# jjhbw/GoMILP

Measured on AMD Instinct MI355X. Metric: simplex pivots/sec on 2048x4096 fp64 dense LP, higher is better.
Workload: dtype f64

## Files before the change

gomilp_amd/csrc/c_api.cpp:

```cpp
#include <math.h>
#include <stdint.h>
#include <stdio.h>
#include <stdlib.h>
#include <string.h>

#include <atomic>
#include <chrono>
#include <condition_variable>
#include <deque>
#include <functional>
#include <map>
#include <memory>
#include <mutex>
#include <string>
#include <thread>
#include <vector>

#include "engine.hpp"
#include "engine_batch.hpp"
#include "engine_batch_revised.hpp"
#include "lu_host.h"

using gomilp::BatchEngine;
using gomilp::Engine;
// ... 625 lines not shown

extern "C" {

int gomilp_frontier_solve_roots(gomilp_pool *pool, int64_t count, const int32_t *root_of, const int64_t *koff, const int32_t *var,
                                const double *sign, const double *rhs, double tol, double *z_out, double *x_out, int64_t ldx,
                                int32_t *status_out, int32_t *has_x_out, gomilp_frontier_stats *stats) {
    return frontier_solve_impl(pool, count, root_of, koff, var, sign, rhs, tol, z_out, x_out, ldx, status_out, has_x_out, stats, nullptr);
}

int gomilp_frontier_solve_warm(gomilp_pool *pool, int64_t count, const int64_t *koff, const int32_t *var, const double *sign,
                               const double *rhs, const int64_t *parent, const int64_t *tag, const int32_t *keep, int32_t dual_budget,
                               double tol, double *z_out, double *x_out, int32_t *status_out, int32_t *has_x_out,
                               gomilp_frontier_stats *stats) {
    if (!pool) return GOMILP_ERR_BAD_SHAPE;
    WarmArgs wa{parent, tag, keep, dual_budget};
    return frontier_solve_impl(pool, count, nullptr, koff, var, sign, rhs, tol, z_out, x_out, pool->n0, status_out, has_x_out, stats, &wa);
}

int gomilp_pool_release_warm(gomilp_pool *pool, int64_t tag) {
    if (!pool) return GOMILP_ERR_BAD_SHAPE;
    std::lock_guard<std::mutex> g(pool->call_mu);
    if (tag < 0) pool->warm.clear(); else pool->warm.release(tag);
    return GOMILP_OK;
}

int gomilp_frontier_solve(gomilp_pool *pool, int64_t count, const int64_t *koff, const int32_t *var, const double *sign,
                          const double *rhs, double tol, double *z_out, double *x_out, int32_t *status_out,
                          int32_t *has_x_out, gomilp_frontier_stats *stats) {
    if (!pool) return GOMILP_ERR_BAD_SHAPE;
    return gomilp_frontier_solve_roots(pool, count, nullptr, koff, var, sign, rhs, tol, z_out, x_out, pool->n0, status_out, has_x_out, stats);
}

int gomilp_pool_solve_root(gomilp_pool *pool, double tol, double *opt_f, double *opt_x, int32_t *has_x, gomilp_lp_stats *stats) {
    if (!pool || pool->root[0] < 0) return GOMILP_ERR_BAD_SHAPE;
    std::lock_guard<std::mutex> g(pool->call_mu);
    return pool->eng[0]->solve(pool->root[0], tol, nullptr, opt_f, opt_x, has_x, nullptr, stats);
}

int gomilp_pool_add_root(gomilp_pool *pool, const double *c, const double *A, int64_t lda, const double *b, int64_t m, int64_t n) {
    if (!pool) return -GOMILP_ERR_BAD_SHAPE;
    std::lock_guard<std::mutex> g(pool->call_mu);
    if (pool->root[0] < 0) return -GOMILP_ERR_BAD_SHAPE;
    const int64_t id = pool->eng[0]->upload(c, A, lda, b, m, n);
    if (id < 0) return (int)id;
    std::unique_ptr<Engine::RootView> v(new Engine::RootView);
    if (!pool->eng[0]->root_view(id, v.get())) return -GOMILP_ERR_DEVICE;
    if (!v->unit_basis && v->verify_status == GOMILP_OK) pool->eng[0]->root_general(id, v.get());
    pool->extra_root.push_back(id);
    pool->extra_view.push_back(std::move(v));
    return (int)pool->extra_root.size();
}

int64_t gomilp_debug_find_independent(const double *A, int64_t lda, int64_t m, int64_t n, int64_t *idx_out, int fast) {
    if (!A || !idx_out || m <= 0 || n <= 0 || lda < n || m > 4096 || n > (1 << 20)) return -GOMILP_ERR_BAD_SHAPE;
    std::vector<double> a((size_t)m * n);
    for (int64_t i = 0; i < m; i++) for (int64_t j = 0; j < n; j++) a[(size_t)i * n + j] = A[i * lda + j];
    std::vector<int32_t> idx;
    if (fast) gomilp::general_find_linearly_independent(a, (int)m, (int)n, idx);
    else gomilp::general_find_linearly_independent_slow(a, (int)m, (int)n, idx);
    for (size_t k = 0; k < idx.size(); k++) idx_out[k] = idx[k];
    return (int64_t)idx.size();
}

double gomilp_debug_cond_estimate(const double *B, int64_t n, int inf) {
    if (!B || n <= 0 || n > 4096) return -1.0;
    std::vector<double> b((size_t)n * n), inv;
    for (int64_t i = 0; i < n * n; i++) b[(size_t)i] = B[i];
    if (!gomilp::general_invert(b, (int)n, inv)) return -1.0;
    double norm = 0;
    if (!inf) { for (int64_t j = 0; j < n; j++) { double s2 = 0; for (int64_t i = 0; i < n; i++) s2 += fabs(b[(size_t)(i * n + j)]); norm = std::max(norm, s2); } }
    else { for (int64_t i = 0; i < n; i++) { double s2 = 0; for (int64_t j = 0; j < n; j++) s2 += fabs(b[(size_t)(i * n + j)]); norm = std::max(norm, s2); } }
    return norm * gomilp::inverse_norm1_estimate(inv, (int)n, inf != 0);
}

int gomilp_debug_gonum_lu_cond(const double *M, int64_t n, int transposed, double *cond) {
    if (!M || !cond || n < 1 || n > gomilp::kGonumCondMax) return -1;
    bool dz = false;
    if (!gomilp::gonum_lu_cond(M, (int)n, (int)n, transposed != 0, cond, &dz)) return -1;
    return dz ? 1 : 0;
}

int gomilp_debug_lu_host_solve(int64_t m, int64_t nd, const int32_t *dl, const int32_t *phys, const double *diag, const double *W, int coupled,
                               const double *rhs, double *x) {
    if (m < 1 || m > 16384 || nd < 0 || nd > m || !phys || !diag || !rhs || !x || (nd > 0 && (!dl || !W))) return -1;
    const int64_t nx = coupled ? nd : m;
    for (int64_t i = 0; i < nx; i++) x[i] = 0.0;
    if (gomilp::lu_det_is_zero(diag, phys, (int)m)) return 1;
    if (coupled) {
        std::vector<double> xdl((size_t)nd);
        gomilp::lu_host_solve_coupled((int)nd, dl, phys, diag, W, rhs, xdl.data(), x);
    } else gomilp::lu_host_solve((int)m, (int)nd, dl, phys, diag, W, rhs, x);
    return 0;
}

int64_t gomilp_debug_find_independent_device(gomilp_ctx *ctx, int64_t problem, int64_t *idx_out, int64_t cap) {
    if (!ctx || !idx_out) return -GOMILP_ERR_BAD_SHAPE;
    std::vector<int32_t> idx;
    const int rc = ctx->eng->debug_find_independent(problem, idx);
    if (rc != GOMILP_OK && rc != GOMILP_ERR_SINGULAR) return -rc;
    for (size_t k = 0; k < idx.size() && (int64_t)k < cap; k++) idx_out[k] = idx[k];
    return (int64_t)idx.size();
}

long long gomilp_debug_loop_rep_launches(void) { return gomilp::bt_loop_rep_launches(); }
#ifdef GOMILP_DEBUG
void gomilp_debug_luc_stamps(unsigned long long *out) { gomilp::luc_stamps_read(out); }
void gomilp_debug_lux_stamps(unsigned long long *out) { gomilp::lux_stamps_read(out); }
void gomilp_debug_res_stamps(unsigned long long *out) { gomilp::res_stamps_read(out); }
#endif

int64_t gomilp_lp_last_trace(gomilp_ctx *ctx, gomilp_pivot *out, int64_t cap) {
    if (!ctx) return -1;
    return ctx->eng->last_trace(out, cap);
}

namespace {
constexpr int kFlatMaxCtx = 32;
struct FlatPool {
    std::mutex mu;
    std::condition_variable cv;
    std::vector<gomilp_ctx *> free_list;
    int created = 0;
};
FlatPool &flat_pool(int dev) {
    static std::mutex mu;
    static std::map<int, FlatPool *> pools;
    std::lock_guard<std::mutex> g(mu);
    auto it = pools.find(dev);
    if (it == pools.end()) it = pools.emplace(dev, new FlatPool).first;
    return *it->second;
}
}

int gomilp_lp_simplex(const double *c, const double *A, int64_t lda, const double *b, int64_t m, int64_t n, double tol,
                      const int64_t *initial_basic, double *opt_f, double *opt_x, int32_t *has_x, int64_t *basis_out,
                      gomilp_lp_stats *stats) {
    if (has_x) *has_x = 0;
    if (opt_f) *opt_f = NAN;
    if (!c || !A || !b || !opt_f || !opt_x || !has_x || m <= 0 || n <= 0 || lda < n) return GOMILP_ERR_BAD_SHAPE;
    int dev = 0;
    if (gomilp::device_count() <= 0 || hipGetDevice(&dev) != hipSuccess) return GOMILP_ERR_DEVICE;
    FlatPool &fp = flat_pool(dev);
    gomilp_ctx *ctx = nullptr;
    {
        std::unique_lock<std::mutex> lk(fp.mu);
        for (;;) {
            if (!fp.free_list.empty()) { ctx = fp.free_list.back(); fp.free_list.pop_back(); break; }
            if (fp.created < kFlatMaxCtx) { fp.created++; break; }
            fp.cv.wait(lk);
        }
    }
    if (!ctx) {
        int st = 0;
        ctx = gomilp_ctx_create(dev, &st);
        if (!ctx) {
            { std::lock_guard<std::mutex> lk(fp.mu); fp.created--; }
            fp.cv.notify_one();
            return st;
        }
    }
    int rc;
    int64_t id = ctx->eng->upload(c, A, lda, b, m, n, true);
    if (id < 0) rc = (int)-id;
    else {
        rc = gomilp_lp_solve_resident(ctx, id, tol, initial_basic, opt_f, opt_x, has_x, basis_out, stats);
        gomilp_lp_free(ctx, id);
    }
    { std::lock_guard<std::mutex> lk(fp.mu); fp.free_list.push_back(ctx); }
    fp.cv.notify_one();
    return rc;
}

}
```

gomilp_amd/csrc/device_types.h:

```cpp
#pragma once
#include <stdint.h>
#include <stdlib.h>

#ifdef GOMILP_DEBUG
#define GOMILP_DBG_ENV(name) getenv(name)
#else
#define GOMILP_DBG_ENV(name) (static_cast<const char *>(nullptr))
#endif

namespace gomilp {

enum : int32_t {
    ST_RUNNING = 0,
    ST_OPTIMAL = 1,
    ST_UNBOUNDED = 2,
    ST_NEED_BLAND = 3,
    ST_MAX_PIVOTS = 4,
    ST_LU_SINGULAR = 5,
    ST_BLAND_FAILED = 6,
    ST_FORCED_DONE = 7,
    ST_XCHG_TIMEOUT = 9,
    ST_DUAL_INFEASIBLE = 11,
    ST_NEED_EXACT = 10
};
// ... 128 lines not shown
    BS_HOST = 5,
    BS_DUAL_START = 7,
    BS_DUAL = 8,
    BS_COLD = 9
};

struct BatchLP {
    BTArgs bt;
    const double *At0;
    const double *c0, *b0;
    const int32_t *rho0;
    const int32_t *var;
    const double *sign, *rhs;
    int32_t ld0, m0, n0, K;
    int32_t m, n;
    int32_t ldu, cap_ldt;
    double *T[2];
    double *R, *xb, *U, *V, *scratch, *art;
    int32_t *basic, *nonbasic, *srcpos;
    DevState *st;
    const double *gT0;
    const double *gxb0;
    const int32_t *gbasic0, *gnonbasic0;
    const int32_t *gposvar0;
    int32_t gldt, gen;
    const double *wT, *wxb;
    const int32_t *wbasic, *wnonbasic, *wposvar;
    int32_t warm, wm;
    int32_t dual_budget, art_pos;
    int64_t pivd;
    const double *A0r;
    int32_t lda0r, virt, virt_t0, pad2;
    double tol_user;
    int32_t stage;
    int32_t tcur;
    int32_t do_permute, do_r, r_phase;
    int32_t perm_ld_in, perm_nn_out;
    int32_t kblock;
    int32_t status;
    int32_t wrapped;
    int32_t phase1_used, pad0;
    int64_t piv1, piv2, bland;
};

struct BatchOut {
    int32_t stage, status, wrapped, phase1_used;
    int64_t piv1, piv2, bland, pivd;
    int32_t tcur, pad;
};

struct GsState {
    int32_t k;
    int32_t accept;
    int32_t kacc;
    int32_t done;
    int32_t stop_col;
    int32_t scanned;
    double nR, nRinv;
    double vv;
    double beta_last;
};

struct GsBlock {
    int32_t nacc;
    int32_t k0;
    int32_t pad0, pad1;
    double vv[16];
};

struct LUCtl {
    int32_t k_next;
    int32_t k0, k1;
    int32_t nsteps;
    int32_t ndrop;
    int32_t rounds;
    int32_t nnext;
    int32_t ksync;
    int32_t steps[32];
    int32_t prow[32];
    int32_t dropcol[32], dropin[32], dropout[32];
    int32_t next[32];
    uint32_t cnt_x, cnt_u, cnt_s;
    int32_t fault;
};

struct LUArgs {
    double *W;
    int32_t ldw, m;
    int32_t *lpos;
    int32_t *rowstep;
    unsigned long long *pk[2];
    unsigned int *pl[2];
    unsigned int *pr[2];
    DevState *st;
    const int32_t *unit_row;
    int32_t *dense_flag;
    LUCtl *ctl;
    double *Lp, *Up;
    int32_t slots, look;
    const LUCtl *ctl_prev;
    const double *Lp_prev, *Up_prev;
    int32_t *rowsnap;
    const int32_t *rowsnap_prev;
    LUCtl *ctl_base;
    int32_t round, pad3;
};

}
```

gomilp_amd/csrc/engine.cpp:

```cpp
#include "engine_work.hpp"

#include <condition_variable>
#include <atomic>

namespace gomilp {

int device_count() {
    int n = 0;
    if (hipGetDeviceCount(&n) != hipSuccess) return 0;
    return n;
}

const char *compiled_arch() { return "gfx950"; }

Engine::Engine(int device) : device_(device), w_(new Work) {}

Engine::~Engine() {
    hipSetDevice(device_);
    if (up_dA_) hipFree(up_dA_);
    if (up_stats_) hipFree(up_stats_);
    for (auto *vec : {&problems_, &child_pool_, &root_pool_})
        for (auto &p : *vec) {
            if (!p) continue;
            hipFree(p->dAt); hipFree(p->db);
            if (!p->is_child) {
                hipFree(p->dc); hipFree(p->dc1);
                if (p->dvar) hipFree(p->dvar);
                if (p->dsign) hipFree(p->dsign);
            }
        }
    for (auto &kv : kept_) if (kv.second.d) hipFree(kv.second.d);
    for (auto &b : keep_pool_) hipFree(b.first);
    w_->release_all();
    if (stream_) hipStreamDestroy(stream_);
}

namespace {
struct LoopSlots { std::mutex mu; std::condition_variable cv; int used = 0, big_waiting = 0; bool busy[4] = {false, false, false, false}; };
LoopSlots &loop_slots(int dev) { static LoopSlots s[64]; return s[dev & 63]; }
}
int Engine::loop_acquire(int dev, int weight) {
    LoopSlots &L = loop_slots(dev);
    std::unique_lock<std::mutex> lk(L.mu);
    if (weight >= 4) {
        L.big_waiting++;
        L.cv.wait(lk, [&] { return L.used == 0; });
        L.big_waiting--;
        L.used = 4;
        for (bool &b2 : L.busy) b2 = true;
        return 0;
    }
    L.cv.wait(lk, [&] { return L.used < 4 && L.big_waiting == 0; });
    L.used++;
    for (int i = 0; i < 4; i++) if (!L.busy[i]) { L.busy[i] = true; return i; }
    return 0;
}
bool Engine::loop_try_acquire_all(int dev) {
    LoopSlots &L = loop_slots(dev);
    std::lock_guard<std::mutex> lk(L.mu);
    if (L.used != 0 || L.big_waiting != 0) return false;
    L.used = 4;
    for (bool &b2 : L.busy) b2 = true;
    return true;
}
void Engine::loop_release(int dev, int weight, int slot) {
    LoopSlots &L = loop_slots(dev);
    {
        std::lock_guard<std::mutex> lk(L.mu);
        if (weight >= 4) { L.used = 0; for (bool &b2 : L.busy) b2 = false; }
        else { L.used--; L.busy[slot & 3] = false; }
    }
    L.cv.notify_all();
}

int Engine::set(const std::string &key, int64_t v) {
    std::lock_guard<std::mutex> g(mu_);
    if (key == "chunk") { if (v < 1) return GOMILP_ERR_BAD_SHAPE; chunk_ = v; }
    else if (key == "refresh") { if (v < 0) return GOMILP_ERR_BAD_SHAPE; refresh_ = v; }
    else if (key == "trace") trace_on_ = v ? 1 : 0;
    else if (key == "max_pivots") max_pivots_ = v < 0 ? 0 : v;
    else if (key == "sample_events") sample_events_ = v < 0 ? 0 : v;
    else if (key == "fused") fused_ = v ? 1 : 0;
    else if (key == "lu_look") lu_look_ = v ? 1 : 0;
    else if (key == "lu_large") lu_large_ = v ? 1 : 0;
    else if (key == "lu_blocked") lu_blocked_ = v < 0 ? 0 : (v > 2 ? 3 : v);
    else if (key == "tableau") tableau_ = v ? 1 : 0;
    else if (key == "blocked") blocked_ = v ? 1 : 0;
    else if (key == "bt_nt") { if (v != 0 && v != 256 && v != 512 && v != 1024) return GOMILP_ERR_BAD_SHAPE; bt_nt_ = v; }
    else if (key == "bt_old") bt_old_ = v ? 1 : 0;
    else if (key == "bt_upd_valu") bt_upd_valu_ = v ? 1 : 0;
#ifdef GOMILP_DEBUG
    else if (key == "bt_fault") bt_fault_ = v;
#endif
    else if (key == "general_device") general_device_ = v ? 1 : 0;
    else if (key == "lu_cross") lu_cross_ = v < 0 ? -1 : (v > 2 ? 2 : v);
    else if (key == "general_block") general_block_ = v ? 1 : 0;
    else if (key == "general_min_rows") general_min_rows_ = v < 2 ? 2 : v;
    else if (key == "bt_groups") { if (v != -1 && v != 0 && v != 2 && v != 4 && v != 8 && v != 16) return GOMILP_ERR_BAD_SHAPE; bt_groups_ = v; }
    else if (key == "bt_stamps") bt_stamps_ = v ? 1 : 0;
    else if (key == "bt_lag") bt_lag_ = v ? 1 : 0;
    else if (key == "exact_degenerate") { if (v < 0 || v > 3) return GOMILP_ERR_BAD_SHAPE; exact_degenerate_ = v; }
    else if (key == "loop_grid") { if (v < 0 || v > 4096) return GOMILP_ERR_BAD_SHAPE; loop_grid_ = v; }
    else if (key == "loop_chunk") { if (v < 32) return GOMILP_ERR_BAD_SHAPE; loop_chunk_ = v; }
    else if (key == "cond_guard") cond_guard_ = v ? 1 : 0;
    else if (key == "poll_delay") { if (v < 0 || v > 64) return GOMILP_ERR_BAD_SHAPE; poll_delay_ = v; }
    else if (key == "loop_upd") { if (v < 0) return GOMILP_ERR_BAD_SHAPE; loop_upd_ = v; }
    else if (key == "loop_rep") loop_rep_ = v ? 1 : 0;
    else if (key == "loop_g") { if (v != 0 && v != 8 && v != 16) return GOMILP_ERR_BAD_SHAPE; loop_g_ = v; }
    else if (key == "loop_k") { if (v != 0 && v != 8 && v != 12 && v != 16) return GOMILP_ERR_BAD_SHAPE; loop_k_ = v; }
    else if (key == "row_chunk") { if (v < 0 || v % 512 != 0 || v > kLdsWindowLd) return GOMILP_ERR_BAD_SHAPE; row_chunk_ = v; }
    else if (key == "block_k") { if (v < 0 || v > bt_max_k()) return GOMILP_ERR_BAD_SHAPE; block_k_ = v; }
    else return GOMILP_ERR_BAD_SHAPE;
    return GOMILP_OK;
}

int Engine::ensure_work(int m, int ncols) {
    HIP_TRY(hipSetDevice(device_));
    if (!stream_) HIP_TRY(hipStreamCreateWithFlags(&stream_, hipStreamNonBlocking));
    Work &w = *w_;
    if (!w.st) {
        int ncu = 0;
        if (hipDeviceGetAttribute(&ncu, hipDeviceAttributeMultiprocessorCount, device_) == hipSuccess && ncu > 0) ncu_ = ncu;
        HIP_TRY(dmalloc(&w.pk_price, 2 * kMaxPartials)); HIP_TRY(dmalloc(&w.pk_ratio, 2 * kMaxPartials));
        HIP_TRY(dmalloc(&w.pi_price, kMaxPartials)); HIP_TRY(dmalloc(&w.pi_ratio, kMaxPartials));
        HIP_TRY(dmalloc(&w.pv_price, kMaxPartials)); HIP_TRY(dmalloc(&w.pb_ratio, kMaxPartials)); HIP_TRY(dmalloc(&w.pd_ratio, kMaxPartials)); HIP_TRY(dmalloc(&w.px_ratio, kMaxPartials));
        for (int t = 0; t < 2; t++) {
            HIP_TRY(dmalloc(&w.lpk[t], kMaxPartials)); HIP_TRY(dmalloc(&w.lpl[t], kMaxPartials)); HIP_TRY(dmalloc(&w.lpr[t], kMaxPartials));
        }
        HIP_TRY(dmalloc(&w.st, 1));
        HIP_TRY(hipHostMalloc(reinterpret_cast<void **>(&w.st_host), sizeof(DevState), hipHostMallocDefault));
        HIP_TRY(dmalloc(&w.luctl, 2));
        HIP_TRY(hipHostMalloc(reinterpret_cast<void **>(&w.luctl_host), 2 * sizeof(LUCtl), hipHostMallocDefault));
        w.trace_cap = 1 << 18;
        HIP_TRY(dmalloc(&w.trace, (size_t)w.trace_cap));
        HIP_TRY(hipEventCreate(&w.ev[0])); HIP_TRY(hipEventCreate(&w.ev[1]));
    }
    const int ld = (m + 1) & ~1;
    if (m <= w.cap_m && ncols <= w.cap_cols) return GOMILP_OK;
    const int nm = std::max(m + 32 + m / 16, w.cap_m), nc = std::max(ncols + 64 + ncols / 16, w.cap_cols);
    const int nld = std::max((nm + 1) & ~1, w.cap_ld);
    w.release();
    for (auto &p : w.binv) HIP_TRY(dmalloc(&p, (size_t)nm * nld));
    HIP_TRY(dmalloc(&w.W, (size_t)nm * nld));
    HIP_TRY(dmalloc(&w.xb, (size_t)nld)); HIP_TRY(dmalloc(&w.yb[0], (size_t)nld)); HIP_TRY(dmalloc(&w.yb[1], (size_t)nld));
    HIP_TRY(dmalloc(&w.dvec, (size_t)nld));
    HIP_TRY(dmalloc(&w.move, (size_t)nld)); HIP_TRY(dmalloc(&w.rvec, (size_t)nc));
    HIP_TRY(dmalloc(&w.yscratch, (size_t)64 * nld));
    HIP_TRY(dmalloc(&w.basic, (size_t)nm + (size_t)nc)); w.nonbasic = w.basic + nm;
    HIP_TRY(dmalloc(&w.lpos, (size_t)nm)); HIP_TRY(dmalloc(&w.rowstep, (size_t)3 * nm)); HIP_TRY(dmalloc(&w.rho, (size_t)nm));
    HIP_TRY(dmalloc(&w.unitrow, (size_t)nm)); HIP_TRY(dmalloc(&w.denseflag, (size_t)nm)); HIP_TRY(dmalloc(&w.dlist, (size_t)nm));
    HIP_TRY(dmalloc(&w.ludiag, (size_t)nm)); HIP_TRY(dmalloc(&w.Wd, (size_t)nm * nld + 512));
    HIP_TRY(dmalloc(&w.luLp, (size_t)64 * nld)); HIP_TRY(dmalloc(&w.luUp, (size_t)64 * nld));
    HIP_TRY(hipHostMalloc(reinterpret_cast<void **>(&w.h_W), ((size_t)nm * nld + 512) * sizeof(double), hipHostMallocDefault));
    HIP_TRY(hipHostMalloc(reinterpret_cast<void **>(&w.h_vec), (size_t)std::max(nld, nc) * sizeof(double), hipHostMallocDefault));
    HIP_TRY(hipHostMalloc(reinterpret_cast<void **>(&w.h_chk), (size_t)nld * sizeof(double), hipHostMallocDefault));
    HIP_TRY(hipHostMalloc(reinterpret_cast<void **>(&w.h_idx), ((size_t)nm + (size_t)nc) * sizeof(int32_t), hipHostMallocDefault));
    {
        const size_t cap = std::max<size_t>(4096, sizeof(double) * ((size_t)std::max(nld, nc) + 64));
        for (int t = 0; t < Work::kStageSlots; t++) {
            if (w.stage_cap[t] >= cap) continue;
            if (w.stage_inflight) { hipStreamSynchronize(stream_); w.stage_inflight = 0; }
            if (w.stage_buf[t]) hipHostFree(w.stage_buf[t]);
            w.stage_buf[t] = nullptr; w.stage_cap[t] = 0;
            HIP_TRY(hipHostMalloc(reinterpret_cast<void **>(&w.stage_buf[t]), cap, hipHostMallocDefault));
            w.stage_cap[t] = cap;
        }
    }
    w.cap_m = nm; w.cap_ld = nld; w.cap_cols = nc;
    return GOMILP_OK;
}

int64_t Engine::upload(const double *c, const double *A, int64_t lda, const double *b, int64_t m64, int64_t n64, bool lazy_host) {
    std::lock_guard<std::mutex> g(mu_);
    if (!c || !A || !b || m64 <= 0 || n64 <= 0 || lda < n64 || m64 > (1 << 20) || n64 > (1 << 22)) return -GOMILP_ERR_BAD_SHAPE;
    const int m = (int)m64, n = (int)n64;
    const int ld = (m + 1) & ~1;
    if (ld > kLdsWindowLd && lds_window_only_) return -GOMILP_ERR_UNSUPPORTED;
    if (hipSetDevice(device_) != hipSuccess) return -GOMILP_ERR_DEVICE;
    if (!stream_ && hipStreamCreateWithFlags(&stream_, hipStreamNonBlocking) != hipSuccess) return -GOMILP_ERR_DEVICE;
    const double t0 = now_s();
    const size_t need_at = (size_t)(n + 1) * ld, need_c = (size_t)n + 1, need_b = (size_t)ld;
    std::unique_ptr<Problem> P;
    for (size_t i = 0; i < root_pool_.size(); i++) {
        Problem &q = *root_pool_[i];
        if (q.cap_at >= need_at && q.cap_c >= need_c && q.cap_b >= need_b) {
            P = std::move(root_pool_[i]);
            root_pool_.erase(root_pool_.begin() + i);
            break;
        }
    }
    const bool recycled = (bool)P;
    if (ld > kLdsWindowLd) {
        const size_t dbl = (up_dA_cap_ < (size_t)m * n ? (size_t)m * n : 0) + (recycled ? 0 : need_at + 2 * need_c + need_b);
        if (!device_fits(dbl * sizeof(double))) {
            if (recycled) root_pool_.push_back(std::move(P));
            return -GOMILP_ERR_UNSUPPORTED;
        }
    }
    if (!P) P.reset(new Problem);
    P->m = m; P->n = n; P->ld = ld;
    double *dA = nullptr;
    int32_t *dstats = nullptr;
    auto fail = [&](int code) -> int64_t {
        if (P->dAt) hipFree(P->dAt);
        if (P->dc) hipFree(P->dc);
        if (P->dc1) hipFree(P->dc1);
        if (P->db) hipFree(P->db);
        return -code;
    };
#define UP_TRY(expr) do { if ((expr) != hipSuccess) return fail(GOMILP_ERR_DEVICE); } while (0)
    if (up_dA_cap_ < (size_t)m * n) {
        if (up_dA_) hipFree(up_dA_);
        up_dA_ = nullptr; up_dA_cap_ = 0;
        UP_TRY(dmalloc(&up_dA_, (size_t)m * n));
        up_dA_cap_ = (size_t)m * n;
// ... 804 lines not shown
        {
            LPArgs a = make_args(P, 1, 1e-10, 0, P.dc1);
            launch_ftran(a, 0, -1, n, stream_);
            launch_update(a, 0, (int)minidx, 1, 0, stream_);
            launches_ += 2;
            cur_ ^= 1;
        }
        basic[minidx] = n;
        build_nonbasic(n + 1);
        if ((rc = upload_index_lists(basic, nonbasic)) != GOMILP_OK) return finish(rc);
        refresh_xb_y(P, P.dc1);
        HIP_TRY(hipMemcpyAsync(w.h_vec, w.xb, (size_t)m * sizeof(double), hipMemcpyDeviceToHost, stream_));
        HIP_TRY(sync_stream());
        for (int i = 0; i < m; i++) if (w.h_vec[i] < -1e-13) return finish(GOMILP_ERR_PANIC);
        rc = run_loop(P, 1, 1e-10, (int)nonbasic.size(), P.dc1, st);
        if (rc == GOMILP_ERR_DEVICE) return finish(rc);
        if (rc != GOMILP_OK) { st->wrapped_status = rc; return finish(GOMILP_ERR_PHASE1_WRAPPED); }
        HIP_TRY(hipMemcpyAsync(w.h_idx, w.basic, (size_t)m * sizeof(int32_t), hipMemcpyDeviceToHost, stream_));
        HIP_TRY(hipMemcpyAsync(w.h_vec, w.xb, (size_t)m * sizeof(double), hipMemcpyDeviceToHost, stream_));
        HIP_TRY(sync_stream());
        int added = -1;
        for (int i = 0; i < m; i++) { basic[i] = w.h_idx[i]; xb[i] = w.h_vec[i]; if (basic[i] == n) added = i; }
        double xart = added >= 0 ? xb[added] : 0.0;
        if (added >= 0 && fabs(xart) > 1e-13 && fabs(xart) < 1e-11) {
            if ((rc = final_solve(P, xb_exact, &singular)) != GOMILP_OK) return finish(rc);
            if (!singular) xart = xb_exact[added];
        }
        if (fabs(xart) > 1e-12) return finish(GOMILP_ERR_INFEASIBLE);
        if (added >= 0) {
            bool exchanged = false;
            std::vector<char> inb(n + 1, 0);
            for (int i = 0; i < m; i++) inb[basic[i]] = 1;
            for (int j = 0; j < n && !exchanged; j++) {
                if (inb[j]) continue;
                w.st_host->done = 0; w.st_host->status = ST_RUNNING; w.st_host->rq = 0;
                sync_state_to_device();
                LPArgs a = make_args(P, 1, 1e-10, 0, P.dc1);
                launch_ftran(a, 0, -1, j, stream_);
                launches_++;
                HIP_TRY(hipMemcpyAsync(w.h_vec, w.dvec, (size_t)m * sizeof(double), hipMemcpyDeviceToHost, stream_));
                HIP_TRY(sync_stream());
                double dmax = 0;
                for (int i = 0; i < m; i++) dmax = std::max(dmax, fabs(w.h_vec[i]));
                const double dpv = w.h_vec[added];
                if (!(fabs(dpv) > 1e-9 * std::max(1.0, dmax))) continue;
                const double theta = xb[added] / dpv;
                bool feas = true;
                for (int i = 0; i < m && feas; i++) {
                    const double v = (i == added) ? theta : xb[i] - theta * w.h_vec[i];
                    if (v < -1e-13) feas = false;
                }
                if (!feas) continue;
                launch_update(a, 0, added, 1, 0, stream_);
                launches_++;
                cur_ ^= 1;
                basic[added] = j;
                exchanged = true;
                st->art_exchanges++;
            }
            if (!exchanged) return finish(GOMILP_ERR_INFEASIBLE);
        }
    }

    build_nonbasic(n);
    if ((rc = upload_index_lists(basic, nonbasic)) != GOMILP_OK) return finish(rc);
    if (st->phase1_used) {
        refresh_xb_y(P, P.dc);
    } else {
        launch_y_from_binv(w.binv[cur_], P.ld, m, P.dc, w.basic, w.yscratch, w.yb[ycur_], stream_);
        launches_ += 2;
    }
    loop_rc = run_loop(P, 2, tol, (int)nonbasic.size(), P.dc, st);
    }
    rc = solve_tail(P, id, loop_rc, basic, xb, basic_start, unit_basis ? &rho : nullptr, opt_f, opt_x, has_x, basis_out, st);
    return finish(rc);
}

int Engine::solve_tail(const Problem &P, int64_t id, int loop_rc, std::vector<int32_t> &basic, std::vector<double> &xb,
                       const std::vector<int32_t> &basic_start, const std::vector<int32_t> *rho_slack, double *opt_f, double *opt_x,
                       int32_t *has_x, int64_t *basis_out, gomilp_lp_stats *st) {
    const double inf = std::numeric_limits<double>::infinity();
    const int m = P.m, n = P.n;
    Work &w = *w_;
    if (loop_rc == GOMILP_ERR_DEVICE) return loop_rc;
    const bool loop_unbounded = loop_rc == GOMILP_ERR_UNBOUNDED;
    if (loop_unbounded && !shadow_trace_) { *opt_f = -inf; return loop_rc; }

    HIP_TRY(hipMemcpyAsync(w.h_idx, w.basic, (size_t)m * sizeof(int32_t), hipMemcpyDeviceToHost, stream_));
    HIP_TRY(hipMemcpyAsync(w.h_vec, w.xb, (size_t)m * sizeof(double), hipMemcpyDeviceToHost, stream_));
    HIP_TRY(sync_stream());
    for (int i = 0; i < m; i++) { basic[i] = w.h_idx[i]; xb[i] = w.h_vec[i]; }
    if (shadow_trace_ && (loop_rc == GOMILP_OK || loop_rc == GOMILP_ERR_BLAND || loop_unbounded)) {
        HIP_TRY(hipMemcpyAsync(w.st_host, w.st, sizeof(DevState), hipMemcpyDeviceToHost, stream_));
        HIP_TRY(sync_stream());
        const int64_t cnt = std::min<int64_t>(w.st_host->trace_len, w.trace_cap);
        std::vector<DevPivot> tr((size_t)cnt);
        if (cnt) HIP_TRY(hipMemcpy(tr.data(), w.trace, (size_t)cnt * sizeof(DevPivot), hipMemcpyDeviceToHost));
        std::vector<std::pair<int, int>> piv;
        for (auto &e : tr) piv.emplace_back((int)e.replace, (int)e.entering);
        std::vector<int32_t> bas = basic_start;
        int cst = GOMILP_OK;
        int64_t evals = 0;
        const int stop = general_condition_replay(P.hA, m, n, bas, piv, loop_unbounded, &cst, &evals);
        st->cond_fallbacks += evals;
        if (cst != GOMILP_OK) {
            std::vector<double> xs;
            if (general_solve_basis(P.hA, m, n, bas, P.hb, xs)) {
                std::vector<double> cb(m);
                for (int i = 0; i < m; i++) cb[i] = P.hc[bas[i]];
                *opt_f = dot_unitary(cb.data(), xs.data(), m);
                for (int j = 0; j < n; j++) opt_x[j] = 0;
                for (int i = 0; i < m; i++) opt_x[bas[i]] = xs[i];
                *has_x = 1;
                if (basis_out) for (int i = 0; i < m; i++) basis_out[i] = bas[i];
                st->pivots_phase2 = stop;
                shadow_trace_ = false;
                return cst;
            }
        }
    }
    shadow_trace_ = false;
    if (loop_unbounded) { *opt_f = -inf; return loop_rc; }
    if (keep_id_ == id && loop_rc == GOMILP_OK) keep_capture(P, id, st->pipeline, basic, basic_start, rho_slack);
    const int rc = epilogue(P, basic, xb, loop_rc, opt_f, opt_x, has_x, basis_out, st);
    if (rc == GOMILP_ERR_DEVICE) return rc;
    if (trace_on_) {
        HIP_TRY(hipMemcpyAsync(w.st_host, w.st, sizeof(DevState), hipMemcpyDeviceToHost, stream_));
        HIP_TRY(sync_stream());
        last_trace_total_ = w.st_host->trace_len;
        const int64_t cnt = std::min<int64_t>(last_trace_total_, w.trace_cap);
        std::vector<DevPivot> tmp((size_t)cnt);
        if (cnt) HIP_TRY(hipMemcpy(tmp.data(), w.trace, (size_t)cnt * sizeof(DevPivot), hipMemcpyDeviceToHost));
        last_trace_.resize((size_t)cnt);
        for (int64_t i = 0; i < cnt; i++) {
            last_trace_[i].phase = tmp[i].phase; last_trace_[i].bland = tmp[i].bland;
            last_trace_[i].min_idx = tmp[i].min_idx; last_trace_[i].replace = tmp[i].replace;
            last_trace_[i].entering = tmp[i].entering; last_trace_[i].leaving = tmp[i].leaving;
        }
    }
    return rc;
}

int Engine::epilogue(const Problem &P, std::vector<int32_t> &basic, std::vector<double> &xb, int loop_rc, double *opt_f,
                     double *opt_x, int32_t *has_x, int64_t *basis_out, gomilp_lp_stats *st) {
    const int m = P.m, n = P.n;
    std::vector<double> xb_exact;
    bool singular = false;
    const double t1 = now_s();
    int rc = final_solve(P, xb_exact, &singular, basic.data());
    if (rc != GOMILP_OK) return rc;
    st->seconds_final_solve = now_s() - t1;
    if (singular) {
        xb_exact = xb;
        if (loop_rc == GOMILP_OK) loop_rc = GOMILP_ERR_CONDITION;
    }
    double drift = 0;
    for (int i = 0; i < m; i++) drift = std::max(drift, fabs(xb[i] - xb_exact[i]));
    st->drift_xb = drift;
    std::vector<double> cb(m);
    for (int i = 0; i < m; i++) cb[i] = P.hc[basic[i]];
    *opt_f = dot_unitary(cb.data(), xb_exact.data(), m);
    for (int j = 0; j < n; j++) opt_x[j] = 0;
    for (int i = 0; i < m; i++) opt_x[basic[i]] = xb_exact[i];
    *has_x = 1;
    if (basis_out) for (int i = 0; i < m; i++) basis_out[i] = basic[i];
    return loop_rc;
}

bool Engine::root_view(int64_t id, RootView *out) {
    std::lock_guard<std::mutex> g(mu_);
    if (id < 0 || (size_t)id >= problems_.size() || !problems_[id]) return false;
    const Problem &P = *problems_[id];
    out->gen.reset();
    out->m = P.m; out->n = P.n; out->ld = P.ld; out->dAt = P.dAt; out->dc = P.dc; out->db = P.db;
// ... 250 lines not shown
```

gomilp_amd/csrc/engine.hpp:

```cpp
#pragma once
#include <hip/hip_runtime_api.h>
#include <stdint.h>

#include <functional>
#include <map>
#include <memory>
#include <mutex>
#include <string>
#include <vector>

#include "../../include/gomilp_lp.h"
#include "device_types.h"

namespace gomilp {

constexpr int kLdsWindowLd = 8192;
constexpr int kAutoRowChunk = 4096;

struct Problem {
    int m = 0, n = 0, ld = 0;
    double *dAt = nullptr;
    double *dc = nullptr;
    double *dc1 = nullptr;
    double *db = nullptr;
    std::vector<double> hb, hc;
    mutable std::vector<double> hA;
    std::vector<int32_t> nnz, lastrow, allone;
    int verify_status = GOMILP_OK;
    double seconds_upload = 0;
    uint64_t serial = 0;
    bool lazy_host = false;
    double scale_span = 1.0;
    bool is_child = false;
    size_t cap_at = 0, cap_c = 0, cap_b = 0;
    int32_t *dvar = nullptr;
    double *dsign = nullptr;
    int cap_k = 0;
    int64_t root = -1;
    const Problem *root_ptr = nullptr;
    std::vector<int32_t> kvar;
    std::vector<double> ksign;
};

struct LuPlan {
    int m = 0;
    bool compressed = false;
    bool blocked = false;
    bool large = false;
    bool small = false;
    bool look_wanted = false;
    int cross_G = 0;
    int cross_slots = 16;
    bool oneshot = false;
    bool inject_fault = false;
    int steps_down = 0;
    bool split(int nd) const { return compressed && m >= 1024 && nd > 0; }
    static LuPlan make(int m, int64_t lu_blocked, int64_t lu_look, int64_t lu_cross, int64_t lu_large, int64_t bt_fault, size_t small_pack_cap_bytes);
    bool step_down();
};
struct LuRoundsEnd { bool gave_up = false, landed = false; int enq = 0; };

class Engine {
   public:
    explicit Engine(int device);
    ~Engine();
    int device() const { return device_; }
    static int loop_acquire(int dev, int weight);
    static void loop_release(int dev, int weight, int slot);
    static bool loop_try_acquire_all(int dev);
    int set(const std::string &key, int64_t v);

    int64_t upload(const double *c, const double *A, int64_t lda, const double *b, int64_t m, int64_t n, bool lazy_host = false);
    int free_problem(int64_t id);
    int64_t upload_child(int64_t root, int K, const int32_t *var, const double *sign, const double *rhs);
    int64_t upload_child_of(Engine &owner, int64_t root, int K, const int32_t *var, const double *sign, const double *rhs);
    int solve(int64_t id, double tol, const int64_t *initial_basic, double *opt_f, double *opt_x, int32_t *has_x,
              int64_t *basis_out, gomilp_lp_stats *stats);
    int solve_warm(int64_t id, int64_t parent, int keep, int dual_budget, double tol, double *opt_f, double *opt_x, int32_t *has_x,
                   int64_t *basis_out, gomilp_lp_stats *stats, gomilp_warm_stats *wstats);
   private:
    int solve_locked(int64_t id, double tol, const int64_t *initial_basic, double *opt_f, double *opt_x, int32_t *has_x,
                     int64_t *basis_out, gomilp_lp_stats *stats);
    int solve_cold_locked(int64_t id, double tol, const int64_t *initial_basic, double *opt_f, double *opt_x, int32_t *has_x,
                          int64_t *basis_out, gomilp_lp_stats *stats);
    int solve_tail(const Problem &P, int64_t id, int loop_rc, std::vector<int32_t> &basic, std::vector<double> &xb,
                   const std::vector<int32_t> &basic_start, const std::vector<int32_t> *rho_slack, double *opt_f, double *opt_x,
                   int32_t *has_x, int64_t *basis_out, gomilp_lp_stats *st);
    struct Kept {
        double *d = nullptr;
        size_t cap = 0;
        int m = 0, ld = 0;
        bool no_warm = false;
        std::vector<int32_t> basic;
    };
    std::map<int64_t, Kept> kept_;
    std::vector<std::pair<double *, size_t>> keep_pool_;
    int64_t keep_id_ = -1;
    void keep_capture(const Problem &P, int64_t id, int pipeline, const std::vector<int32_t> &basic, const std::vector<int32_t> &basic_start,
                      const std::vector<int32_t> *rho_slack);
    void drop_kept(int64_t id);
    bool descendant(const Problem &P, int64_t parent, int *J) const;
    int warm_locked(int64_t id, const Kept &K, int J, int dual_budget, double tol, double *opt_f, double *opt_x, int32_t *has_x,
                    int64_t *basis_out, gomilp_lp_stats *st, gomilp_warm_stats *ws);
    int run_dual_loop(const Problem &P, double tol, int nn, int dual_budget, gomilp_warm_stats *ws);
   public:
    int64_t last_trace(gomilp_pivot *out, int64_t cap);

    struct RootView {
        int m = 0, n = 0, ld = 0;
        const double *dAt = nullptr, *dc = nullptr, *db = nullptr;
        double scale_span = 1.0;
        bool unit_basis = false;
        std::vector<int32_t> rho0;
        int verify_status = GOMILP_OK;
        uint64_t serial = 0;
        std::vector<double> hb, hc;
        struct General {
            int m = 0, nn = 0, ldt = 0;
            double *dT0 = nullptr, *dxb0 = nullptr;
            int32_t *dbasic0 = nullptr, *dnonbasic0 = nullptr, *dposvar0 = nullptr;
            ~General();
        };
        std::shared_ptr<General> gen;
        struct RowMajor { double *dA = nullptr; int lda = 0; ~RowMajor(); };
        std::shared_ptr<RowMajor> rm;
    };
    bool root_view(int64_t id, RootView *out);
    bool root_general(int64_t id, RootView *out);
    int finish_from_basis(int64_t id, const int32_t *basic, const double *xb_updated, int loop_rc, double *opt_f, double *opt_x,
                          int32_t *has_x, int64_t *basis_out, gomilp_lp_stats *stats);
    int debug_find_independent(int64_t id, std::vector<int32_t> &idxs);

    void limit_rows_to_lds_window() { lds_window_only_ = true; }

   private:
    struct Work;
    int row_chunk2(const Problem &P) const;
    bool device_fits(size_t bytes);
    bool large_solve_fits(const Problem &P);
    int ensure_work(int m, int ncols);
    const Problem *problem_ptr(int64_t id);
    int64_t upload_child_impl(const Problem &R, int64_t root_id, int K, const int32_t *var, const double *sign, const double *rhs);
    LPArgs make_args(const Problem &P, int phase, double tol, int nn, const double *cost);
    int run_loop(const Problem &P, int phase, double tol, int nn, const double *cost, gomilp_lp_stats *st);
    int run_loop_fused(const Problem &P, int phase, double tol, int nn, const double *cost, gomilp_lp_stats *st);
    int run_loop_tab(const Problem &P, int phase, double tol, int nn, gomilp_lp_stats *st);
    int host_bland_tab(const Problem &P, int phase, double tol, int nn, gomilp_lp_stats *st, int *par_out);
    TabArgs make_tab_args(const Problem &P, int phase, double tol, int nn);
    int tab_forced_pivot(const Problem &P, int phase, double tol, int nn, int q, int ent, double rq, int p, double dp, double xp,
                         int lea, int flags, long long t);
    int solve_tableau(const Problem &P, double tol, std::vector<int32_t> &basic, const std::vector<int32_t> &rho,
                      std::vector<double> &xb, bool feasible, gomilp_lp_stats *st, int *loop_rc,
                      const std::vector<double> *binv_host);
    void bt_layout(const Problem &P, bool tiled);
    BTArgs make_bt_args(const Problem &P, int phase, double tol, int nn, int kmax);
    void bt_plan(const Problem &P, int *K, bool *tiled, bool *lag = nullptr) const;
    int bt_forced_pivot(const Problem &P, int phase, double tol, int nn, int q, int p, int nocommit);
    int run_loop_bt(const Problem &P, int phase, double tol, int nn, gomilp_lp_stats *st);
    void account_samples(gomilp_lp_stats *st, const std::vector<int64_t> &sample_t, int64_t executed, int nk);
    int host_bland(const Problem &P, LPArgs &a, gomilp_lp_stats *st);
    int refresh_xb_y(const Problem &P, const double *cost);
    int epilogue(const Problem &P, std::vector<int32_t> &basic, std::vector<double> &xb, int loop_rc, double *opt_f, double *opt_x,
                 int32_t *has_x, int64_t *basis_out, gomilp_lp_stats *st);
    int final_solve(const Problem &P, std::vector<double> &xb_exact, bool *singular, const int32_t *basic_host = nullptr,
                    bool transpose = false, const double *rhs_host = nullptr);
    int lu_factor(const Problem &P, bool *singular, const int32_t *basic_host = nullptr, bool transpose = false);
    int lu_solve(const Problem &P, std::vector<double> &x, const double *rhs_host = nullptr);
    int gather_basis(const Problem &P, const LuPlan &plan, bool transpose);
    int upload_unit_rows(const Problem &P, const int32_t *basic_host, bool transpose, int *nonunit);
    int run_compressed_rounds(const LUArgs &a, const LuPlan &plan, int nonunit, LuRoundsEnd *end);
    int pack_and_fetch(const LUArgs &a, const LuPlan &plan, std::vector<int32_t> &dl);
    struct LuCache {
        bool valid = false, split = false, singular = false;
        int m = 0, nd = 0;
        std::vector<int32_t> phys, dl;
        std::vector<double> diag;
        LUArgs args;
    } lu_cache_;
    int exact_step(const Problem &P, int phase, double tol, int nn, int *q_out, int *p_out, gomilp_lp_stats *st);
    int exact_iter(const Problem &P, int phase, double tol, int nn, double *y_dev, double *r_dev, int ldr,
                   const std::function<int(int, int, const std::vector<int32_t> &, const std::vector<double> &)> &check_column, int *q_out,
                   int *p_out, gomilp_lp_stats *st);
    int exact_column_check(const Problem &P, const std::vector<int32_t> &basic, const std::vector<double> &dsol, const double *col_dev,
                           double *binv_dst, bool *rebuilt, gomilp_lp_stats *st);
    int cond_check(const Problem &P, int nn, double *k1, double *kinf);
    int cond_fresh(const Problem &P, const int32_t *basic_host, double *k1, double *kinf);
    int groups_knob(const Problem &P) const;
    bool ensure_host_A(const Problem &P);
    int find_independent_device(const Problem &P, std::vector<int32_t> &basic, std::vector<double> *binv_out, bool *binv_on_device = nullptr);
    int stage_upload(void *dst, const void *src, size_t bytes);
    hipError_t sync_stream();
    int upload_index_lists(const std::vector<int32_t> &basic, const std::vector<int32_t> &nonbasic);
    void sync_state_to_device();

    int device_;
    hipStream_t stream_ = nullptr;
    int ncu_ = 256;
    std::mutex mu_;
    std::vector<std::unique_ptr<Problem>> problems_;
    std::vector<std::unique_ptr<Problem>> child_pool_;
    std::vector<std::unique_ptr<Problem>> root_pool_;
    double *up_dA_ = nullptr; size_t up_dA_cap_ = 0;
    int32_t *up_stats_ = nullptr; size_t up_stats_cap_ = 0;
    std::unique_ptr<Work> w_;
    int64_t lu_look_faults_ = 0;
    int lu_look_fault_ = 0;
    int64_t lu_look_ = 1;
    int64_t lu_large_ = 0;
    int64_t chunk_ = 32, refresh_ = 0, trace_on_ = 0, max_pivots_ = 0, sample_events_ = 0, fused_ = 1, lu_blocked_ = 3, tableau_ = 1, blocked_ = 1, block_k_ = 0,
            bt_nt_ = 0, bt_old_ = 0, bt_stamps_ = 0, bt_upd_valu_ = 0, bt_fault_ = 0, general_device_ = 1, general_block_ = 1, general_min_rows_ = 96, lu_cross_ = -1, bt_groups_ = 0,
            bt_lag_ = 1,
            loop_chunk_ = 512,
            loop_grid_ = 0,
            poll_delay_ = 0,
            loop_upd_ = 0,
            loop_rep_ = 0,
            loop_g_ = 0,
            loop_k_ = 0,
            exact_degenerate_ = 1,
            cond_guard_ = 1,
            row_chunk_ = 0;
    bool lds_window_only_ = false;
    bool badly_scaled_ = false;
    bool gen_binv_dev_ = false;
    bool gen_start_ = false;
    bool gen_revised_ = false;
    double lp_guard_ = 0.0;
    std::vector<double> exact_xb_;
    bool xchg_timeout_ = false;
    bool shadow_trace_ = false;
    int cur_ = 0;
    int ycur_ = 0;
    int grid_ratio_ = 1;
    int tcur_ = 0, rcur_ = 0, ldt_ = 0;
    bool t_tiled_ = false;
    bool use_bt_ = false;
    int64_t launches_ = 0;
    double fs_device_ = 0, fs_host_ = 0;
    int64_t lu_dense_ = 0, lu_rounds_ = 0;
    std::vector<gomilp_pivot> last_trace_;
    int64_t last_trace_total_ = 0;
};

int general_find_linearly_independent(const std::vector<double> &A, int m, int n, std::vector<int32_t> &idxs, std::vector<double> *binv_out = nullptr);
int general_finish_last_column(const std::vector<double> &A, int m, int n, std::vector<int32_t> &idxs, int start_col, std::vector<double> *binv_out);
int general_find_linearly_independent_slow(const std::vector<double> &A, int m, int n, std::vector<int32_t> &idxs);
bool general_basis_inverse(const std::vector<double> &A, int m, int n, const std::vector<int32_t> &basic, int ncols_with_art,
                           const std::vector<double> &art, std::vector<double> &binv);

int general_condition_replay(const std::vector<double> &A, int m, int n, std::vector<int32_t> &basic, const std::vector<std::pair<int, int>> &pivots,
                             bool ended_in_compute_move, int *status_out, int64_t *evaluations);
double general_cond_inf(const std::vector<double> &A, int n);
bool general_invert(const std::vector<double> &B, int m, std::vector<double> &inv);
double inverse_norm1_estimate(const std::vector<double> &M, int n, bool transposed);
constexpr int kGonumCondMax = 64;
bool gonum_lu_cond(const double *M, int n, int ldm, bool transposed, double *cond, bool *det_zero);
bool gonum_lu_solve(const double *M, int n, int ldm, const double *b, double *x);
double general_basis_cond1(const std::vector<double> &A, int m, int n, const std::vector<int32_t> &basic, const std::vector<double> &art);
bool general_solve_basis(const std::vector<double> &A, int m, int n, const std::vector<int32_t> &basic, const std::vector<double> &b, std::vector<double> &x);

int device_count();
const char *compiled_arch();

int launch_price(const LPArgs &a, hipStream_t s, hipEvent_t e0 = nullptr, hipEvent_t e1 = nullptr);
int launch_ftran(const LPArgs &a, int nparts_price, int forced_pos, int forced_var, hipStream_t s, hipEvent_t e0 = nullptr,
                 hipEvent_t e1 = nullptr);
void launch_update(const LPArgs &a, int nparts_ratio, int forced_p, int no_swap, int bland, hipStream_t s,
                   hipEvent_t e0 = nullptr, hipEvent_t e1 = nullptr);
void launch_dual_leave(const double *xb, int m, double tol, DevState *st, hipStream_t s);
int launch_dual_price(const LPArgs &a, hipStream_t s);
void launch_warm_binv(const double *Bp, int ldp, int mp, double *B, int ld, int m, const int32_t *kpos, const double *ksign, hipStream_t s);
void launch_tab_to_binv(const double *T, int ldt, bool tiled, int m, const int32_t *src, double *B, int ld, hipStream_t s);
bool fused_supported(int ld);
int launch_price_fused(const LPArgs &a, const double *y_in, double *y_out, int pending, int nparts_ratio, hipStream_t s,
                       hipEvent_t e0, hipEvent_t e1);
int launch_update_ftran_fused(const LPArgs &a, int pending, int nparts_price, hipStream_t s, hipEvent_t e0, hipEvent_t e1);
int tab_ld(int nn);
int launch_tableau_pivot(const TabArgs &a, int flags, int nparts, long long t, hipStream_t s, hipEvent_t e0, hipEvent_t e1);
void launch_tab_gather(const double *At, int ld, int m, int nn, const int32_t *nonbasic, const int32_t *rho, double *T, int ldt,
                       bool tiled, hipStream_t s);
void launch_tab_gemm(const double *Binv, int ldb, const double *At, int ld, int m, int nn, const int32_t *nonbasic, double *T, int ldt, bool tiled, hipStream_t s);
void launch_tab_permute_cols(const double *Tin, int ld_in, double *Tout, int ld_out, int m, int nn_out, const int32_t *srcpos,
                             bool tiled, hipStream_t s);
int tab_r_chunks(int m);
void launch_tab_r(const double *T, int ldt, int m, int nn, const double *cost, const int32_t *basic, const int32_t *nonbasic,
                  double *scratch, double *r, bool tiled, hipStream_t s);
void launch_tab_row_colmax(const double *T, int ldt, int m, int nn, int row, double *out, bool tiled, hipStream_t s);
void launch_tab_column(const double *T, int ldt, int m, int jp, const double *xb, double *dvec, double *move, bool tiled, hipStream_t s);
void launch_cond_check(const double *T, int ldt, int m, int nn, const int32_t *nonbasic, const int32_t *basic, const double *At, int ld, int slack0, int nvar,
                       double *scratch, bool tiled, hipStream_t s);
void launch_exact_r(const double *At, int ld, int m, int nn, const int32_t *nonbasic, const double *y, const double *cost, double *r, int ldt, hipStream_t s);
void launch_gs_init(double *QT, int ldq, int m, GsState *st, hipStream_t s);
void launch_gs_init_perm(double *QT, double *Rinv, int ldq, int m, const int32_t *perm, const double *sgn, const double *beta, int s0, GsState *st, hipStream_t s);
void launch_gs_candidate(const double *acol, double *QT, double *Rinv, int ldq, int m, double *w, double *t, double *ypart, int cand, int32_t *idxs, GsState *st, hipStream_t s,
                         int last = 0);
int launch_luc_rounds_cross(const LUArgs &base, int32_t *pivrow, int nrounds, int round_base, double *xrec, int G, int slots, hipStream_t s);
size_t luc_cross_doubles();
void launch_luc_lpos_final(const LUArgs &a, hipStream_t s);
int luc_cross_groups(int m, int want);
int luc_large_rpt(int m);
int gs_scratch_rows();
int gs_block_width(int m);
int gs_block_scratch_rows();
void launch_gs_block(const double *At, int ld, int col0, int ncand, double *QT, double *Rinv, int ldq, int m, double *scratch, int32_t *idxs, GsState *st, hipStream_t s);
void launch_gs_binv(const double *Rinv, const double *QT, int ldq, int m, double *C, hipStream_t s);
void launch_gs_art(const double *At, int ld, int m, const int32_t *basic, int minidx, const double *b, double *art, hipStream_t s);
void launch_gs_norms(const double *C, int ldq, int m, double *out, const double *At, int ld, const int32_t *idxs, int cand, double *colsum, hipStream_t s);
bool bt_supported(int m, int nn);
int bt_max_k();
int bt_reg_k(int m, int ldt, int nt_force);
bool bt_tiled(int m, int ldt, int kmax, int nt_force, bool old_only);
BtGroupCfg bt_group_cfg(int m, int ldt, int knob);
size_t bt_xbuf_doubles();
void launch_bt_inner_groups(const BTArgs &a, hipStream_t s, hipEvent_t e0, hipEvent_t e1);
const char *bt_group_kernel_name(int G, int ri);
constexpr int kBtStampSegs = 16;
void launch_bt_tile(const double *src, double *dst, int m, int ldt, bool to_tiles, hipStream_t s);
void launch_bt_inner(const BTArgs &a, hipStream_t s, hipEvent_t e0, hipEvent_t e1);
void launch_bt_update(const BTArgs &a, hipStream_t s, hipEvent_t e0, hipEvent_t e1);
bool bt_loop_supported(const BtGroupCfg &c);
void launch_bt_loop(const BTArgs &a, int ncu, hipStream_t s, hipEvent_t e0, hipEvent_t e1);
bool bt_loop_rep_supported(int m, int ldt);
int bt_loop_rep_threads(int m, int ldt);
long long bt_loop_rep_launches();
void launch_bt_loop_rep(const BTArgs &a, int ncu, hipStream_t s, hipEvent_t e0, hipEvent_t e1);
bool bt_batch_supported(int m_max, int ldt_max);
int bt_batch_k(int m_max, int ldt_max);
void launch_bt_inner_batch(const BatchLP *lps, const int *ids, const int *count, int nlp, int m_max, int ldt_max, hipStream_t s, hipEvent_t e0 = nullptr, hipEvent_t e1 = nullptr, int xcd_off = 0);
void launch_bt_update_batch(const BatchLP *lps, const int *ids, const int *count, int nlp, int m_max, int ldt_max, hipStream_t s, hipEvent_t e0 = nullptr, hipEvent_t e1 = nullptr);
const char *bt_batch_kernel_name(int m_max, int ldt_max);
bool bt_virt_batch_supported(int m_max, int ldt_max);
void launch_bt_inner_virt_batch(const BatchLP *lps, const int *ids, const int *count, int nlp, hipStream_t s, hipEvent_t e0 = nullptr, hipEvent_t e1 = nullptr);
int b_loop_slots(int ncu);
bool b_loop_supported(int m_max, int ldt_max);
void launch_b_loop(const BatchLP *lps, const int *ids, const int *count, int nlp, int nblocks, int par, hipStream_t s, hipEvent_t e0 = nullptr, hipEvent_t e1 = nullptr);
size_t b_res_slot_bytes();
int b_res_max_slots();
int b_res_groups(int m_max, int nn_max, int ldt_max);
void launch_b_res(const BatchLP *lps, const int *ids, const int *count, int nlp, int G, int nb, double seq0, void *xbase, hipStream_t s, hipEvent_t e0 = nullptr, hipEvent_t e1 = nullptr);
int batch_ldt(int nn);
void launch_b_setup(BatchLP *lps, int nlp, hipStream_t s);
void launch_b_setup_warm(BatchLP *lps, int nlp, hipStream_t s);
void launch_b_posvar(const int32_t *basic, int m, const int32_t *nonbasic, int nn, int32_t *posvar, hipStream_t s);
bool bt_dual_batch_supported(int m_max, int ldt_max);
void launch_bt_inner_dual_batch(const BatchLP *lps, const int *ids, const int *count, int nlp, int m_max, int ldt_max, hipStream_t s);
void launch_b_gather(const BatchLP *lps, int nlp, int m_max, int ldt_max, int mode, hipStream_t s);
void launch_b_write_virt(const BatchLP *lps, const int *ids, const int *count, int *list, int *nalive, int bound, int m_max, int ldt_max, int ncu, hipStream_t s);
void launch_b_ctrl(BatchLP *lps, const int *ids_in, const int *count_in, int bound, int n_max, BatchOut *outs, int *ids_out, int *count_out, int loop_par, hipStream_t s);
void launch_b_init_ids(int *ids, int *count, int nlp, hipStream_t s);
void launch_b_permute(const BatchLP *lps, const int *ids, const int *count, int bound, int m_max, int ldt_max, hipStream_t s);
void launch_b_tab_r(const BatchLP *lps, const int *ids, const int *count, int bound, int m_max, int ldt_max, hipStream_t s);
void launch_transpose_in(const double *A, int64_t lda, int m, int n, double *At, int ld, hipStream_t s);
void launch_col_stats(const double *At, int ld, int m, int n, int32_t *nnz, int32_t *lastrow, int32_t *allone, int32_t *rowflag, unsigned long long *range,
                      hipStream_t s);
void launch_set_binv_perm(double *binv, int ld, int m, const int32_t *rho, hipStream_t s);
void launch_child_assemble(const double *At0, int ld0, int m0, int n0, double *At1, int ld1, int K, const int32_t *var,
                           const double *sign, hipStream_t s);
void launch_matvec_rows(const double *M, int ld, int m, const double *vec, double *out, hipStream_t s, int row_chunk2 = 0);
int y_chunks(int m);
void launch_y_from_binv(const double *binv, int ld, int m, const double *cost, const int32_t *basic, double *scratch,
                        double *y, hipStream_t s);
void launch_gather_w(const double *At, int ld, int m, const int32_t *basic, double *W, int ldw, hipStream_t s);
int lu_grid(int m);
void launch_lu(const LUArgs &a, hipStream_t s);
bool lu_blocked_supported(int m);
int launch_lu_blocked(const LUArgs &a, int32_t *pivrow, hipStream_t s);
bool lu_compressed_supported(int m, bool large);
int lu_compressed_nb();
void launch_luc_init(const LUArgs &a, hipStream_t s);
int launch_luc_rounds(const LUArgs &a, int32_t *pivrow, int nrounds, int round_base, hipStream_t s);
void launch_luc_gather(const double *At, int ld, int m, const int32_t *basic, double *W, int ldw, hipStream_t s);
void launch_luc_pack_dense(const LUArgs &a, const int32_t *dlist, int nd, const int32_t *pivrow, double *Wdd, double *diag, hipStream_t s);
void launch_luc_solve_rows(const LUArgs &a, const int32_t *dlist, int nd, const double *b, const double *xdL, const double *xdU,
                           double *x, hipStream_t s);
void launch_luc_pack(const LUArgs &a, const int32_t *dlist, int nd, double *Wd, double *diag, hipStream_t s);
void launch_luc_pack_small(const LUArgs &a, double *out, hipStream_t s);
size_t luc_pack_small_bytes(int m);
void launch_lu_pack(const LUArgs &a, const int32_t *dlist, int nd, double *Wd, double *diag, hipStream_t s);

}
```

gomilp_amd/csrc/engine_final.cpp:

```cpp
#include <stdio.h>
#include <stdlib.h>

#include "engine_work.hpp"
#include "lu_host.h"

namespace gomilp {

int Engine::final_solve(const Problem &P, std::vector<double> &x, bool *singular, const int32_t *basic_host, bool transpose, const double *rhs_host) {
    int rc = lu_factor(P, singular, basic_host, transpose);
    if (rc != GOMILP_OK) return rc;
    return lu_solve(P, x, rhs_host);
}

LuPlan LuPlan::make(int m, int64_t lu_blocked, int64_t lu_look, int64_t lu_cross, int64_t lu_large, int64_t bt_fault, size_t small_pack_cap_bytes) {
    LuPlan p;
    p.m = m;
    p.compressed = lu_blocked >= 2 && lu_compressed_supported(m, lu_large != 0);
    p.large = p.compressed && luc_large_rpt(m) > 0;
    p.blocked = p.compressed || (lu_blocked && lu_blocked_supported(m));
    p.small = p.compressed && m <= 128;
    p.inject_fault = bt_fault == 2;
    const int cross_mode = lu_cross >= 0 ? (int)lu_cross : ((m > 1280 && m <= 2048 && lu_look) ? 2 : 0);
    p.cross_G = p.large ? 8 : ((cross_mode && p.compressed) ? luc_cross_groups(m, 1) : 0);
    p.cross_slots = (p.large ? lu_cross == 2 : cross_mode == 2) ? 32 : 16;
    p.look_wanted = lu_blocked >= 3 && lu_look && m > 768 && p.compressed && !p.large && !(p.cross_G && cross_mode != 2);
    p.oneshot = p.small && !p.cross_G && luc_pack_small_bytes(m) <= small_pack_cap_bytes;
    return p;
}

bool LuPlan::step_down() {
    if (steps_down >= 2 || !(look_wanted || cross_G)) return false;
    steps_down++;
    if (look_wanted) look_wanted = false; else cross_G = 0;
    if (large) compressed = blocked = large = false;
    oneshot = false;
    return true;
}

namespace {

struct LookSlot {
    int dev; bool held;
    LookSlot(int d, bool want) : dev(d), held(want && Engine::loop_try_acquire_all(d)) {}
    ~LookSlot() { drop(); }
    void drop() { if (held) Engine::loop_release(dev, 4, 0); held = false; }
};

}

int Engine::gather_basis(const Problem &P, const LuPlan &plan, bool transpose) {
    Work &w = *w_;
    if (plan.compressed != transpose) launch_luc_gather(P.dAt, P.ld, P.m, w.basic, w.W, P.ld, stream_);
    else {
        if (transpose) HIP_TRY(hipMemsetAsync(w.W, 0, (size_t)P.m * P.ld * sizeof(double), stream_));
        launch_gather_w(P.dAt, P.ld, P.m, w.basic, w.W, P.ld, stream_);
    }
    return GOMILP_OK;
}

int Engine::upload_unit_rows(const Problem &P, const int32_t *basic_host, bool transpose, int *nonunit) {
    Work &w = *w_;
    const int m = P.m;
    if (!basic_host) {
        HIP_TRY(hipMemcpyAsync(w.h_idx, w.basic, (size_t)m * sizeof(int32_t), hipMemcpyDeviceToHost, stream_));
        HIP_TRY(sync_stream());
        basic_host = w.h_idx;
    }
    std::vector<int32_t> ur(m);
    *nonunit = 0;
    for (int pos = 0; pos < m; pos++) {
        const int j = basic_host[pos];
        ur[pos] = (!transpose && j < P.n && P.nnz[j] == 1 && P.allone[j]) ? P.lastrow[j] : -1;
        if (ur[pos] < 0) (*nonunit)++;
    }
    return stage_upload(w.unitrow, ur.data(), (size_t)m * sizeof(int32_t));
}

int Engine::run_compressed_rounds(const LUArgs &a, const LuPlan &plan, int nonunit, LuRoundsEnd *end) {
    Work &w = *w_;
    const int m = a.m;
    int32_t *h_dense = w.h_idx + w.cap_m;
    launch_luc_init(a, stream_);
    launches_++;
    const int nb = lu_compressed_nb();
    int batch = std::max(1, (std::min(m, (5 * nonunit) / 2) + nb - 1) / nb);
    bool oneshot = plan.oneshot;
    if (oneshot && GOMILP_DBG_ENV("GOMILP_DEBUG_LU_SHORT")) batch = 1;
    int enq = 0;
    int k_seen = -1;
    const LUCtl *last = w.luctl_host;
    for (;;) {
        launches_ += plan.cross_G ? launch_luc_rounds_cross(a, w.rho, batch, enq, w.luxrec, plan.cross_G, plan.cross_slots, stream_) : launch_luc_rounds(a, w.rho, batch, enq, stream_);
        enq += batch;
        if (oneshot) {
            launch_luc_pack_small(a, w.Wd, stream_);
            launches_++;
            HIP_TRY(hipMemcpyAsync(w.h_W, w.Wd, luc_pack_small_bytes(m), hipMemcpyDeviceToHost, stream_));
            HIP_TRY(sync_stream());
            const double *blk = w.h_W;
            const int32_t *io = reinterpret_cast<const int32_t *>(blk + (size_t)m * m + m);
            memcpy(w.h_vec, blk + (size_t)m * m, (size_t)m * sizeof(double));
            memcpy(w.h_idx, io, (size_t)m * sizeof(int32_t));
            memcpy(h_dense, io + m, (size_t)m * sizeof(int32_t));
            memcpy(w.luctl_host, io + 2 * m, 2 * sizeof(LUCtl));
            w.st_host->lu_singular = io[2 * m + (int)(2 * sizeof(LUCtl) / sizeof(int32_t))];
        } else {
            HIP_TRY(hipMemcpyAsync(w.luctl_host, w.luctl, 2 * sizeof(LUCtl), hipMemcpyDeviceToHost, stream_));
            HIP_TRY(hipMemcpyAsync(h_dense, w.denseflag, (size_t)m * sizeof(int32_t), hipMemcpyDeviceToHost, stream_));
            HIP_TRY(sync_stream());
        }
        last = w.luctl_host + (a.look ? ((enq - 1) & 1) : 0);
        if (w.luctl_host[0].fault || last->k_next >= m) break;
        if (last->k_next <= k_seen) return GOMILP_ERR_DEVICE;
        k_seen = last->k_next;
        oneshot = false;
        batch = std::max(4, (int)(((int64_t)(m - last->k_next) * last->rounds) / std::max(1, last->k_next)) + 2);
        if (batch > 64) batch = 64;
    }
    lu_rounds_ = last->rounds;
    end->gave_up = w.luctl_host[0].fault != 0;
    end->landed = oneshot;
    end->enq = enq;
    if (plan.cross_G && !end->gave_up) { launch_luc_lpos_final(a, stream_); launches_++; }
    return GOMILP_OK;
}

int Engine::pack_and_fetch(const LUArgs &a, const LuPlan &plan, std::vector<int32_t> &dl) {
    Work &w = *w_;
    const int m = a.m;
    int32_t *h_dense = w.h_idx + w.cap_m;
    dl.clear();
    if (plan.blocked) {
        if (!plan.compressed) {
            HIP_TRY(hipMemcpyAsync(h_dense, w.denseflag, (size_t)m * sizeof(int32_t), hipMemcpyDeviceToHost, stream_));
            HIP_TRY(sync_stream());
        }
        for (int k = 0; k < m; k++) if (h_dense[k]) dl.push_back(k);
    } else {
        for (int k = 0; k < m; k++) dl.push_back(k);
    }
    const int nd = (int)dl.size();
    int rc = stage_upload(w.dlist, dl.data(), (size_t)nd * sizeof(int32_t));
    if (rc != GOMILP_OK) return rc;
    const bool split = plan.split(nd);
    if (split) launch_luc_pack_dense(a, w.dlist, nd, w.rho, w.Wd, w.ludiag, stream_);
    else if (plan.compressed) launch_luc_pack(a, w.dlist, nd, w.Wd, w.ludiag, stream_);
    else launch_lu_pack(a, w.dlist, nd, w.Wd, w.ludiag, stream_);
    launches_++;
    if (nd) HIP_TRY(hipMemcpyAsync(w.h_W, w.Wd, (size_t)(split ? nd : m) * nd * sizeof(double), hipMemcpyDeviceToHost, stream_));
    HIP_TRY(hipMemcpyAsync(w.h_vec, w.ludiag, (size_t)m * sizeof(double), hipMemcpyDeviceToHost, stream_));
    HIP_TRY(hipMemcpyAsync(w.h_idx, w.lpos, (size_t)m * sizeof(int32_t), hipMemcpyDeviceToHost, stream_));
    if (plan.small)
        HIP_TRY(hipMemcpyAsync(&w.st_host->lu_singular, &w.st->lu_singular, sizeof(w.st_host->lu_singular), hipMemcpyDeviceToHost, stream_));
    else
        HIP_TRY(hipMemcpyAsync(w.st_host, w.st, sizeof(DevState), hipMemcpyDeviceToHost, stream_));
    HIP_TRY(sync_stream());
    return GOMILP_OK;
}

int Engine::lu_factor(const Problem &P, bool *singular, const int32_t *basic_host, bool transpose) {
    Work &w = *w_;
    const double tf0 = now_s();
    const int m = P.m;
    LuPlan plan = LuPlan::make(m, lu_blocked_, lu_look_, lu_cross_, lu_large_, bt_fault_, ((size_t)w.cap_m * w.cap_ld + 512) * sizeof(double));
    lu_cache_.valid = false;
    int rc = gather_basis(P, plan, transpose);
    if (rc != GOMILP_OK) return rc;
    int nonunit = 0;
    if ((rc = upload_unit_rows(P, basic_host, transpose, &nonunit)) != GOMILP_OK) return rc;
    LookSlot look_slot(device_, plan.look_wanted);
    if (!look_slot.held) plan.look_wanted = false;
    LUArgs a;
    a.W = w.W; a.ldw = P.ld; a.m = m; a.lpos = w.lpos; a.rowstep = w.rowstep;
    for (int t = 0; t < 2; t++) { a.pk[t] = w.lpk[t]; a.pl[t] = w.lpl[t]; a.pr[t] = w.lpr[t]; }
    a.st = w.st;
    a.unit_row = w.unitrow;
    a.dense_flag = plan.blocked ? w.denseflag : nullptr;
    a.ctl = w.luctl; a.Lp = w.luLp; a.Up = w.luUp;
    a.slots = 1; a.look = plan.look_wanted ? 1 : 0;
    a.ctl_prev = a.ctl; a.Lp_prev = a.Lp; a.Up_prev = a.Up;
    a.rowsnap = w.rowstep + w.cap_m; a.rowsnap_prev = a.rowsnap;
    a.ctl_base = a.ctl; a.round = 0; a.pad3 = plan.inject_fault ? 1 : 0;
    if (plan.cross_G && !w.luxrec) {
        HIP_TRY(dmalloc(&w.luxrec, luc_cross_doubles()));
        HIP_TRY(hipMemsetAsync(w.luxrec, 0, luc_cross_doubles() * sizeof(double), stream_));
    }
    w.st_host->lu_singular = 0;
    if (!plan.small) sync_state_to_device();
    lu_rounds_ = 0;
    LuRoundsEnd end;
    if (plan.compressed) {
        for (;;) {
            rc = run_compressed_rounds(a, plan, nonunit, &end);
            look_slot.drop();
            if (rc != GOMILP_OK) return rc;
            if (!end.gave_up) break;
            if (!plan.step_down()) return GOMILP_ERR_DEVICE;
            a.look = 0; a.dense_flag = plan.blocked ? w.denseflag : nullptr;
            lu_look_faults_++; lu_look_fault_++;
            if (w.luxrec) HIP_TRY(hipMemsetAsync(w.luxrec, 0, luc_cross_doubles() * sizeof(double), stream_));
            if (GOMILP_DBG_ENV("GOMILP_DEBUG_LOOP")) fprintf(stderr, "final_solve: a look-ahead launch gave up a wait (m %d, rounds enqueued %d, cnt_x %u cnt_u %u cnt_s %u): plain schedule\n", m, end.enq, w.luctl_host[0].cnt_x, w.luctl_host[0].cnt_u, w.luctl_host[0].cnt_s);
            if ((rc = gather_basis(P, plan, transpose)) != GOMILP_OK) return rc;
            if (!plan.compressed) { lu_rounds_ = 0; sync_state_to_device(); launch_lu(a, stream_); launches_ += m + 2; end = LuRoundsEnd(); break; }
        }
    } else if (plan.blocked) launches_ += launch_lu_blocked(a, w.rho, stream_) + 1;
    else { launch_lu(a, stream_); launches_ += m + 2; }
    std::vector<int32_t> dl;
    if (end.landed) {
        dl.resize(m);
        for (int k = 0; k < m; k++) dl[k] = k;
        const int32_t *h_dense = w.h_idx + w.cap_m;
        lu_dense_ = 0;
        for (int k = 0; k < m; k++) lu_dense_ += h_dense[k] != 0;
    } else {
        if ((rc = pack_and_fetch(a, plan, dl)) != GOMILP_OK) return rc;
        lu_dense_ = (int64_t)dl.size();
    }
    const int nd = (int)dl.size();
    HIP_TRY(hipGetLastError());
    const double tf1 = now_s();
    fs_device_ += tf1 - tf0;
    std::vector<int32_t> phys(m);
    for (int R = 0; R < m; R++) phys[w.h_idx[R]] = R;
    const double *diag = w.h_vec;
    *singular = w.st_host->lu_singular != 0 || lu_det_is_zero(diag, phys.data(), m);
    if (*singular && GOMILP_DBG_ENV("GOMILP_DEBUG_LOOP")) {
        int nz = 0; double dmin = 1e300, logdet = 0;
        for (int i = 0; i < m; i++) { if (diag[phys[i]] == 0) nz++; dmin = std::min(dmin, fabs(diag[phys[i]])); logdet += log(fabs(diag[phys[i]])); }
        fprintf(stderr, "final_solve: singular (transpose %d, m %d, nd %d, rounds %lld, lu_singular flag %d, logdet %g, zero diagonals %d, min |u_ii| %g, compressed %d)\n",
                (int)transpose, m, nd, (long long)lu_rounds_, (int)w.st_host->lu_singular, logdet, nz, dmin, (int)plan.compressed);
    }
    lu_cache_.m = m; lu_cache_.nd = nd; lu_cache_.split = !end.landed && plan.split(nd); lu_cache_.singular = *singular;
    lu_cache_.phys = phys; lu_cache_.dl = dl;
    lu_cache_.diag.assign(diag, diag + m);
    lu_cache_.args = a;
    lu_cache_.valid = true;
    fs_host_ += now_s() - tf1;
    return GOMILP_OK;
}

int Engine::lu_solve(const Problem &P, std::vector<double> &x, const double *rhs_host) {
    Work &w = *w_;
    const LuCache &c = lu_cache_;
    if (!c.valid || c.m != P.m) return GOMILP_ERR_DEVICE;
    const double tf1 = now_s();
    const int m = P.m, nd = c.nd;
    const double *rhs = rhs_host ? rhs_host : P.hb.data();
    x.assign(m, 0.0);
    if (c.singular) return GOMILP_OK;
    if (!c.split) {
        lu_host_solve(m, nd, c.dl.data(), c.phys.data(), c.diag.data(), w.h_W, rhs, x.data());
        fs_host_ += now_s() - tf1;
        return GOMILP_OK;
    }
    const double *rhs_dev = P.db;
    if (rhs_host) {
        int rcr = stage_upload(w.move, rhs_host, (size_t)m * sizeof(double));
        if (rcr != GOMILP_OK) return rcr;
        rhs_dev = w.move;
    }
    std::vector<double> xdl(nd), xdu(nd);
    lu_host_solve_coupled(nd, c.dl.data(), c.phys.data(), c.diag.data(), w.h_W, rhs, xdl.data(), xdu.data());
    fs_host_ += now_s() - tf1;
    const double tf2 = now_s();
    double *dxl = w.yscratch, *dxu = w.yscratch + P.ld, *dx = w.yscratch + 2 * (size_t)P.ld;
    int rcs = stage_upload(dxl, xdl.data(), (size_t)nd * sizeof(double));
    if (rcs == GOMILP_OK) rcs = stage_upload(dxu, xdu.data(), (size_t)nd * sizeof(double));
    if (rcs != GOMILP_OK) return rcs;
    launch_luc_solve_rows(c.args, w.dlist, nd, rhs_dev, dxl, dxu, dx, stream_);
    launches_++;
    HIP_TRY(hipMemcpyAsync(w.h_vec, dx, (size_t)m * sizeof(double), hipMemcpyDeviceToHost, stream_));
    HIP_TRY(sync_stream());
    HIP_TRY(hipGetLastError());
    for (int i = 0; i < m; i++) x[i] = w.h_vec[i];
    for (int s = 0; s < nd; s++) x[c.dl[s]] = xdu[s];
    fs_device_ += now_s() - tf2;
    return GOMILP_OK;
}

}
```

gomilp_amd/csrc/engine_tableau.cpp:

```cpp
#include <stdio.h>
#include <stdlib.h>

#include "engine_work.hpp"

namespace gomilp {

TabArgs Engine::make_tab_args(const Problem &P, int phase, double tol, int nn) {
    Work &w = *w_;
    TabArgs a;
    memset(&a, 0, sizeof(a));
    a.m = P.m; a.nn = nn; a.ldt = ldt_; a.phase = phase; a.tol = tol;
    bt_layout(P, false);
    a.T_cur = w.T[tcur_]; a.T_next = w.T[tcur_ ^ 1];
    a.r_in = w.R[rcur_]; a.r_out = w.R[rcur_ ^ 1];
    a.xb = w.xb; a.dvec = w.dvec; a.move = w.move;
    a.basic = w.basic; a.nonbasic = w.nonbasic;
    a.pk_ratio = w.pk_ratio; a.pi_ratio = w.pi_ratio; a.pb_ratio = w.pb_ratio; a.pd_ratio = w.pd_ratio; a.px_ratio = w.px_ratio;
    a.st = w.st;
    a.trace = (trace_on_ || shadow_trace_) ? w.trace : nullptr;
    a.trace_cap = w.trace_cap;
    return a;
}

int Engine::tab_forced_pivot(const Problem &P, int phase, double tol, int nn, int q, int ent, double rq, int p, double dp,
// ... 517 lines not shown
        }
        seen = hs.pivots;
        last_par = ci.par;
        if (!hs.done) {
            if (max_pivots_ > 0 && hs.pivots >= max_pivots_) { ret = GOMILP_ERR_UNSUPPORTED; break; }
            if (!more) { ret = GOMILP_ERR_UNSUPPORTED; break; }
            if (!speculate) { int rc1 = enqueue_chunk(cur ^ 1, pred, blocks_per_chunk); if (rc1 != GOMILP_OK) return rc1; pred += blocks_per_chunk * K; }
            cur ^= 1;
            continue;
        }
        if (hs.status == ST_OPTIMAL) break;
        if (hs.status == ST_UNBOUNDED) { ret = GOMILP_ERR_UNBOUNDED; break; }
        if (hs.status == ST_BLAND_FAILED) { ret = GOMILP_ERR_BLAND; break; }
        if (hs.status == ST_NEED_EXACT) {
            if (lag) {
                tcur_ = hs.tsel2[(last_par ^ 1) & 1];
                if (launch_no > 0) hipEventSynchronize(w.pipe_ev[(int)(last_slot_enqueued)]);
            } else HIP_TRY(hipEventSynchronize(w.pipe_ev[last_slot_enqueued]));
            hs.done = 0; hs.status = ST_RUNNING;
            const DevState keep = hs;
            int fq = -1, fp = -1;
            const int verdict = exact_step(P, phase, tol, nn, &fq, &fp, st);
            hs = keep;
            hs.done = 0; hs.status = ST_RUNNING; hs.lu_singular = 0;
            hs.tsel2[0] = hs.tsel2[1] = tcur_; hs.kdone2[0] = hs.kdone2[1] = 0; hs.loop_blocks = 0;
            if (verdict < 0) { ret = -verdict; break; }
            if (verdict == 1) { hs.done = 1; hs.status = ST_OPTIMAL; break; }
            if (verdict == 2) { ret = GOMILP_ERR_UNBOUNDED; break; }
            sync_state_to_device();
            forced_q_pending = fq; forced_p_pending = fp;
            exact_pending = true;
            seg0 = hs.pivots;
            goto restart_segment;
        }
        if (hs.status == ST_XCHG_TIMEOUT && w.xbuf) {
            hipStreamSynchronize(stream_);
            hipMemsetAsync(w.xbuf, 0, bt_xbuf_doubles() * sizeof(double), stream_);
            w.loop_launches = 0;
            xchg_timeout_ = true;
        }
        if (GOMILP_DBG_ENV("GOMILP_DEBUG_LOOP")) fprintf(stderr, "run_loop_bt: device status %d after %lld pivots (lag %d, loop_blocks %d)\n", hs.status, (long long)hs.pivots, (int)lag, hs.loop_blocks);
        ret = GOMILP_ERR_DEVICE;
        break;
    }
    if (lag) {
        tcur_ = hs.tsel2[(last_par ^ 1) & 1];
        if (launch_no > 0) hipEventSynchronize(w.pipe_ev[(int)(last_slot_enqueued)]);
    }
    if (bt_stamps_ && w.stamps) {
        const size_t nb = (size_t)(16 * kBtStampSegs + 8) * sizeof(unsigned long long);
        HIP_TRY(hipMemcpyAsync(w.stamps_host, w.stamps, nb, hipMemcpyDeviceToHost, stream_));
        HIP_TRY(sync_stream());
        const unsigned long long np = w.stamps_host[16 * kBtStampSegs];
        fprintf(stderr, "{\"bt_stamps\": {\"m\": %d, \"nn\": %d, \"phase\": %d, \"pivots\": %llu, \"cycles_per_pivot_by_wave\": [", P.m, nn, phase, np);
        for (int wv = 0; wv < 16; wv++) {
            fprintf(stderr, "%s[", wv ? ", " : "");
            for (int sg = 0; sg < 13; sg++) fprintf(stderr, "%s%.1f", sg ? ", " : "", np ? (double)w.stamps_host[wv * kBtStampSegs + sg] / (double)np : 0.0);
            fprintf(stderr, "]");
        }
        fprintf(stderr, "]}}\n");
    }
    if (st) {
        st->seconds_pivot_loop += now_s() - t_loop0;
        st->bland_steps += hs.bland_steps;
        if (phase == 1) st->pivots_phase1 += hs.pivots; else st->pivots_phase2 += hs.pivots;
    }
    return ret;
}

int Engine::solve_tableau(const Problem &P, double tol, std::vector<int32_t> &basic, const std::vector<int32_t> &rho,
                          std::vector<double> &xb, bool feasible, gomilp_lp_stats *st, int *loop_rc,
                          const std::vector<double> *binv_host) {
    Work &w = *w_;
    const int m = P.m, n = P.n;
    int rc;
    std::vector<int32_t> nonbasic;
    auto build_nonbasic = [&](int ncols) {
        std::vector<char> inb(ncols, 0);
        for (int i = 0; i < m; i++) inb[basic[i]] = 1;
        nonbasic.clear();
        for (int j = 0; j < ncols; j++) if (!inb[j]) nonbasic.push_back(j);
    };
    tcur_ = 0; rcur_ = 0; t_tiled_ = false;
    if (!binv_host && (rc = stage_upload(w.rho, rho.data(), (size_t)m * sizeof(int32_t))) != GOMILP_OK) return rc;
    std::vector<double> art(P.ld, 0.0);
    bool binv_on_device = gen_binv_dev_;
    auto set_up_T = [&](int nn) -> int {
        ldt_ = tab_ld(nn);
        if (!binv_host) {
            { int K0; bool tl0; bt_plan(P, &K0, &tl0); t_tiled_ = use_bt_ && tl0; }
            launch_tab_gather(P.dAt, P.ld, m, nn, w.nonbasic, w.rho, w.T[0], ldt_, t_tiled_, stream_);
            launches_++;
            return GOMILP_OK;
        }
        { int K0; bool tl0; bt_plan(P, &K0, &tl0); t_tiled_ = use_bt_ && tl0; }
        if (!binv_on_device) {
            HIP_TRY(hipMemcpy2DAsync(w.binv[0], (size_t)P.ld * sizeof(double), binv_host->data(), (size_t)m * sizeof(double), (size_t)m * sizeof(double), m,
                                     hipMemcpyHostToDevice, stream_));
            HIP_TRY(sync_stream());
            binv_on_device = true;
        }
        launch_tab_gemm(w.binv[0], P.ld, P.dAt, P.ld, m, nn, w.nonbasic, w.T[0], ldt_, t_tiled_, stream_);
        launches_++;
        return GOMILP_OK;
    };
    int nn;
    const double t_st0 = now_s();
    if (!feasible) {
        st->phase1_used = 1;
        const int64_t minidx = min_idx(xb.data(), m);
        const bool art_on_device = binv_host && m >= general_min_rows_;
        for (int k = 0; k < m; k++) art[k] = P.hb[k];
        if (!binv_host) {
            for (int i = 0; i < m; i++) { if (i == minidx) continue; art[rho[i]] = -1 * 1.0 + art[rho[i]]; }
        } else if (!art_on_device) {
            for (int i = 0; i < m; i++) {
                if (i == minidx) continue;
                for (int k = 0; k < m; k++) art[k] = -1 * P.hA[(size_t)k * n + basic[i]] + art[k];
            }
        }
        build_nonbasic(n + 1);
        nn = (int)nonbasic.size();
        if ((rc = upload_index_lists(basic, nonbasic)) != GOMILP_OK) return rc;
        if (art_on_device) {
            launch_gs_art(P.dAt, P.ld, m, w.basic, (int)minidx, P.db, P.dAt + (size_t)n * P.ld, stream_);
            launches_++;
            HIP_TRY(hipMemcpyAsync(art.data(), P.dAt + (size_t)n * P.ld, (size_t)P.ld * sizeof(double), hipMemcpyDeviceToHost, stream_));
            HIP_TRY(sync_stream());
        }
        bool art_zero = true;
        for (int k = 0; k < m; k++) if (art[k] != 0) { art_zero = false; break; }
        if (art_zero) { st->wrapped_status = GOMILP_ERR_ZERO_COLUMN; return GOMILP_ERR_PHASE1_WRAPPED; }
        if (!art_on_device && (rc = stage_upload(P.dAt + (size_t)n * P.ld, art.data(), (size_t)P.ld * sizeof(double))) != GOMILP_OK) return rc;
        const double t_st1 = now_s();
        if ((rc = set_up_T(nn)) != GOMILP_OK) return rc;
        if (binv_host && GOMILP_DBG_ENV("GOMILP_DEBUG_GS")) { (void)sync_stream(); fprintf(stderr, "phase I set-up: artificial column + lists %.2f ms, B^-1 upload + T = B^-1 A_N %.2f ms\n", 1e3 * (t_st1 - t_st0), 1e3 * (now_s() - t_st1)); }
        const int qa = nn - 1;
        if (!use_bt_) {
            launch_tab_column(w.T[0], ldt_, m, qa, w.xb, w.dvec, w.move, t_tiled_, stream_);
            launches_++;
        }
        double dp = 0;
        if (!binv_host) dp = art[rho[minidx]];
        else if (!use_bt_) {
            std::vector<double> brow(m);
            if (gen_binv_dev_) { HIP_TRY(hipMemcpyAsync(brow.data(), w.binv[0] + (size_t)minidx * P.ld, (size_t)m * sizeof(double), hipMemcpyDeviceToHost, stream_)); HIP_TRY(sync_stream()); }
            else for (int i = 0; i < m; i++) brow[i] = (*binv_host)[(size_t)minidx * m + i];
            for (int i = 0; i < m; i++) dp += brow[i] * art[i];
        }
        const int slack = basic[minidx];
        const bool swap_on_device = use_bt_ && t_tiled_;
        if (use_bt_) rc = bt_forced_pivot(P, 1, 1e-10, nn, qa, (int)minidx, swap_on_device ? 2 : 1);
        else rc = tab_forced_pivot(P, 1, 1e-10, nn, qa, n, 0.0, (int)minidx, dp, xb[minidx], slack, 4, 0);
        if (rc != GOMILP_OK) return rc;
        basic[minidx] = n;
        nonbasic[qa] = slack;
        bool lists_current = swap_on_device;
        {
            std::vector<int32_t> asc = nonbasic;
            std::sort(asc.begin(), asc.end());
            if (asc != nonbasic) {
                std::vector<int32_t> pos_of(n + 1, -1), srcpos(nn);
                for (int jp = 0; jp < nn; jp++) pos_of[nonbasic[jp]] = jp;
                for (int jp = 0; jp < nn; jp++) srcpos[jp] = pos_of[asc[jp]];
                if ((rc = stage_upload(w.srcpos, srcpos.data(), (size_t)nn * sizeof(int32_t))) != GOMILP_OK) return rc;
                launch_tab_permute_cols(w.T[tcur_], ldt_, w.T[tcur_ ^ 1], ldt_, m, nn, w.srcpos, t_tiled_, stream_);
// ... 9 lines not shown
        HIP_TRY(hipMemcpyAsync(w.h_chk, w.xb, (size_t)m * sizeof(double), hipMemcpyDeviceToHost, stream_));
        rc = use_bt_ ? run_loop_bt(P, 1, 1e-10, nn, st) : run_loop_tab(P, 1, 1e-10, nn, st);
        if (rc == GOMILP_ERR_DEVICE) return rc;
        for (int i = 0; i < m; i++) if (w.h_chk[i] < -1e-13) return GOMILP_ERR_PANIC;
        if (rc != GOMILP_OK) { st->wrapped_status = rc; return GOMILP_ERR_PHASE1_WRAPPED; }
        const size_t gap = (size_t)(w.nonbasic - w.basic);
        HIP_TRY(hipMemcpyAsync(w.h_idx, w.basic, (gap + (size_t)nn) * sizeof(int32_t), hipMemcpyDeviceToHost, stream_));
        HIP_TRY(hipMemcpyAsync(w.h_vec, w.xb, (size_t)m * sizeof(double), hipMemcpyDeviceToHost, stream_));
        HIP_TRY(sync_stream());
        int added = -1;
        for (int i = 0; i < m; i++) { basic[i] = w.h_idx[i]; xb[i] = w.h_vec[i]; if (basic[i] == n) added = i; }
        for (int jp = 0; jp < nn; jp++) nonbasic[jp] = w.h_idx[gap + jp];
        double xart = added >= 0 ? xb[added] : 0.0;
        if (added >= 0 && fabs(xart) > 1e-13 && fabs(xart) < 1e-11) {
            std::vector<double> xe;
            bool sing = false;
            if ((rc = final_solve(P, xe, &sing)) != GOMILP_OK) return rc;
            if (!sing) xart = xe[added];
        }
        if (fabs(xart) > 1e-12) return GOMILP_ERR_INFEASIBLE;
        if (added >= 0) {
            std::vector<std::pair<int32_t, int>> cand;
            for (int jp = 0; jp < nn; jp++) if (nonbasic[jp] < n) cand.emplace_back(nonbasic[jp], jp);
            std::sort(cand.begin(), cand.end());
            bool exchanged = false;
            launch_tab_row_colmax(w.T[tcur_], ldt_, m, nn, added, w.tscratch, t_tiled_, stream_);
            launches_++;
            std::vector<double> rowmax((size_t)2 * ldt_);
            HIP_TRY(hipMemcpyAsync(rowmax.data(), w.tscratch, rowmax.size() * sizeof(double), hipMemcpyDeviceToHost, stream_));
            HIP_TRY(sync_stream());
            for (auto &cv : cand) {
                const int jp = cv.second;
                if (!(fabs(rowmax[jp]) > 1e-9 * std::max(1.0, rowmax[(size_t)ldt_ + jp]))) continue;
                launch_tab_column(w.T[tcur_], ldt_, m, jp, w.xb, w.dvec, w.move, t_tiled_, stream_);
                launches_++;
                HIP_TRY(hipMemcpyAsync(w.h_vec, w.dvec, (size_t)m * sizeof(double), hipMemcpyDeviceToHost, stream_));
                HIP_TRY(sync_stream());
                double dmax = 0;
                for (int i = 0; i < m; i++) dmax = std::max(dmax, fabs(w.h_vec[i]));
                const double dpv = w.h_vec[added];
                if (!(fabs(dpv) > 1e-9 * std::max(1.0, dmax))) continue;
                const double theta = xb[added] / dpv;
                bool feas = true;
                for (int i = 0; i < m && feas; i++) {
                    const double v = (i == added) ? theta : xb[i] - theta * w.h_vec[i];
                    if (v < -1e-13) feas = false;
                }
                if (!feas) continue;
                if (use_bt_) rc = bt_forced_pivot(P, 1, 1e-10, nn, jp, added, 1);
                else rc = tab_forced_pivot(P, 1, 1e-10, nn, jp, cv.first, 0.0, added, dpv, xb[added], n, 4, 0);
                if (rc != GOMILP_OK) return rc;
                basic[added] = cv.first;
                nonbasic[jp] = n;
                exchanged = true;
                st->art_exchanges++;
                break;
            }
            if (!exchanged) return GOMILP_ERR_INFEASIBLE;
        }
        std::vector<int32_t> old_nb = nonbasic;
        build_nonbasic(n);
        const int nn2 = (int)nonbasic.size();
        std::vector<int32_t> pos_of(n + 1, -1), srcpos(nn2);
        for (int jp = 0; jp < nn; jp++) pos_of[old_nb[jp]] = jp;
        for (int jp = 0; jp < nn2; jp++) srcpos[jp] = pos_of[nonbasic[jp]];
        if ((rc = stage_upload(w.srcpos, srcpos.data(), (size_t)nn2 * sizeof(int32_t))) != GOMILP_OK) return rc;
        const int ldt2 = tab_ld(nn2);
        launch_tab_permute_cols(w.T[tcur_], ldt_, w.T[tcur_ ^ 1], ldt2, m, nn2, w.srcpos, t_tiled_, stream_);
        launches_++;
        tcur_ ^= 1;
        ldt_ = ldt2;
        nn = nn2;
        if ((rc = upload_index_lists(basic, nonbasic)) != GOMILP_OK) return rc;
    } else {
        build_nonbasic(n);
        nn = (int)nonbasic.size();
        if ((rc = upload_index_lists(basic, nonbasic)) != GOMILP_OK) return rc;
        if ((rc = set_up_T(nn)) != GOMILP_OK) return rc;
    }
    launch_tab_r(w.T[tcur_], ldt_, m, nn, P.dc, w.basic, w.nonbasic, w.tscratch, w.R[rcur_], t_tiled_, stream_);
    launches_ += 2;
    *loop_rc = use_bt_ ? run_loop_bt(P, 2, tol, nn, st) : run_loop_tab(P, 2, tol, nn, st);
    if (*loop_rc == GOMILP_OK && cond_guard_ && !binv_host && m > 64) {
        double k1 = 0, kinf = 0;
        if ((rc = cond_check(P, nn, &k1, &kinf)) != GOMILP_OK) return rc;
        st->cond1_final = k1; st->condinf_final = kinf;
        if (k1 > 1e16 || k1 != k1 || kinf > 1e16 || kinf != kinf) *loop_rc = GOMILP_ERR_CONDITION;
    }
    return GOMILP_OK;
}

int Engine::cond_check(const Problem &P, int nn, double *k1, double *kinf) {
    Work &w = *w_;
    *k1 = *kinf = 0.0;
    const size_t need = (size_t)ldt_ + 3 * (size_t)P.ld + 4;
    if (need > (size_t)64 * w.cap_ldt) return GOMILP_OK;
    launch_cond_check(w.T[tcur_], ldt_, P.m, nn, w.nonbasic, w.basic, P.dAt, P.ld, P.n - P.m, P.n, w.tscratch, t_tiled_, stream_);
    launches_ += 3;
    HIP_TRY(hipMemcpyAsync(w.h_vec, w.tscratch + (size_t)ldt_ + 3 * (size_t)P.ld, 4 * sizeof(double), hipMemcpyDeviceToHost, stream_));
    HIP_TRY(sync_stream());
    const double b1 = w.h_vec[0], binf = w.h_vec[2];
    *k1 = b1 * w.h_vec[1];
    *kinf = binf * w.h_vec[3];
    if (!(*k1 > 1e16) && !(*kinf > 1e16)) return GOMILP_OK;
    const int m = P.m;
    const double tk1 = *k1, tkinf = *kinf;
    { int rc = cond_fresh(P, nullptr, k1, kinf); if (rc != GOMILP_OK) return rc; }
    if (GOMILP_DBG_ENV("GOMILP_DEBUG_LOOP")) fprintf(stderr, "cond_check: m %d tableau kappa_1 %.6g kappa_inf %.6g -> fresh %.6g %.6g\n", m, tk1, tkinf, *k1, *kinf);
    return GOMILP_OK;
}


int Engine::cond_fresh(const Problem &P, const int32_t *basic_host, double *k1, double *kinf) {
    Work &w = *w_;
    const int m = P.m;
    std::vector<int32_t> basic(m);
    if (basic_host) for (int i = 0; i < m; i++) basic[i] = basic_host[i];
    else {
        HIP_TRY(hipMemcpyAsync(w.h_idx, w.basic, (size_t)m * sizeof(int32_t), hipMemcpyDeviceToHost, stream_));
        HIP_TRY(sync_stream());
        for (int i = 0; i < m; i++) basic[i] = w.h_idx[i];
    }
    std::vector<double> cols((size_t)m * P.ld), B((size_t)m * m), inv;
    for (int p = 0; p < m; p++)
        HIP_TRY(hipMemcpyAsync(&cols[(size_t)p * P.ld], P.dAt + (size_t)basic[p] * P.ld, (size_t)m * sizeof(double), hipMemcpyDeviceToHost, stream_));
    HIP_TRY(sync_stream());
    for (int i = 0; i < m; i++) for (int p = 0; p < m; p++) B[(size_t)i * m + p] = cols[(size_t)p * P.ld + i];
    if (m <= kGonumCondMax) {
        bool dz = false;
        gonum_lu_cond(B.data(), m, m, true, k1, &dz);
        if (dz) *k1 = std::numeric_limits<double>::infinity();
        gonum_lu_cond(B.data(), m, m, false, kinf, &dz);
        if (dz) *kinf = std::numeric_limits<double>::infinity();
        return GOMILP_OK;
    }
    if (!general_invert(B, m, inv)) { *k1 = *kinf = std::numeric_limits<double>::infinity(); return GOMILP_OK; }
    double n1 = 0, ninf = 0, i1 = 0, iinf = 0;
    {
        std::vector<double> cb(m, 0.0), ci(m, 0.0);
        for (int i = 0; i < m; i++) {
            double rb = 0, ri = 0;
            for (int p = 0; p < m; p++) { const double vb = fabs(B[(size_t)i * m + p]), vi = fabs(inv[(size_t)i * m + p]); rb += vb; ri += vi; cb[p] += vb; ci[p] += vi; }
            ninf = std::max(ninf, rb); iinf = std::max(iinf, ri);
        }
        for (int p = 0; p < m; p++) { n1 = std::max(n1, cb[p]); i1 = std::max(i1, ci[p]); }
    }
    *k1 = n1 * i1; *kinf = ninf * iinf;
    if (*k1 > 1e16 || *kinf > 1e16) {
        *k1 = n1 * inverse_norm1_estimate(inv, m, false);
        *kinf = ninf * inverse_norm1_estimate(inv, m, true);
    }
    return GOMILP_OK;
}

}
```

gomilp_amd/csrc/engine_work.hpp:

```cpp
#pragma once
#include <math.h>
#include <string.h>

#include <algorithm>
#include <chrono>
#include <limits>

#include "engine.hpp"

namespace gomilp {

namespace {

double now_s() {
    using namespace std::chrono;
    return duration<double>(steady_clock::now().time_since_epoch()).count();
}

#ifdef GOMILP_DEBUG
#define HIP_TRY(expr)                                                                                                   \
    do {                                                                                                                \
        hipError_t _e = (expr);                                                                                         \
        if (_e != hipSuccess) {                                                                                         \
            fprintf(stderr, "gomilp: %s:%d: %s -> %s\n", __FILE__, __LINE__, #expr, hipGetErrorString(_e));              \
            return GOMILP_ERR_DEVICE;                                                                                   \
        }                                                                                                               \
    } while (0)
#else
#define HIP_TRY(expr)                                   \
    do {                                                \
        hipError_t _e = (expr);                         \
        if (_e != hipSuccess) return GOMILP_ERR_DEVICE; \
    } while (0)
#endif

int64_t min_idx(const double *s, int64_t n) {
    double mn = std::numeric_limits<double>::quiet_NaN();
    int64_t ind = 0;
    for (int64_t i = 0; i < n; i++) {
        const double v = s[i];
        if (v != v) continue;
        if (v < mn || mn != mn) { mn = v; ind = i; }
    }
    return ind;
}

double dot_unitary(const double *x, const double *y, int64_t n) {
    double s0 = 0, s1 = 0, s2 = 0, s3 = 0;
    int64_t i = 0;
    for (; i + 4 <= n; i += 4) {
        s0 += x[i] * y[i];
        s1 += x[i + 1] * y[i + 1];
        s2 += x[i + 2] * y[i + 2];
        s3 += x[i + 3] * y[i + 3];
    }
    for (; i < n; i++) s0 += x[i] * y[i];
    return (s0 + s2) + (s1 + s3);
}

template <typename T>
hipError_t dmalloc(T **p, size_t count) {
    return hipMalloc(reinterpret_cast<void **>(p), std::max<size_t>(count, 1) * sizeof(T));
}

}

struct Engine::Work {
    int cap_m = 0, cap_ld = 0, cap_cols = 0;
    double *binv[2] = {nullptr, nullptr};
    double *yb[2] = {nullptr, nullptr};
    double *xb = nullptr, *dvec = nullptr, *move = nullptr, *rvec = nullptr, *yscratch = nullptr, *W = nullptr;
    int32_t *basic = nullptr, *nonbasic = nullptr, *lpos = nullptr, *rowstep = nullptr, *rho = nullptr;
    unsigned long long *pk_price = nullptr, *pk_ratio = nullptr, *lpk[2] = {nullptr, nullptr};
    unsigned int *pi_price = nullptr, *pi_ratio = nullptr, *lpl[2] = {nullptr, nullptr}, *lpr[2] = {nullptr, nullptr};
    unsigned int *pv_price = nullptr, *pb_ratio = nullptr;
    double *pd_ratio = nullptr, *px_ratio = nullptr;
    double *T[2] = {nullptr, nullptr}, *R[2] = {nullptr, nullptr}, *tscratch = nullptr;
    double *btU = nullptr, *btV = nullptr;
    double *xbuf = nullptr;
    int64_t loop_launches = 0;
    double *luxrec = nullptr;
    GsState *gs_state = nullptr, *gs_host = nullptr;
    int32_t *gs_idx = nullptr; int cap_gs_idx = 0;
    int32_t *srcpos = nullptr;
    int32_t *unitrow = nullptr;
    int32_t *denseflag = nullptr, *dlist = nullptr;
    double *ludiag = nullptr;
    double *luLp = nullptr, *luUp = nullptr;
    double *Wd = nullptr;
    size_t cap_T = 0;
    size_t cap_btU = 0;
    unsigned long long *stamps = nullptr, *stamps_host = nullptr;
    int cap_ldt = 0;
    DevState *st = nullptr;
    DevState *st_host = nullptr;
    LUCtl *luctl = nullptr, *luctl_host = nullptr;
    DevPivot *trace = nullptr;
    int64_t trace_cap = 0;
    double *h_W = nullptr;
    double *h_vec = nullptr;
    double *h_chk = nullptr;
    int32_t *h_idx = nullptr;
    static constexpr int kStageSlots = 32;
    char *stage_buf[kStageSlots] = {};
    size_t stage_cap[kStageSlots] = {};
    int stage_next = 0;
    int stage_inflight = 0;
    char *child_stage = nullptr;
    size_t child_stage_cap = 0;
    hipEvent_t ev[2] = {nullptr, nullptr};
    DevState *pipe_state[2] = {nullptr, nullptr};
    hipEvent_t pipe_ev[2] = {nullptr, nullptr};
    std::vector<hipEvent_t> sample_ev;

    void release() {
        for (auto &p : binv) { if (p) hipFree(p); p = nullptr; }
        for (double **p : {&xb, &yb[0], &yb[1], &dvec, &move, &rvec, &yscratch, &W, &ludiag, &Wd, &luLp, &luUp}) { if (*p) hipFree(*p); *p = nullptr; }
        nonbasic = nullptr;
        for (int32_t **p : {&basic, &lpos, &rowstep, &rho, &unitrow, &denseflag, &dlist}) { if (*p) hipFree(*p); *p = nullptr; }
        if (h_W) hipHostFree(h_W); h_W = nullptr;
        if (h_vec) hipHostFree(h_vec); h_vec = nullptr;
        if (h_chk) hipHostFree(h_chk); h_chk = nullptr;
        if (h_idx) hipHostFree(h_idx); h_idx = nullptr;
        cap_m = cap_ld = cap_cols = 0;
    }
    void release_all() {
        release();
        for (auto **p : {&pk_price, &pk_ratio, &lpk[0], &lpk[1]}) { if (*p) hipFree(*p); *p = nullptr; }
        for (auto **p : {&pi_price, &pi_ratio, &lpl[0], &lpl[1], &lpr[0], &lpr[1], &pv_price, &pb_ratio}) { if (*p) hipFree(*p); *p = nullptr; }
        if (pd_ratio) hipFree(pd_ratio); pd_ratio = nullptr;
        if (px_ratio) hipFree(px_ratio); px_ratio = nullptr;
        for (double **p : {&T[0], &T[1], &R[0], &R[1], &tscratch, &btU, &btV, &xbuf}) { if (*p) hipFree(*p); *p = nullptr; }
        if (srcpos) hipFree(srcpos); srcpos = nullptr;
        cap_T = 0; cap_ldt = 0; cap_btU = 0;
        if (luxrec) hipFree(luxrec); luxrec = nullptr;
        if (gs_state) hipFree(gs_state); gs_state = nullptr;
        if (gs_host) hipHostFree(gs_host); gs_host = nullptr;
        if (gs_idx) hipFree(gs_idx); gs_idx = nullptr; cap_gs_idx = 0;
        if (stamps) hipFree(stamps); stamps = nullptr;
        if (stamps_host) hipHostFree(stamps_host); stamps_host = nullptr;
        if (st) hipFree(st); st = nullptr;
        if (st_host) hipHostFree(st_host); st_host = nullptr;
        if (child_stage) hipHostFree(child_stage); child_stage = nullptr; child_stage_cap = 0;
        if (trace) hipFree(trace); trace = nullptr;
        for (auto &e : ev) { if (e) hipEventDestroy(e); e = nullptr; }
        for (auto &e : sample_ev) hipEventDestroy(e);
        sample_ev.clear();
        for (int t = 0; t < 2; t++) {
            if (pipe_state[t]) hipHostFree(pipe_state[t]); pipe_state[t] = nullptr;
            if (pipe_ev[t]) hipEventDestroy(pipe_ev[t]); pipe_ev[t] = nullptr;
        }
        for (int t = 0; t < kStageSlots; t++) {
            if (stage_buf[t]) hipHostFree(stage_buf[t]); stage_buf[t] = nullptr; stage_cap[t] = 0;
        }
        if (luctl) hipFree(luctl); luctl = nullptr;
        if (luctl_host) hipHostFree(luctl_host); luctl_host = nullptr;
    }
};


}
```

gomilp_amd/csrc/lu_compressed.hip:

```cpp
#include <hip/hip_runtime.h>
#include <stdint.h>
#include <stdlib.h>

#include <algorithm>

#include "device_types.h"
#include "kernels_common.h"
#include "luc_role.h"

namespace gomilp {

#ifdef GOMILP_DEBUG
__device__ unsigned long long g_luc_stamps[4 * 16];
#define LUC_STAMP(S)                                                                      \
    do {                                                                                  \
        unsigned long long t_;                                                            \
        __builtin_amdgcn_sched_barrier(0);                                                \
        asm volatile("s_memtime %0\n\ts_waitcnt lgkmcnt(0)" : "=s"(t_)::"memory");        \
        __builtin_amdgcn_sched_barrier(0);                                                \
        if ((S) >= 0) tacc[(S) >= 0 ? (S) : 0] += t_ - tprev;                             \
        tprev = t_;                                                                       \
    } while (0)
#else
#define LUC_STAMP(S) do { } while (0)
// ... 401 lines not shown
    for (int idx = tid; idx < NB * 64; idx += 256) {
        const int s = idx / 64, c = idx % 64;
        Ls[s][c] = (s < ns && R0 + c < a.m) ? a.Lp[(size_t)s * ldw + R0 + c] : 0.0;
        Us[s][c] = (s < ns && j0 + c < a.m) ? a.Up[(size_t)s * ldw + j0 + c] : 0.0;
    }
    __syncthreads();
    int cls = 0;
    if (tid < 64) {
        const int R = R0 + tid;
        int rs = -1;
        if (R < a.m) {
            rs = a.rowstep[R];
            cls = rs < 0 ? 1 : (rs >= k0 ? 2 : 0);
        }
        rowcls[tid] = (unsigned char)cls;
        rstep[tid] = rs;
    } else if (tid < 128) {
        const int j = j0 + (tid - 64);
        int din = 0, dout = 0;
        for (int t = 0; t < nd; t++)
            if (Dc[t] == j) { din = Di[t]; dout = Do[t]; }
        cdin[tid - 64] = din; cdout[tid - 64] = dout;
    }
    if (!__syncthreads_or(cls > 0)) return;
    bool live[4][4];
#pragma unroll
    for (int cc = 0; cc < 4; cc++) {
        const int c = ty * 4 + cc;
#pragma unroll
        for (int rr = 0; rr < 4; rr++) {
            const int r = tx * 4 + rr;
            live[cc][rr] = rowcls[r] > 0 && (j0 + c) < a.m && !(rowcls[r] == 2 && rstep[r] >= cdin[c] && rstep[r] < cdout[c]);
        }
    }
#pragma unroll
    for (int s = 0; s < NB; s++) {
        if (s < ns) {
            double l[4], u[4];
#pragma unroll
            for (int rr = 0; rr < 4; rr++) l[rr] = Ls[s][tx * 4 + rr];
#pragma unroll
            for (int cc = 0; cc < 4; cc++) u[cc] = Us[s][ty * 4 + cc];
#pragma unroll
            for (int rr = 0; rr < 4; rr++) {
                const bool nz = l[rr] != 0;
#pragma unroll
                for (int cc = 0; cc < 4; cc++) acc[cc][rr] = nz ? __dadd_rn(__dmul_rn(l[rr], u[cc]), acc[cc][rr]) : acc[cc][rr];
            }
        }
    }
#pragma unroll
    for (int cc = 0; cc < 4; cc++) {
        const int c = ty * 4 + cc;
#pragma unroll
        for (int rr = 0; rr < 4; rr++)
            if (live[cc][rr]) a.W[(size_t)(j0 + c) * ldw + R0 + tx * 4 + rr] = acc[cc][rr];
    }
}

__global__ void k_luc_init(LUArgs a) {
    const int R = blockIdx.x * blockDim.x + threadIdx.x;
    if (R < a.m) {
        a.lpos[R] = R; a.rowstep[R] = -1;
        if (a.dense_flag) a.dense_flag[R] = 0;
    }
    if (R == 0) {
        a.st->lu_singular = 0;
        for (int t = 0; t < 2; t++) {
            LUCtl *c = a.ctl + t;
            c->k_next = 0; c->k0 = 0; c->k1 = 0; c->nsteps = 0; c->ndrop = 0; c->rounds = 0; c->nnext = 0; c->ksync = 0;
            c->cnt_x = 0; c->cnt_u = 0; c->cnt_s = 0; c->fault = 0;
        }
    }
}

__global__ __launch_bounds__(256) void k_luc_gather(const double *__restrict__ At, int ld, int m, const int32_t *__restrict__ basic,
                                                    double *__restrict__ W, int ldw) {
    const int k = blockIdx.x;
    const double *src = At + (size_t)basic[k] * ld;
    double *dst = W + (size_t)k * ldw;
    for (int R = threadIdx.x; R < ldw; R += 256) dst[R] = R < m ? src[R] : 0.0;
}

__global__ __launch_bounds__(256) void k_luc_pack(LUArgs a, const int32_t *__restrict__ dlist, int nd, double *__restrict__ Wd,
                                                  double *__restrict__ diag) {
    __shared__ double tile[32][33];
    const int t0 = blockIdx.x * 32, R0 = blockIdx.y * 32;
    const int tx = threadIdx.x & 31, ty = threadIdx.x >> 5;
    const size_t ldw = (size_t)a.ldw;
    for (int tt = ty; tt < 32; tt += 8) {
        const int t = t0 + tt, R = R0 + tx;
        tile[tt][tx] = (t < nd && R < a.m) ? a.W[(size_t)dlist[t] * ldw + R] : 0.0;
    }
    __syncthreads();
    for (int rr = ty; rr < 32; rr += 8) {
        const int R = R0 + rr, t = t0 + tx;
        if (R < a.m && t < nd) Wd[(size_t)R * nd + t] = tile[tx][rr];
    }
    if (blockIdx.x == 0 && threadIdx.x < 32) {
        const int R = R0 + threadIdx.x;
        if (R < a.m) diag[R] = a.W[(size_t)a.lpos[R] * ldw + R];
    }
}


__global__ __launch_bounds__(256) void k_luc_pack_dense(LUArgs a, const int32_t *__restrict__ dlist, int nd,
                                                        const int32_t *__restrict__ pivrow, double *__restrict__ Wdd,
                                                        double *__restrict__ diag) {
    const size_t ldw = (size_t)a.ldw;
    const int s = blockIdx.x;
    if (s < nd) {
        const int R = pivrow[dlist[s]];
        for (int t = threadIdx.x; t < nd; t += 256) Wdd[(size_t)s * nd + t] = a.W[(size_t)dlist[t] * ldw + R];
    }
    for (int R = blockIdx.x * 256 + threadIdx.x; R < a.m; R += gridDim.x * 256) diag[R] = a.W[(size_t)a.lpos[R] * ldw + R];
}

__global__ __launch_bounds__(256) void k_luc_solve_rows(LUArgs a, const int32_t *__restrict__ dlist, int nd,
                                                        const double *__restrict__ b, const double *__restrict__ xdL,
                                                        const double *__restrict__ xdU, double *__restrict__ x) {
    const int R = blockIdx.x * 256 + threadIdx.x;
    if (R >= a.m) return;
    const int i = a.lpos[R];
    if (a.dense_flag[i]) return;
    const size_t ldw = (size_t)a.ldw;
    int lo = 0, hi = nd;
    while (lo < hi) { const int mid = (lo + hi) >> 1; if (dlist[mid] < i) lo = mid + 1; else hi = mid; }
    const int cnt = lo;
    double acc = b[R];
    for (int t0 = 0; t0 < nd; t0 += 8) {
        double va[8], xk[8];
#pragma unroll
        for (int u = 0; u < 8; u++) {
            const int t = t0 + u;
            va[u] = t < nd ? a.W[(size_t)dlist[t < nd ? t : 0] * ldw + R] : 0.0;
            xk[u] = t < nd ? (t < cnt ? xdL[t] : xdU[t]) : 0.0;
        }
#pragma unroll
        for (int u = 0; u < 8; u++)
            if (va[u] != 0) acc = __dadd_rn(__dmul_rn(-va[u], xk[u]), acc);
    }
    const double tinv = 1.0 / a.W[(size_t)i * ldw + R];
    x[i] = __dmul_rn(acc, tinv);
}

constexpr int kLucSlotSteps = 32;
template <int T, int RPT, int NB>
static void luc_rounds_slots(const LUArgs &base, int32_t *pivrow, int nrounds, int round_base, hipStream_t s) {
    const int m = base.m;
    const int nt = (m + 63) / 64;
    if (!base.look) {
        LUArgs a = base;
        a.ctl_prev = a.ctl; a.Lp_prev = a.Lp; a.Up_prev = a.Up; a.rowsnap_prev = a.rowsnap;
        for (int r = 0; r < nrounds; r++) {
            hipLaunchKernelGGL((k_luc_panel_slots<T, RPT, NB, kLucSlotSteps, false>), dim3(1), dim3(T), 0, s, a, pivrow);
            hipLaunchKernelGGL((k_luc_usolve<kLucSlotSteps>), dim3(nt), dim3(256), 0, s, a);
            hipLaunchKernelGGL((k_luc_trail<kLucSlotSteps>), dim3(nt, nt), dim3(256), 0, s, a);
        }
        return;
    }
    const size_t pstride = (size_t)kLucSlotSteps * (size_t)base.ldw;
    const int rest = std::max(nt, std::min(255, (nt * nt + std::max(1, T / 256) - 1) / std::max(1, T / 256)));
    for (int r = 0; r < nrounds; r++) {
        const int p = (round_base + r) & 1;
        LUArgs a = base;
        a.ctl = base.ctl + p; a.ctl_prev = base.ctl + (p ^ 1);
        a.Lp = base.Lp + p * pstride; a.Lp_prev = base.Lp + (p ^ 1) * pstride;
        a.Up = base.Up + p * pstride; a.Up_prev = base.Up + (p ^ 1) * pstride;
        a.rowsnap = base.rowsnap + (size_t)p * m; a.rowsnap_prev = base.rowsnap + (size_t)(p ^ 1) * m;
        if (!luc_look_ok<T, RPT>()) {
            a.look = 0;
            hipLaunchKernelGGL((k_luc_panel_slots<T, RPT, NB, kLucSlotSteps, false>), dim3(1), dim3(T), 0, s, a, pivrow);
            hipLaunchKernelGGL((k_luc_usolve<kLucSlotSteps>), dim3(nt), dim3(256), 0, s, a);
            hipLaunchKernelGGL((k_luc_trail<kLucSlotSteps>), dim3(nt, nt), dim3(256), 0, s, a);
            continue;
        }
        a.ctl_base = base.ctl; a.round = round_base + r;
        if constexpr (luc_look_ok<T, RPT>()) hipLaunchKernelGGL((k_luc_panel_slots<T, RPT, NB, kLucSlotSteps, true>), dim3(1 + rest), dim3(T), 0, s, a, pivrow);
    }
}

void launch_luc_cross_panel(const LUArgs &a, int32_t *pivrow, double *xrec, int G, int slots, int nrole, hipStream_t s);
void launch_luc_large_panel(const LUArgs &a, int32_t *pivrow, double *xrec, int slots, hipStream_t s);
int luc_large_rpt(int m);
int launch_luc_rounds_cross(const LUArgs &base, int32_t *pivrow, int nrounds, int round_base, double *xrec, int G, int slots, hipStream_t s) {
    const int m = base.m, nt = (m + 63) / 64;
    if (!base.look) {
        LUArgs a = base;
        a.ctl_prev = a.ctl; a.Lp_prev = a.Lp; a.Up_prev = a.Up; a.rowsnap_prev = a.rowsnap;
        for (int r = 0; r < nrounds; r++) {
            if (luc_large_rpt(m)) launch_luc_large_panel(a, pivrow, xrec, slots, s);
            else launch_luc_cross_panel(a, pivrow, xrec, G, slots, 0, s);
            hipLaunchKernelGGL((k_luc_usolve<kLucSlotSteps>), dim3(nt), dim3(256), 0, s, a);
            hipLaunchKernelGGL((k_luc_trail<kLucSlotSteps>), dim3(nt, nt), dim3(256), 0, s, a);
        }
        return 3 * nrounds;
    }
    const size_t pstride = (size_t)kLucSlotSteps * (size_t)base.ldw;
    const int rest = std::max(nt, std::min(256 - G, nt * nt));
    for (int r = 0; r < nrounds; r++) {
        const int p = (round_base + r) & 1;
        LUArgs a = base;
        a.ctl = base.ctl + p; a.ctl_prev = base.ctl + (p ^ 1);
        a.Lp = base.Lp + p * pstride; a.Lp_prev = base.Lp + (p ^ 1) * pstride;
        a.Up = base.Up + p * pstride; a.Up_prev = base.Up + (p ^ 1) * pstride;
        a.rowsnap = base.rowsnap + (size_t)p * m; a.rowsnap_prev = base.rowsnap + (size_t)(p ^ 1) * m;
        a.ctl_base = base.ctl; a.round = round_base + r;
        launch_luc_cross_panel(a, pivrow, xrec, G, 32, rest, s);
    }
    return 3 * nrounds;
}

bool lu_compressed_supported(int m, bool large) { return m <= 4096 || (large && luc_large_rpt(m) > 0); }
int lu_compressed_nb() { return kLucSlotSteps; }

void launch_luc_init(const LUArgs &a, hipStream_t s) {
    hipLaunchKernelGGL(k_luc_init, dim3((a.m + 255) / 256), dim3(256), 0, s, a);
}
void launch_luc_gather(const double *At, int ld, int m, const int32_t *basic, double *W, int ldw, hipStream_t s) {
    hipLaunchKernelGGL(k_luc_gather, dim3(m), dim3(256), 0, s, At, ld, m, basic, W, ldw);
}
void launch_luc_pack_dense(const LUArgs &a, const int32_t *dlist, int nd, const int32_t *pivrow, double *Wdd, double *diag, hipStream_t s) {
    const int grid = std::max(nd, (a.m + 255) / 256);
    hipLaunchKernelGGL(k_luc_pack_dense, dim3(grid > 0 ? grid : 1), dim3(256), 0, s, a, dlist, nd, pivrow, Wdd, diag);
}
void launch_luc_solve_rows(const LUArgs &a, const int32_t *dlist, int nd, const double *b, const double *xdL, const double *xdU,
                           double *x, hipStream_t s) {
    hipLaunchKernelGGL(k_luc_solve_rows, dim3((a.m + 255) / 256), dim3(256), 0, s, a, dlist, nd, b, xdL, xdU, x);
}
__global__ __launch_bounds__(256) void k_luc_pack_small(LUArgs a, double *__restrict__ out) {
    const int m = a.m;
    const size_t ldw = (size_t)a.ldw;
    const int tid = blockIdx.x * 256 + threadIdx.x, nth = gridDim.x * 256;
    for (int idx = tid; idx < m * m; idx += nth) {
        const int R = idx / m, t = idx % m;
        out[idx] = a.W[(size_t)t * ldw + R];
    }
    double *diag = out + (size_t)m * m;
    for (int R = tid; R < m; R += nth) diag[R] = a.W[(size_t)a.lpos[R] * ldw + R];
    int32_t *io = reinterpret_cast<int32_t *>(diag + m);
    for (int R = tid; R < m; R += nth) { io[R] = a.lpos[R]; io[m + R] = a.dense_flag ? a.dense_flag[R] : 1; }
    int32_t *cb = io + 2 * m;
    const int32_t *src = reinterpret_cast<const int32_t *>(a.ctl_base);
    constexpr int NC = (int)(2 * sizeof(LUCtl) / sizeof(int32_t));
    for (int t = tid; t < NC; t += nth) cb[t] = src[t];
    if (tid == 0) cb[NC] = a.st->lu_singular;
}
size_t luc_pack_small_bytes(int m) { return ((size_t)m * m + m) * sizeof(double) + (size_t)(2 * m + 1) * sizeof(int32_t) + 2 * sizeof(LUCtl); }
void launch_luc_pack_small(const LUArgs &a, double *out, hipStream_t s) {
    const int grid = std::max(1, std::min(64, (a.m * a.m + 255) / 256));
    hipLaunchKernelGGL(k_luc_pack_small, dim3(grid), dim3(256), 0, s, a, out);
}
void launch_luc_pack(const LUArgs &a, const int32_t *dlist, int nd, double *Wd, double *diag, hipStream_t s) {
    dim3 grid((nd + 31) / 32 > 0 ? (nd + 31) / 32 : 1, (a.m + 31) / 32);
    hipLaunchKernelGGL(k_luc_pack, grid, dim3(256), 0, s, a, dlist, nd, Wd, diag);
}

int launch_luc_rounds(const LUArgs &a, int32_t *pivrow, int nrounds, int round_base, hipStream_t s) {
    const int m = a.m;
    {
#ifdef GOMILP_DEBUG
        static const int forced = [] { const char *e = getenv("GOMILP_LUC_SLOTS"); return e ? atoi(e) : -1; }();
        if (forced >= 0) {
            bool done = true;
            switch (forced) {
                case 10: if (m <= 2048) luc_rounds_slots<256, 8, 8>(a, pivrow, nrounds, round_base, s); else done = false; break;
                case 11: if (m <= 2048) luc_rounds_slots<512, 4, 16>(a, pivrow, nrounds, round_base, s); else done = false; break;
                case 12: if (m <= 2048) luc_rounds_slots<1024, 2, 16>(a, pivrow, nrounds, round_base, s); else done = false; break;
                case 13: if (m <= 2048) luc_rounds_slots<512, 4, 8>(a, pivrow, nrounds, round_base, s); else done = false; break;
                case 20: if (m <= 1024) luc_rounds_slots<512, 2, 32>(a, pivrow, nrounds, round_base, s); else done = false; break;
                case 21: if (m <= 1024) luc_rounds_slots<256, 4, 16>(a, pivrow, nrounds, round_base, s); else done = false; break;
                case 22: if (m <= 1024) luc_rounds_slots<512, 2, 16>(a, pivrow, nrounds, round_base, s); else done = false; break;
                case 23: if (m <= 1024) luc_rounds_slots<1024, 1, 32>(a, pivrow, nrounds, round_base, s); else done = false; break;
                case 30: if (m <= 512) luc_rounds_slots<256, 2, 32>(a, pivrow, nrounds, round_base, s); else done = false; break;
                case 31: if (m <= 512) luc_rounds_slots<256, 2, 16>(a, pivrow, nrounds, round_base, s); else done = false; break;
                case 32: if (m <= 512) luc_rounds_slots<128, 4, 16>(a, pivrow, nrounds, round_base, s); else done = false; break;
                default: done = false;
            }
            if (done) return 3 * nrounds;
        }
#endif
        if (m <= 512) luc_rounds_slots<512, 1, 32>(a, pivrow, nrounds, round_base, s);
        else if (m <= 1024) luc_rounds_slots<512, 2, 16>(a, pivrow, nrounds, round_base, s);
        else if (m <= 2048) luc_rounds_slots<1024, 2, 16>(a, pivrow, nrounds, round_base, s);
        else luc_rounds_slots<1024, 4, 8>(a, pivrow, nrounds, round_base, s);
        return 3 * nrounds;
    }
    return 0;
}

#ifdef GOMILP_DEBUG
void luc_stamps_read(unsigned long long *out) { (void)hipMemcpyFromSymbol(out, HIP_SYMBOL(g_luc_stamps), sizeof(unsigned long long) * 64); }
#endif

}
```

gomilp_amd/csrc/lu_host.cpp:

```cpp
#include "lu_host.h"

#include <math.h>

#include <algorithm>
#include <cmath>
#include <vector>

namespace gomilp {

bool lu_det_is_zero(const double *diag, const int32_t *phys, int m) {
    long long esum = 0;
    bool plain = true;
    for (int i = 0; i < m; i++) {
        int e = 0;
        const double d = diag[i];
        if (!(fabs(d) > 0) || !std::isfinite(d)) { plain = false; break; }
        (void)frexp(d, &e);
        esum += e;
    }
    if (plain && (double)(esum - m) * 0.6931471805599453 > -700.0) return false;
    double logdet = 0;
    for (int i = 0; i < m; i++) logdet += log(fabs(diag[phys[i]]));
    return exp(logdet) == 0;
}

namespace {

inline double term(double bi, double va, double xk) { return va != 0 ? (-va) * xk + bi : bi; }

inline double chain(double bi, const double *row, const double *x, int lo, int hi) {
    for (int t = lo; t < hi; t++) bi = term(bi, row[t], x[t]);
    return bi;
}

inline void chain4(double acc[4], const double *const row[4], const double *x, int lo, int hi) {
    double b0 = acc[0], b1 = acc[1], b2 = acc[2], b3 = acc[3];
    const double *r0 = row[0], *r1 = row[1], *r2 = row[2], *r3 = row[3];
    for (int t = lo; t < hi; t++) {
        const double xk = x[t];
        b0 = term(b0, r0[t], xk); b1 = term(b1, r1[t], xk); b2 = term(b2, r2[t], xk); b3 = term(b3, r3[t], xk);
    }
    acc[0] = b0; acc[1] = b1; acc[2] = b2; acc[3] = b3;
}

}

void lu_host_solve(int m, int nd, const int32_t *dl, const int32_t *phys, const double *diag, const double *W, const double *rhs, double *x) {
    for (int i = 0; i < m; i++) x[i] = rhs[phys[i]];
    std::vector<double> xdv(nd);
    double *xd = xdv.data();
    struct Row { int i, below; };
    std::vector<Row> nl;
    nl.reserve(m - nd);
    for (int i = 0, cnt = 0; i < m; i++) {
        if (cnt < nd && dl[cnt] == i) cnt++;
        else nl.push_back({i, cnt});
    }
    const double *row[4];
    double acc[4];
    auto load = [&](size_t g) {
        const int k = (int)std::min<size_t>(4, nl.size() - g);
        for (int r = 0; r < k; r++) { row[r] = W + (size_t)phys[nl[g + r].i] * nd; acc[r] = x[nl[g + r].i]; }
        return k;
    };
    for (int s = 0; s < nd; s++) {
        const int i = dl[s];
        x[i] = xd[s] = chain(x[i], W + (size_t)phys[i] * nd, xd, 0, s);
    }
    for (size_t g = 0; g < nl.size(); g += 4) {
        const int k = load(g);
        const int c0 = k == 4 ? nl[g].below : 0;
        if (k == 4) chain4(acc, row, xd, 0, c0);
        for (int r = 0; r < k; r++) x[nl[g + r].i] = chain(acc[r], row[r], xd, c0, nl[g + r].below);
    }
    for (int s = nd - 1; s >= 0; s--) {
        const int i = dl[s];
        const double tinv = 1 / diag[phys[i]];
        x[i] = xd[s] = chain(x[i], W + (size_t)phys[i] * nd, xd, s + 1, nd) * tinv;
    }
    for (size_t g = 0; g < nl.size(); g += 4) {
        const int k = load(g);
        const int f3 = k == 4 ? nl[g + 3].below : nd;
        for (int r = 0; r < k; r++) acc[r] = chain(acc[r], row[r], xd, nl[g + r].below, f3);
        if (k == 4) chain4(acc, row, xd, f3, nd);
        for (int r = 0; r < k; r++) {
            const int i = nl[g + r].i;
            const double tinv = 1 / diag[phys[i]];
            x[i] = acc[r] * tinv;
        }
    }
}

void lu_host_solve_coupled(int nd, const int32_t *dl, const int32_t *phys, const double *diag, const double *W, const double *rhs,
                           double *xdl, double *xdu) {
    int s = 0;
    for (; s + 4 <= nd; s += 4) {
        const double *row[4];
        double acc[4];
        for (int r = 0; r < 4; r++) { row[r] = W + (size_t)(s + r) * nd; acc[r] = rhs[phys[dl[s + r]]]; }
        chain4(acc, row, xdl, 0, s);
        for (int r = 0; r < 4; r++) xdl[s + r] = chain(acc[r], row[r], xdl, s, s + r);
    }
    for (; s < nd; s++) xdl[s] = chain(rhs[phys[dl[s]]], W + (size_t)s * nd, xdl, 0, s);
    for (s = nd - 1; s >= 0; s--) {
        const double tinv = 1 / diag[phys[dl[s]]];
        xdu[s] = chain(xdl[s], W + (size_t)s * nd, xdu, s + 1, nd) * tinv;
    }
}

}
```

gomilp_amd/csrc/lu_host.h:

```cpp
#pragma once
#include <stdint.h>

namespace gomilp {

bool lu_det_is_zero(const double *diag, const int32_t *phys, int m);

void lu_host_solve(int m, int nd, const int32_t *dl, const int32_t *phys, const double *diag, const double *W, const double *rhs, double *x);

void lu_host_solve_coupled(int nd, const int32_t *dl, const int32_t *phys, const double *diag, const double *W, const double *rhs,
                           double *xdl, double *xdu);

}
```

gomilp_amd/lp.py:

```python
from __future__ import annotations

import ctypes as C
import math
import os
from dataclasses import dataclass, field
from typing import List, Optional

import numpy as np

from . import build as _build

OK, ERR_BLAND, ERR_INFEASIBLE, ERR_LINSOLVE, ERR_UNBOUNDED, ERR_SINGULAR = 0, 1, 2, 3, 4, 5
ERR_ZERO_COLUMN, ERR_ZERO_ROW, ERR_CONDITION, ERR_PHASE1_WRAPPED, ERR_BAD_SHAPE, ERR_PANIC = 6, 7, 8, 9, 10, 11
ERR_DEVICE, ERR_UNSUPPORTED = 12, 13

STATUS_NAMES = {
    OK: "ok", ERR_BLAND: "ErrBland", ERR_INFEASIBLE: "ErrInfeasible", ERR_LINSOLVE: "ErrLinSolve",
    ERR_UNBOUNDED: "ErrUnbounded", ERR_SINGULAR: "ErrSingular", ERR_ZERO_COLUMN: "ErrZeroColumn",
    ERR_ZERO_ROW: "ErrZeroRow", ERR_CONDITION: "mat.Condition", ERR_PHASE1_WRAPPED: "phase1-wrapped",
    ERR_BAD_SHAPE: "panic:badShape", ERR_PANIC: "panic", ERR_DEVICE: "device", ERR_UNSUPPORTED: "unsupported",
}


class Stats(C.Structure):
    _fields_ = [
        ("pivots_phase1", C.c_int64), ("pivots_phase2", C.c_int64), ("bland_steps", C.c_int64),
        ("refreshes", C.c_int64), ("kernel_launches", C.c_int64),
        ("phase1_used", C.c_int32), ("device_id", C.c_int32), ("wrapped_status", C.c_int32), ("pipeline", C.c_int32),
        ("seconds_total", C.c_double), ("seconds_upload", C.c_double), ("seconds_pivot_loop", C.c_double),
        ("seconds_final_solve", C.c_double), ("drift_xb", C.c_double), ("pivot_kernel_seconds", C.c_double * 4),
        ("seconds_final_device", C.c_double), ("seconds_final_host", C.c_double), ("lu_dense_steps", C.c_int64),
        ("lu_rounds", C.c_int64), ("art_exchanges", C.c_int64), ("cond_fallbacks", C.c_int64), ("device_retries", C.c_int64),
        ("cond1_final", C.c_double), ("condinf_final", C.c_double),
    ]


class WarmStats(C.Structure):
    _fields_ = [("warm_started", C.c_int32), ("fallback", C.c_int32), ("new_rows", C.c_int32), ("kept", C.c_int32),
                ("pivots_dual", C.c_int64), ("keep_bytes", C.c_int64), ("seconds_setup", C.c_double), ("seconds_dual", C.c_double)]


WARM_FALLBACKS = {0: "none", 1: "no parent", 2: "parent not kept", 3: "not a descendant", 4: "dual budget spent",
                  5: "no warm path for this mode / shape"}


class Pivot(C.Structure):
    _fields_ = [("phase", C.c_int32), ("bland", C.c_int32), ("min_idx", C.c_int64), ("replace", C.c_int64),
                ("entering", C.c_int64), ("leaving", C.c_int64)]


class FrontierStats(C.Structure):
    _fields_ = [("relaxations", C.c_int64), ("pivots_phase1", C.c_int64), ("pivots_phase2", C.c_int64),
                ("bland_steps", C.c_int64), ("phase1_runs", C.c_int64), ("kernel_launches", C.c_int64),
                ("workers", C.c_int32), ("device_id", C.c_int32), ("seconds_total", C.c_double),
                ("seconds_busy_sum", C.c_double), ("batched_relaxations", C.c_int64), ("host_fallbacks", C.c_int64),
                ("supersteps", C.c_int64), ("seconds_batch", C.c_double), ("blocks", C.c_int64), ("blocks_sampled", C.c_int64),
                ("seconds_inner_kernels", C.c_double), ("seconds_update_kernels", C.c_double),
                ("warm_started", C.c_int64), ("warm_fallbacks", C.c_int64), ("warm_kept", C.c_int64), ("pivots_dual", C.c_int64),
                ("art_exchanges", C.c_int64)]


EXPORTS = [
    "gomilp_lp_solve_warm", "gomilp_frontier_solve_warm", "gomilp_pool_release_warm",
    "gomilp_lp_upload_child", "gomilp_pool_create", "gomilp_pool_destroy", "gomilp_pool_set", "gomilp_pool_set_root", "gomilp_frontier_solve", "gomilp_pool_add_root", "gomilp_frontier_solve_roots", "gomilp_pool_solve_root", "gomilp_debug_find_independent", "gomilp_debug_find_independent_device", "gomilp_debug_cond_estimate", "gomilp_debug_gonum_lu_cond", "gomilp_debug_lu_host_solve",
    "gomilp_lp_simplex", "gomilp_ctx_create", "gomilp_ctx_destroy", "gomilp_ctx_device", "gomilp_ctx_set",
    "gomilp_lp_upload", "gomilp_lp_free", "gomilp_lp_solve_resident", "gomilp_lp_last_trace", "gomilp_version",
    "gomilp_device_count", "gomilp_compiled_arch", "gomilp_comm_unique_id", "gomilp_comm_create", "gomilp_comm_destroy",
    "gomilp_comm_rank", "gomilp_comm_world", "gomilp_incumbent_allreduce", "gomilp_incumbent_pick",
]

_lib = None


def lib():
    global _lib
    if _lib is not None:
        return _lib
    path = _build.build()
    L = C.CDLL(path)
    dp, ip = C.POINTER(C.c_double), C.POINTER(C.c_int64)
    L.gomilp_version.restype = C.c_char_p
    L.gomilp_compiled_arch.restype = C.c_char_p
    L.gomilp_device_count.restype = C.c_int
    L.gomilp_ctx_create.restype = C.c_void_p
    L.gomilp_ctx_create.argtypes = [C.c_int, C.POINTER(C.c_int)]
    L.gomilp_ctx_destroy.argtypes = [C.c_void_p]
    L.gomilp_ctx_device.argtypes = [C.c_void_p]
    L.gomilp_ctx_set.argtypes = [C.c_void_p, C.c_char_p, C.c_int64]
    L.gomilp_lp_upload.restype = C.c_int64
    L.gomilp_lp_upload.argtypes = [C.c_void_p, dp, dp, C.c_int64, dp, C.c_int64, C.c_int64]
    L.gomilp_lp_free.argtypes = [C.c_void_p, C.c_int64]
    L.gomilp_lp_solve_resident.argtypes = [C.c_void_p, C.c_int64, C.c_double, ip, dp, dp, C.POINTER(C.c_int32), ip,
                                           C.POINTER(Stats)]
    L.gomilp_lp_solve_warm.argtypes = [C.c_void_p, C.c_int64, C.c_int64, C.c_int32, C.c_int32, C.c_double, dp, dp,
                                       C.POINTER(C.c_int32), ip, C.POINTER(Stats), C.POINTER(WarmStats)]
    L.gomilp_lp_last_trace.restype = C.c_int64
    L.gomilp_lp_last_trace.argtypes = [C.c_void_p, C.POINTER(Pivot), C.c_int64]
    L.gomilp_lp_simplex.argtypes = [dp, dp, C.c_int64, dp, C.c_int64, C.c_int64, C.c_double, ip, dp, dp,
                                    C.POINTER(C.c_int32), ip, C.POINTER(Stats)]
    i32p = C.POINTER(C.c_int32)
    L.gomilp_lp_upload_child.restype = C.c_int64
    L.gomilp_lp_upload_child.argtypes = [C.c_void_p, C.c_int64, C.c_int32, i32p, dp, dp]
    L.gomilp_pool_create.restype = C.c_void_p
    L.gomilp_pool_create.argtypes = [C.c_int, C.c_int, C.POINTER(C.c_int)]
    L.gomilp_pool_destroy.argtypes = [C.c_void_p]
    L.gomilp_pool_set.argtypes = [C.c_void_p, C.c_char_p, C.c_int64]
    L.gomilp_pool_set_root.argtypes = [C.c_void_p, dp, dp, C.c_int64, dp, C.c_int64, C.c_int64]
    L.gomilp_frontier_solve.argtypes = [C.c_void_p, C.c_int64, ip, i32p, dp, dp, C.c_double, dp, dp, i32p, i32p,
                                        C.POINTER(FrontierStats)]
    L.gomilp_frontier_solve_warm.argtypes = [C.c_void_p, C.c_int64, ip, i32p, dp, dp, ip, ip, i32p, C.c_int32, C.c_double, dp, dp, i32p, i32p,
                                             C.POINTER(FrontierStats)]
    L.gomilp_pool_release_warm.argtypes = [C.c_void_p, C.c_int64]
    L.gomilp_pool_solve_root.argtypes = [C.c_void_p, C.c_double, dp, dp, i32p, C.POINTER(Stats)]
    L.gomilp_pool_add_root.argtypes = [C.c_void_p, dp, dp, C.c_int64, dp, C.c_int64, C.c_int64]
    L.gomilp_frontier_solve_roots.argtypes = [C.c_void_p, C.c_int64, i32p, ip, i32p, dp, dp, C.c_double, dp, dp, C.c_int64, i32p, i32p,
                                              C.POINTER(FrontierStats)]
    L.gomilp_debug_cond_estimate.restype = C.c_double
    L.gomilp_debug_cond_estimate.argtypes = [dp, C.c_int64, C.c_int]
    L.gomilp_debug_gonum_lu_cond.restype = C.c_int
    L.gomilp_debug_gonum_lu_cond.argtypes = [dp, C.c_int64, C.c_int, C.POINTER(C.c_double)]
    L.gomilp_debug_lu_host_solve.restype = C.c_int
    L.gomilp_debug_lu_host_solve.argtypes = [C.c_int64, C.c_int64, i32p, i32p, dp, dp, C.c_int, dp, dp]
    L.gomilp_debug_find_independent.restype = C.c_int64
    L.gomilp_debug_find_independent_device.restype = C.c_int64
    L.gomilp_debug_find_independent_device.argtypes = [C.c_void_p, C.c_int64, ip, C.c_int64]
    L.gomilp_debug_find_independent.argtypes = [dp, C.c_int64, C.c_int64, C.c_int64, ip, C.c_int]
    L.gomilp_comm_unique_id.argtypes = [C.c_char_p]
    L.gomilp_comm_create.restype = C.c_void_p
    L.gomilp_comm_create.argtypes = [C.c_int, C.c_int, C.c_char_p, C.c_int, C.POINTER(C.c_int)]
    L.gomilp_comm_destroy.argtypes = [C.c_void_p]
    L.gomilp_comm_rank.argtypes = [C.c_void_p]
    L.gomilp_comm_world.argtypes = [C.c_void_p]
    L.gomilp_incumbent_allreduce.argtypes = [C.c_void_p, C.c_double, C.c_int64, dp, ip]
    L.gomilp_incumbent_pick.restype = None
    L.gomilp_incumbent_pick.argtypes = [dp, C.c_int, dp, ip]
    _lib = L
    return L


def _dp(a):
    return a.ctypes.data_as(C.POINTER(C.c_double))


def _ip(a):
    return a.ctypes.data_as(C.POINTER(C.c_int64))


@dataclass
class LPResult:
    status: int
    z: float
    x: Optional[np.ndarray]
    basis: Optional[np.ndarray]
    stats: dict = field(default_factory=dict)
    pivots: List[tuple] = field(default_factory=list)

    @property
    def ok(self) -> bool:
        return self.status == OK


def _stats_dict(s: Stats) -> dict:
    d = {k: getattr(s, k) for k, _ in Stats._fields_ if k not in ("pivot_kernel_seconds", "pipeline")}
    d["pipeline"] = {0: "three-kernel", 1: "fused", 2: "tableau", 3: "blocked"}.get(s.pipeline, str(s.pipeline))
    d["pivot_kernel_seconds"] = list(s.pivot_kernel_seconds)
    return d


def simplex(c, A, b, tol: float = 0.0, initial_basic=None) -> LPResult:
    A = np.ascontiguousarray(A, dtype=np.float64)
    c = np.ascontiguousarray(c, dtype=np.float64)
    b = np.ascontiguousarray(b, dtype=np.float64)
    m, n = A.shape
    if c.shape != (n,) or b.shape != (m,):
        return LPResult(ERR_BAD_SHAPE, math.nan, None, None)
    x = np.zeros(n)
    basis = np.zeros(m, dtype=np.int64)
    z = C.c_double(math.nan)
    has_x = C.c_int32(0)
    st = Stats()
    ib = None if initial_basic is None else np.ascontiguousarray(initial_basic, dtype=np.int64)
    if ib is not None and ib.shape != (m,):
        return LPResult(ERR_PANIC, math.nan, None, None)
    rc = lib().gomilp_lp_simplex(_dp(c), _dp(A), n, _dp(b), m, n, float(tol), None if ib is None else _ip(ib),
                                 C.byref(z), _dp(x), C.byref(has_x), _ip(basis), C.byref(st))
    return LPResult(rc, z.value, x if has_x.value else None, basis if has_x.value and m != n else None, _stats_dict(st))


class Context:

    def __init__(self, device: int = -1, **knobs):
        st = C.c_int(0)
        self._h = lib().gomilp_ctx_create(int(device), C.byref(st))
        if not self._h:
            raise RuntimeError("gomilp_ctx_create failed: %s (no HIP device or libgomilp_hip.so not usable)"
                               % STATUS_NAMES.get(st.value, st.value))
        for k, v in knobs.items():
            self.set(k, v)

    def set(self, key: str, value: int) -> None:
        rc = lib().gomilp_ctx_set(self._h, key.encode(), int(value))
        if rc != OK:
            raise ValueError("bad knob %s=%s" % (key, value))

    @property
# ... 226 lines not shown


def find_independent(A, fast: bool = True):
    A = np.ascontiguousarray(A, dtype=np.float64)
    m, n = A.shape
    idx = np.zeros(m, dtype=np.int64)
    cnt = lib().gomilp_debug_find_independent(_dp(A), n, m, n, _ip(idx), 1 if fast else 0)
    if cnt < 0:
        raise ValueError("bad shape")
    return [int(v) for v in idx[:cnt]]


def find_independent_device(A, device: int = -1, **knobs):
    A = np.ascontiguousarray(A, dtype=np.float64)
    m, n = A.shape
    cx = Context(device, **knobs)
    try:
        p = cx.upload(np.zeros(n), A, np.zeros(m))
        idx = np.zeros(m, dtype=np.int64)
        cnt = lib().gomilp_debug_find_independent_device(cx._h, p.pid, _ip(idx), m)
        if cnt < 0:
            raise RuntimeError("device search failed: %s" % STATUS_NAMES.get(-cnt, -cnt))
        return [int(v) for v in idx[:cnt]]
    finally:
        cx.close()


def comm_unique_id() -> bytes:
    buf = C.create_string_buffer(COMM_ID_BYTES)
    rc = lib().gomilp_comm_unique_id(buf)
    if rc != OK:
        raise RuntimeError("gomilp_comm_unique_id failed: %s" % STATUS_NAMES.get(rc, rc))
    return buf.raw


def incumbent_pick(table) -> tuple:
    t = np.ascontiguousarray(table, dtype=np.float64).reshape(-1, 2)
    z = C.c_double(math.inf)
    i = C.c_int64(NO_INCUMBENT)
    lib().gomilp_incumbent_pick(_dp(t), t.shape[0], C.byref(z), C.byref(i))
    return z.value, i.value


class Comm:

    def __init__(self, rank: int, world: int, unique_id: bytes, device: int = -1):
        st = C.c_int(0)
        self._h = lib().gomilp_comm_create(int(rank), int(world), unique_id, int(device), C.byref(st))
        if not self._h:
            raise RuntimeError("gomilp_comm_create failed: %s" % STATUS_NAMES.get(st.value, st.value))
        self.rank, self.world = rank, world

    def incumbent_allreduce(self, z_local: float, index_local: int) -> tuple:
        z = C.c_double(math.inf)
        i = C.c_int64(NO_INCUMBENT)
        rc = lib().gomilp_incumbent_allreduce(self._h, float(z_local), int(index_local), C.byref(z), C.byref(i))
        if rc != OK:
            raise RuntimeError("gomilp_incumbent_allreduce failed: %s" % STATUS_NAMES.get(rc, rc))
        return z.value, i.value

    def close(self) -> None:
        if self._h:
            lib().gomilp_comm_destroy(self._h)
            self._h = None

    def __del__(self):
        try:
            self.close()
        except Exception:
            pass


def debug_gonum_lu_cond(M, transposed: bool = False):
    M = np.ascontiguousarray(M, dtype=np.float64)
    n = M.shape[0]
    assert M.shape == (n, n)
    c = C.c_double(0.0)
    rc = lib().gomilp_debug_gonum_lu_cond(_dp(M), n, 1 if transposed else 0, C.byref(c))
    if rc < 0:
        raise ValueError("n out of range")
    return float(c.value), bool(rc)


def debug_lu_host_solve(dl, phys, diag, W, rhs, coupled: bool = False):
    dl = np.ascontiguousarray(dl, dtype=np.int32)
    phys = np.ascontiguousarray(phys, dtype=np.int32)
    diag = np.ascontiguousarray(diag, dtype=np.float64)
    W = np.ascontiguousarray(W, dtype=np.float64)
    rhs = np.ascontiguousarray(rhs, dtype=np.float64)
    m, nd = phys.size, dl.size
    assert diag.shape == (m,) and rhs.shape == (m,) and W.shape == ((nd if coupled else m), nd)
    x = np.zeros(nd if coupled else m)
    i32p = C.POINTER(C.c_int32)
    rc = lib().gomilp_debug_lu_host_solve(m, nd, dl.ctypes.data_as(i32p), phys.ctypes.data_as(i32p), _dp(diag), _dp(W), 1 if coupled else 0, _dp(rhs), _dp(x))
    if rc < 0:
        raise ValueError("bad shape")
    return x, bool(rc)


def debug_cond_estimate(B, inf: bool = False) -> float:
    B = np.ascontiguousarray(B, dtype=np.float64)
    n = B.shape[0]
    assert B.shape == (n, n)
    return float(lib().gomilp_debug_cond_estimate(_dp(B), n, 1 if inf else 0))
```

include/gomilp_lp.h:

```cpp
#ifndef GOMILP_LP_H
#define GOMILP_LP_H

#include <stdint.h>

#ifdef __cplusplus
extern "C" {
#endif

typedef enum {
    GOMILP_OK = 0,
    GOMILP_ERR_BLAND = 1,
    GOMILP_ERR_INFEASIBLE = 2,
    GOMILP_ERR_LINSOLVE = 3,
    GOMILP_ERR_UNBOUNDED = 4,
    GOMILP_ERR_SINGULAR = 5,
    GOMILP_ERR_ZERO_COLUMN = 6,
    GOMILP_ERR_ZERO_ROW = 7,
    GOMILP_ERR_CONDITION = 8,
    GOMILP_ERR_PHASE1_WRAPPED = 9,
    GOMILP_ERR_BAD_SHAPE = 10,
    GOMILP_ERR_PANIC = 11,
    GOMILP_ERR_DEVICE = 12,
    GOMILP_ERR_UNSUPPORTED = 13
} gomilp_status;
// ... 58 lines not shown

int64_t gomilp_lp_upload_child(gomilp_ctx *ctx, int64_t root_problem, int32_t K, const int32_t *var, const double *sign,
                               const double *rhs);

typedef struct gomilp_warm_stats {
    int32_t warm_started;
    int32_t fallback;
    int32_t new_rows;
    int32_t kept;
    int64_t pivots_dual;
    int64_t keep_bytes;
    double seconds_setup;
    double seconds_dual;
} gomilp_warm_stats;

int gomilp_lp_solve_warm(gomilp_ctx *ctx, int64_t problem, int64_t parent, int32_t keep, int32_t dual_budget, double tol,
                         double *opt_f, double *opt_x, int32_t *has_x, int64_t *basis_out,
                         gomilp_lp_stats *stats, gomilp_warm_stats *wstats);

typedef struct gomilp_pool gomilp_pool;

typedef struct gomilp_frontier_stats {
    int64_t relaxations;
    int64_t pivots_phase1, pivots_phase2, bland_steps, phase1_runs;
    int64_t kernel_launches;
    int32_t workers, device_id;
    double seconds_total;
    double seconds_busy_sum;
    int64_t batched_relaxations;
    int64_t host_fallbacks;
    int64_t supersteps;
    double seconds_batch;
    int64_t blocks;
    int64_t blocks_sampled;
    double seconds_inner_kernels;
    double seconds_update_kernels;
    int64_t warm_started;
    int64_t warm_fallbacks;
    int64_t warm_kept;
    int64_t pivots_dual;
    int64_t art_exchanges;
} gomilp_frontier_stats;

gomilp_pool *gomilp_pool_create(int device, int workers, int *status);
void gomilp_pool_destroy(gomilp_pool *pool);
int gomilp_pool_set(gomilp_pool *pool, const char *key, int64_t value);
int gomilp_pool_set_root(gomilp_pool *pool, const double *c0, const double *A0, int64_t lda, const double *b0, int64_t m0,
                         int64_t n0);
int gomilp_frontier_solve(gomilp_pool *pool, int64_t count, const int64_t *koff, const int32_t *var, const double *sign,
                          const double *rhs, double tol, double *z_out, double *x_out, int32_t *status_out,
                          int32_t *has_x_out, gomilp_frontier_stats *stats);

typedef struct gomilp_comm gomilp_comm;
#define GOMILP_COMM_ID_BYTES 128
#define GOMILP_NO_INCUMBENT ((int64_t)1 << 52)
int gomilp_comm_unique_id(char *id_out);
gomilp_comm *gomilp_comm_create(int rank, int world, const char *id, int device, int *status);
void gomilp_comm_destroy(gomilp_comm *comm);
int gomilp_comm_rank(const gomilp_comm *comm);
int gomilp_comm_world(const gomilp_comm *comm);
int gomilp_incumbent_allreduce(gomilp_comm *comm, double local_z, int64_t local_index, double *global_z,
                               int64_t *global_index);
void gomilp_incumbent_pick(const double *table, int world, double *global_z, int64_t *global_index);

int gomilp_pool_solve_root(gomilp_pool *pool, double tol, double *opt_f, double *opt_x, int32_t *has_x, gomilp_lp_stats *stats);

int gomilp_frontier_solve_warm(gomilp_pool *pool, int64_t count, const int64_t *koff, const int32_t *var, const double *sign,
                               const double *rhs, const int64_t *parent, const int64_t *tag, const int32_t *keep, int32_t dual_budget,
                               double tol, double *z_out, double *x_out, int32_t *status_out, int32_t *has_x_out,
                               gomilp_frontier_stats *stats);
int gomilp_pool_release_warm(gomilp_pool *pool, int64_t tag);

int gomilp_pool_add_root(gomilp_pool *pool, const double *c, const double *A, int64_t lda, const double *b, int64_t m, int64_t n);
int gomilp_frontier_solve_roots(gomilp_pool *pool, int64_t count, const int32_t *root_of, const int64_t *koff, const int32_t *var,
                                const double *sign, const double *rhs, double tol, double *z_out, double *x_out, int64_t ldx,
                                int32_t *status_out, int32_t *has_x_out, gomilp_frontier_stats *stats);

int64_t gomilp_debug_find_independent(const double *A, int64_t lda, int64_t m, int64_t n, int64_t *idx_out, int fast);
int64_t gomilp_debug_find_independent_device(gomilp_ctx *ctx, int64_t problem, int64_t *idx_out, int64_t cap);
double gomilp_debug_cond_estimate(const double *B, int64_t n, int inf);
int gomilp_debug_gonum_lu_cond(const double *M, int64_t n, int transposed, double *cond);
int gomilp_debug_lu_host_solve(int64_t m, int64_t nd, const int32_t *dl, const int32_t *phys, const double *diag, const double *W, int coupled,
                               const double *rhs, double *x);

const char *gomilp_version(void);
int gomilp_device_count(void);
const char *gomilp_compiled_arch(void);

#ifdef __cplusplus
}
#endif
#endif
```

Before: 212,000.

## Pack LU factors on device in-loop and defer condition-check readback

For non-large LU plans, each round batch now ends with a device-side finish and pack kernel. The packed dense factor block, using a bounded leading dimension, is copied back in the same synchronisation, so the separate pack-and-fetch round trip goes away. The round batch size is estimated from the projected dense count, and a new lu_batch knob can override it. The condition-number check is now enqueued asynchronously and its verdict read at final extraction, which removes one stream sync per solve. The cost is a strided W layout that the host solvers must honour, and wasted work if the dense-count bound is underestimated.

```diff
diff --git a/gomilp_amd/csrc/c_api.cpp b/gomilp_amd/csrc/c_api.cpp
--- a/gomilp_amd/csrc/c_api.cpp
+++ b/gomilp_amd/csrc/c_api.cpp
@@ -731,14 +731,19 @@
 
 int gomilp_debug_lu_host_solve(int64_t m, int64_t nd, const int32_t *dl, const int32_t *phys, const double *diag, const double *W, int coupled,
                                const double *rhs, double *x) {
-    if (m < 1 || m > 16384 || nd < 0 || nd > m || !phys || !diag || !rhs || !x || (nd > 0 && (!dl || !W))) return -1;
+    return gomilp_debug_lu_host_solve_ld(m, nd, dl, phys, diag, W, nd, coupled, rhs, x);
+}
+
+int gomilp_debug_lu_host_solve_ld(int64_t m, int64_t nd, const int32_t *dl, const int32_t *phys, const double *diag, const double *W, int64_t ld,
+                                  int coupled, const double *rhs, double *x) {
+    if (m < 1 || m > 16384 || nd < 0 || nd > m || ld < nd || ld > 16384 || !phys || !diag || !rhs || !x || (nd > 0 && (!dl || !W))) return -1;
     const int64_t nx = coupled ? nd : m;
     for (int64_t i = 0; i < nx; i++) x[i] = 0.0;
     if (gomilp::lu_det_is_zero(diag, phys, (int)m)) return 1;
     if (coupled) {
         std::vector<double> xdl((size_t)nd);
-        gomilp::lu_host_solve_coupled((int)nd, dl, phys, diag, W, rhs, xdl.data(), x);
-    } else gomilp::lu_host_solve((int)m, (int)nd, dl, phys, diag, W, rhs, x);
+        gomilp::lu_host_solve_coupled((int)nd, dl, phys, diag, W, (int)ld, rhs, xdl.data(), x);
+    } else gomilp::lu_host_solve((int)m, (int)nd, dl, phys, diag, W, (int)ld, rhs, x);
     return 0;
 }
 
diff --git a/gomilp_amd/csrc/device_types.h b/gomilp_amd/csrc/device_types.h
--- a/gomilp_amd/csrc/device_types.h
+++ b/gomilp_amd/csrc/device_types.h
@@ -234,6 +234,7 @@
     int32_t next[32];
     uint32_t cnt_x, cnt_u, cnt_s;
     int32_t fault;
+    int32_t nd;
 };
 
 struct LUArgs {
diff --git a/gomilp_amd/csrc/engine.cpp b/gomilp_amd/csrc/engine.cpp
--- a/gomilp_amd/csrc/engine.cpp
+++ b/gomilp_amd/csrc/engine.cpp
@@ -83,6 +83,7 @@
     else if (key == "fused") fused_ = v ? 1 : 0;
     else if (key == "lu_look") lu_look_ = v ? 1 : 0;
     else if (key == "lu_large") lu_large_ = v ? 1 : 0;
+    else if (key == "lu_batch") { if (v < 0 || v > 4096) return GOMILP_ERR_BAD_SHAPE; lu_batch_ = v; }
     else if (key == "lu_blocked") lu_blocked_ = v < 0 ? 0 : (v > 2 ? 3 : v);
     else if (key == "tableau") tableau_ = v ? 1 : 0;
     else if (key == "blocked") blocked_ = v ? 1 : 0;
@@ -131,6 +132,7 @@
         HIP_TRY(hipHostMalloc(reinterpret_cast<void **>(&w.st_host), sizeof(DevState), hipHostMallocDefault));
         HIP_TRY(dmalloc(&w.luctl, 2));
         HIP_TRY(hipHostMalloc(reinterpret_cast<void **>(&w.luctl_host), 2 * sizeof(LUCtl), hipHostMallocDefault));
+        HIP_TRY(hipHostMalloc(reinterpret_cast<void **>(&w.h_cond), 4 * sizeof(double), hipHostMallocDefault));
         w.trace_cap = 1 << 18;
         HIP_TRY(dmalloc(&w.trace, (size_t)w.trace_cap));
         HIP_TRY(hipEventCreate(&w.ev[0])); HIP_TRY(hipEventCreate(&w.ev[1]));
@@ -1101,6 +1103,8 @@
     const double inf = std::numeric_limits<double>::infinity();
     const int m = P.m, n = P.n;
     Work &w = *w_;
+    const int cond_pending = cond_pending_;
+    cond_pending_ = 0;
     if (loop_rc == GOMILP_ERR_DEVICE) return loop_rc;
     const bool loop_unbounded = loop_rc == GOMILP_ERR_UNBOUNDED;
     if (loop_unbounded && !shadow_trace_) { *opt_f = -inf; return loop_rc; }
@@ -1109,6 +1113,13 @@
     HIP_TRY(hipMemcpyAsync(w.h_vec, w.xb, (size_t)m * sizeof(double), hipMemcpyDeviceToHost, stream_));
     HIP_TRY(sync_stream());
     for (int i = 0; i < m; i++) { basic[i] = w.h_idx[i]; xb[i] = w.h_vec[i]; }
+    if (cond_pending && loop_rc == GOMILP_OK) {
+        double k1 = 0, kinf = 0;
+        const int rcc = cond_verdict(P, cond_pending == 1, &k1, &kinf);
+        if (rcc != GOMILP_OK) return rcc;
+        st->cond1_final = k1; st->condinf_final = kinf;
+        if (k1 > 1e16 || k1 != k1 || kinf > 1e16 || kinf != kinf) loop_rc = GOMILP_ERR_CONDITION;
+    }
     if (shadow_trace_ && (loop_rc == GOMILP_OK || loop_rc == GOMILP_ERR_BLAND || loop_unbounded)) {
         HIP_TRY(hipMemcpyAsync(w.st_host, w.st, sizeof(DevState), hipMemcpyDeviceToHost, stream_));
         HIP_TRY(sync_stream());
diff --git a/gomilp_amd/csrc/engine.hpp b/gomilp_amd/csrc/engine.hpp
--- a/gomilp_amd/csrc/engine.hpp
+++ b/gomilp_amd/csrc/engine.hpp
@@ -54,11 +54,12 @@
     bool oneshot = false;
     bool inject_fault = false;
     int steps_down = 0;
-    bool split(int nd) const { return compressed && m >= 1024 && nd > 0; }
+    bool split_rows() const { return compressed && m >= 1024; }
+    bool split(int nd) const { return split_rows() && nd > 0; }
     static LuPlan make(int m, int64_t lu_blocked, int64_t lu_look, int64_t lu_cross, int64_t lu_large, int64_t bt_fault, size_t small_pack_cap_bytes);
     bool step_down();
 };
-struct LuRoundsEnd { bool gave_up = false, landed = false; int enq = 0; };
+struct LuRoundsEnd { bool gave_up = false, landed = false, packed = false; int enq = 0, ld = 0; };
 
 class Engine {
    public:
@@ -172,7 +173,7 @@
     int pack_and_fetch(const LUArgs &a, const LuPlan &plan, std::vector<int32_t> &dl);
     struct LuCache {
         bool valid = false, split = false, singular = false;
-        int m = 0, nd = 0;
+        int m = 0, nd = 0, ld = 0;
         std::vector<int32_t> phys, dl;
         std::vector<double> diag;
         LUArgs args;
@@ -184,6 +185,9 @@
     int exact_column_check(const Problem &P, const std::vector<int32_t> &basic, const std::vector<double> &dsol, const double *col_dev,
                            double *binv_dst, bool *rebuilt, gomilp_lp_stats *st);
     int cond_check(const Problem &P, int nn, double *k1, double *kinf);
+    int cond_enqueue(const Problem &P, int nn, bool *enqueued);
+    int cond_verdict(const Problem &P, bool enqueued, double *k1, double *kinf);
+    int cond_pending_ = 0;
     int cond_fresh(const Problem &P, const int32_t *basic_host, double *k1, double *kinf);
     int groups_knob(const Problem &P) const;
     bool ensure_host_A(const Problem &P);
@@ -207,6 +211,7 @@
     int lu_look_fault_ = 0;
     int64_t lu_look_ = 1;
     int64_t lu_large_ = 0;
+    int64_t lu_batch_ = 0;
     int64_t chunk_ = 32, refresh_ = 0, trace_on_ = 0, max_pivots_ = 0, sample_events_ = 0, fused_ = 1, lu_blocked_ = 3, tableau_ = 1, blocked_ = 1, block_k_ = 0,
             bt_nt_ = 0, bt_old_ = 0, bt_stamps_ = 0, bt_upd_valu_ = 0, bt_fault_ = 0, general_device_ = 1, general_block_ = 1, general_min_rows_ = 96, lu_cross_ = -1, bt_groups_ = 0,
             bt_lag_ = 1,
@@ -367,6 +372,7 @@
 int launch_lu_blocked(const LUArgs &a, int32_t *pivrow, hipStream_t s);
 bool lu_compressed_supported(int m, bool large);
 int lu_compressed_nb();
+int luc_round_slots(int m);
 void launch_luc_init(const LUArgs &a, hipStream_t s);
 int launch_luc_rounds(const LUArgs &a, int32_t *pivrow, int nrounds, int round_base, hipStream_t s);
 void launch_luc_gather(const double *At, int ld, int m, const int32_t *basic, double *W, int ldw, hipStream_t s);
@@ -374,6 +380,9 @@
 void launch_luc_solve_rows(const LUArgs &a, const int32_t *dlist, int nd, const double *b, const double *xdL, const double *xdU,
                            double *x, hipStream_t s);
 void launch_luc_pack(const LUArgs &a, const int32_t *dlist, int nd, double *Wd, double *diag, hipStream_t s);
+void launch_luc_finish(const LUArgs &a, LUCtl *base, int last_parity, bool cross, int bound, int32_t *dlist, hipStream_t s);
+void launch_luc_pack_dense_dev(const LUArgs &a, const int32_t *dlist, const int32_t *ndp, int bound, const int32_t *pivrow, double *Wdd, double *diag, hipStream_t s);
+void launch_luc_pack_dev(const LUArgs &a, const int32_t *dlist, const int32_t *ndp, int bound, double *Wd, double *diag, hipStream_t s);
 void launch_luc_pack_small(const LUArgs &a, double *out, hipStream_t s);
 size_t luc_pack_small_bytes(int m);
 void launch_lu_pack(const LUArgs &a, const int32_t *dlist, int nd, double *Wd, double *diag, hipStream_t s);
diff --git a/gomilp_amd/csrc/engine_final.cpp b/gomilp_amd/csrc/engine_final.cpp
--- a/gomilp_amd/csrc/engine_final.cpp
+++ b/gomilp_amd/csrc/engine_final.cpp
@@ -83,15 +83,24 @@
     launch_luc_init(a, stream_);
     launches_++;
     const int nb = lu_compressed_nb();
-    int batch = std::max(1, (std::min(m, (5 * nonunit) / 2) + nb - 1) / nb);
+    const bool tail = !plan.large;
+    const int slots = plan.cross_G ? plan.cross_slots : luc_round_slots(m);
+    const int est = std::min(m, 3 * nonunit);
+    int batch = tail && !plan.oneshot ? (est + slots - 1) / slots + 1 : std::max(1, (std::min(m, (5 * nonunit) / 2) + nb - 1) / nb);
+    if (lu_batch_ > 0) batch = (int)std::min<int64_t>(lu_batch_, (m + nb - 1) / nb + 64);
+    int expect = est + std::max(32, est / 8);
     bool oneshot = plan.oneshot;
     if (oneshot && GOMILP_DBG_ENV("GOMILP_DEBUG_LU_SHORT")) batch = 1;
     int enq = 0;
     int k_seen = -1;
+    bool packed = false;
+    int bound = 0;
     const LUCtl *last = w.luctl_host;
     for (;;) {
         launches_ += plan.cross_G ? launch_luc_rounds_cross(a, w.rho, batch, enq, w.luxrec, plan.cross_G, plan.cross_slots, stream_) : launch_luc_rounds(a, w.rho, batch, enq, stream_);
         enq += batch;
+        const int lastp = a.look ? ((enq - 1) & 1) : 0;
+        packed = false;
         if (oneshot) {
             launch_luc_pack_small(a, w.Wd, stream_);
             launches_++;
@@ -104,24 +113,49 @@
             memcpy(h_dense, io + m, (size_t)m * sizeof(int32_t));
             memcpy(w.luctl_host, io + 2 * m, 2 * sizeof(LUCtl));
             w.st_host->lu_singular = io[2 * m + (int)(2 * sizeof(LUCtl) / sizeof(int32_t))];
+        } else if (tail) {
+            bound = (int)std::min<int64_t>(std::min(m, expect), (int64_t)nb * enq);
+            launch_luc_finish(a, w.luctl, lastp, plan.cross_G != 0, bound, w.dlist, stream_);
+            if (plan.split_rows()) launch_luc_pack_dense_dev(a, w.dlist, &w.luctl->nd, bound, w.rho, w.Wd, w.ludiag, stream_);
+            else launch_luc_pack_dev(a, w.dlist, &w.luctl->nd, bound, w.Wd, w.ludiag, stream_);
+            launches_ += 2;
+            HIP_TRY(hipMemcpyAsync(w.luctl_host, w.luctl, 2 * sizeof(LUCtl), hipMemcpyDeviceToHost, stream_));
+            HIP_TRY(hipMemcpyAsync(h_dense, w.denseflag, (size_t)m * sizeof(int32_t), hipMemcpyDeviceToHost, stream_));
+            HIP_TRY(hipMemcpyAsync(w.h_W, w.Wd, (size_t)(plan.split_rows() ? bound : m) * bound * sizeof(double), hipMemcpyDeviceToHost, stream_));
+            HIP_TRY(hipMemcpyAsync(w.h_vec, w.ludiag, (size_t)m * sizeof(double), hipMemcpyDeviceToHost, stream_));
+            HIP_TRY(hipMemcpyAsync(w.h_idx, w.lpos, (size_t)m * sizeof(int32_t), hipMemcpyDeviceToHost, stream_));
+            if (plan.small)
+                HIP_TRY(hipMemcpyAsync(&w.st_host->lu_singular, &w.st->lu_singular, sizeof(w.st_host->lu_singular), hipMemcpyDeviceToHost, stream_));
+            else
+                HIP_TRY(hipMemcpyAsync(w.st_host, w.st, sizeof(DevState), hipMemcpyDeviceToHost, stream_));
+            HIP_TRY(sync_stream());
+            packed = true;
         } else {
             HIP_TRY(hipMemcpyAsync(w.luctl_host, w.luctl, 2 * sizeof(LUCtl), hipMemcpyDeviceToHost, stream_));
             HIP_TRY(hipMemcpyAsync(h_dense, w.denseflag, (size_t)m * sizeof(int32_t), hipMemcpyDeviceToHost, stream_));
             HIP_TRY(sync_stream());
         }
-        last = w.luctl_host + (a.look ? ((enq - 1) & 1) : 0);
+        last = w.luctl_host + lastp;
         if (w.luctl_host[0].fault || last->k_next >= m) break;
         if (last->k_next <= k_seen) return GOMILP_ERR_DEVICE;
         k_seen = last->k_next;
         oneshot = false;
-        batch = std::max(4, (int)(((int64_t)(m - last->k_next) * last->rounds) / std::max(1, last->k_next)) + 2);
+        if (tail) {
+            int d = 0;
+            for (int k = 0; k < last->k_next; k++) d += h_dense[k] != 0;
+            const int64_t proj = d + ((int64_t)(m - last->k_next) * d) / std::max(1, (int)last->k_next);
+            expect = (int)std::min<int64_t>(m, proj + std::max<int64_t>(32, proj / 4));
+        }
+        batch = std::max(tail ? 1 : 4, (int)(((int64_t)(m - last->k_next) * last->rounds) / std::max(1, last->k_next)) + 2);
         if (batch > 64) batch = 64;
     }
     lu_rounds_ = last->rounds;
     end->gave_up = w.luctl_host[0].fault != 0;
     end->landed = oneshot;
+    end->packed = packed && !end->gave_up && w.luctl_host[0].nd >= 0;
+    end->ld = bound;
     end->enq = enq;
-    if (plan.cross_G && !end->gave_up) { launch_luc_lpos_final(a, stream_); launches_++; }
+    if (plan.cross_G && !end->gave_up && !packed) { launch_luc_lpos_final(a, stream_); launches_++; }
     return GOMILP_OK;
 }
 
@@ -212,6 +246,11 @@
         const int32_t *h_dense = w.h_idx + w.cap_m;
         lu_dense_ = 0;
         for (int k = 0; k < m; k++) lu_dense_ += h_dense[k] != 0;
+    } else if (end.packed) {
+        const int32_t *h_dense = w.h_idx + w.cap_m;
+        for (int k = 0; k < m; k++) if (h_dense[k]) dl.push_back(k);
+        if ((int)dl.size() != w.luctl_host[0].nd) return GOMILP_ERR_DEVICE;
+        lu_dense_ = (int64_t)dl.size();
     } else {
         if ((rc = pack_and_fetch(a, plan, dl)) != GOMILP_OK) return rc;
         lu_dense_ = (int64_t)dl.size();
@@ -231,6 +270,7 @@
                 (int)transpose, m, nd, (long long)lu_rounds_, (int)w.st_host->lu_singular, logdet, nz, dmin, (int)plan.compressed);
     }
     lu_cache_.m = m; lu_cache_.nd = nd; lu_cache_.split = !end.landed && plan.split(nd); lu_cache_.singular = *singular;
+    lu_cache_.ld = end.packed ? end.ld : nd;
     lu_cache_.phys = phys; lu_cache_.dl = dl;
     lu_cache_.diag.assign(diag, diag + m);
     lu_cache_.args = a;
@@ -244,12 +284,12 @@
     const LuCache &c = lu_cache_;
     if (!c.valid || c.m != P.m) return GOMILP_ERR_DEVICE;
     const double tf1 = now_s();
-    const int m = P.m, nd = c.nd;
+    const int m = P.m, nd = c.nd, ld = c.ld;
     const double *rhs = rhs_host ? rhs_host : P.hb.data();
     x.assign(m, 0.0);
     if (c.singular) return GOMILP_OK;
     if (!c.split) {
-        lu_host_solve(m, nd, c.dl.data(), c.phys.data(), c.diag.data(), w.h_W, rhs, x.data());
+        lu_host_solve(m, nd, c.dl.data(), c.phys.data(), c.diag.data(), w.h_W, ld, rhs, x.data());
         fs_host_ += now_s() - tf1;
         return GOMILP_OK;
     }
@@ -260,7 +300,7 @@
         rhs_dev = w.move;
     }
     std::vector<double> xdl(nd), xdu(nd);
-    lu_host_solve_coupled(nd, c.dl.data(), c.phys.data(), c.diag.data(), w.h_W, rhs, xdl.data(), xdu.data());
+    lu_host_solve_coupled(nd, c.dl.data(), c.phys.data(), c.diag.data(), w.h_W, ld, rhs, xdl.data(), xdu.data());
     fs_host_ += now_s() - tf1;
     const double tf2 = now_s();
     double *dxl = w.yscratch, *dxu = w.yscratch + P.ld, *dx = w.yscratch + 2 * (size_t)P.ld;
diff --git a/gomilp_amd/csrc/engine_tableau.cpp b/gomilp_amd/csrc/engine_tableau.cpp
--- a/gomilp_amd/csrc/engine_tableau.cpp
+++ b/gomilp_amd/csrc/engine_tableau.cpp
@@ -623,6 +623,7 @@
         for (int j = 0; j < ncols; j++) if (!inb[j]) nonbasic.push_back(j);
     };
     tcur_ = 0; rcur_ = 0; t_tiled_ = false;
+    cond_pending_ = 0;
     if (!binv_host && (rc = stage_upload(w.rho, rho.data(), (size_t)m * sizeof(int32_t))) != GOMILP_OK) return rc;
     std::vector<double> art(P.ld, 0.0);
     bool binv_on_device = gen_binv_dev_;
@@ -798,26 +799,41 @@
     launches_ += 2;
     *loop_rc = use_bt_ ? run_loop_bt(P, 2, tol, nn, st) : run_loop_tab(P, 2, tol, nn, st);
     if (*loop_rc == GOMILP_OK && cond_guard_ && !binv_host && m > 64) {
-        double k1 = 0, kinf = 0;
-        if ((rc = cond_check(P, nn, &k1, &kinf)) != GOMILP_OK) return rc;
-        st->cond1_final = k1; st->condinf_final = kinf;
-        if (k1 > 1e16 || k1 != k1 || kinf > 1e16 || kinf != kinf) *loop_rc = GOMILP_ERR_CONDITION;
+        bool enq = false;
+        if ((rc = cond_enqueue(P, nn, &enq)) != GOMILP_OK) return rc;
+        cond_pending_ = enq ? 1 : 2;
     }
     return GOMILP_OK;
 }
 
 int Engine::cond_check(const Problem &P, int nn, double *k1, double *kinf) {
-    Work &w = *w_;
+    bool enq = false;
     *k1 = *kinf = 0.0;
+    int rc = cond_enqueue(P, nn, &enq);
+    if (rc != GOMILP_OK) return rc;
+    if (enq) HIP_TRY(sync_stream());
+    return cond_verdict(P, enq, k1, kinf);
+}
+
+int Engine::cond_enqueue(const Problem &P, int nn, bool *enqueued) {
+    Work &w = *w_;
+    *enqueued = false;
     const size_t need = (size_t)ldt_ + 3 * (size_t)P.ld + 4;
     if (need > (size_t)64 * w.cap_ldt) return GOMILP_OK;
     launch_cond_check(w.T[tcur_], ldt_, P.m, nn, w.nonbasic, w.basic, P.dAt, P.ld, P.n - P.m, P.n, w.tscratch, t_tiled_, stream_);
     launches_ += 3;
-    HIP_TRY(hipMemcpyAsync(w.h_vec, w.tscratch + (size_t)ldt_ + 3 * (size_t)P.ld, 4 * sizeof(double), hipMemcpyDeviceToHost, stream_));
-    HIP_TRY(sync_stream());
-    const double b1 = w.h_vec[0], binf = w.h_vec[2];
-    *k1 = b1 * w.h_vec[1];
-    *kinf = binf * w.h_vec[3];
+    HIP_TRY(hipMemcpyAsync(w.h_cond, w.tscratch + (size_t)ldt_ + 3 * (size_t)P.ld, 4 * sizeof(double), hipMemcpyDeviceToHost, stream_));
+    *enqueued = true;
+    return GOMILP_OK;
+}
+
+int Engine::cond_verdict(const Problem &P, bool enqueued, double *k1, double *kinf) {
+    Work &w = *w_;
+    *k1 = *kinf = 0.0;
+    if (!enqueued) return GOMILP_OK;
+    const double b1 = w.h_cond[0], binf = w.h_cond[2];
+    *k1 = b1 * w.h_cond[1];
+    *kinf = binf * w.h_cond[3];
     if (!(*k1 > 1e16) && !(*kinf > 1e16)) return GOMILP_OK;
     const int m = P.m;
     const double tk1 = *k1, tkinf = *kinf;
diff --git a/gomilp_amd/csrc/engine_work.hpp b/gomilp_amd/csrc/engine_work.hpp
--- a/gomilp_amd/csrc/engine_work.hpp
+++ b/gomilp_amd/csrc/engine_work.hpp
@@ -95,6 +95,7 @@
     DevState *st = nullptr;
     DevState *st_host = nullptr;
     LUCtl *luctl = nullptr, *luctl_host = nullptr;
+    double *h_cond = nullptr;
     DevPivot *trace = nullptr;
     int64_t trace_cap = 0;
     double *h_W = nullptr;
@@ -155,6 +156,7 @@
         }
         if (luctl) hipFree(luctl); luctl = nullptr;
         if (luctl_host) hipHostFree(luctl_host); luctl_host = nullptr;
+        if (h_cond) hipHostFree(h_cond); h_cond = nullptr;
     }
 };
 
diff --git a/gomilp_amd/csrc/lu_compressed.hip b/gomilp_amd/csrc/lu_compressed.hip
--- a/gomilp_amd/csrc/lu_compressed.hip
+++ b/gomilp_amd/csrc/lu_compressed.hip
@@ -507,10 +507,46 @@
     for (int R = threadIdx.x; R < ldw; R += 256) dst[R] = R < m ? src[R] : 0.0;
 }
 
-__global__ __launch_bounds__(256) void k_luc_pack(LUArgs a, const int32_t *__restrict__ dlist, int nd, double *__restrict__ Wd,
-                                                  double *__restrict__ diag) {
+__global__ __launch_bounds__(1024) void k_luc_finish(LUArgs a, LUCtl *base, int last_parity, int cross, int bound, int32_t *__restrict__ dlist) {
+    __shared__ int s_cnt[16];
+    __shared__ int s_base;
+    const int tid = threadIdx.x, lane = tid & 63, w = tid >> 6;
+    const int m = a.m;
+    if (base->fault || base[last_parity].k_next < m) {
+        if (tid == 0) base->nd = -1;
+        return;
+    }
+    if (cross)
+        for (int R = tid; R < m; R += 1024) a.lpos[R] = a.rowstep[R];
+    if (tid == 0) s_base = 0;
+    __syncthreads();
+    for (int k0 = 0; k0 < m; k0 += 1024) {
+        const int k = k0 + tid;
+        const bool dense = k < m && a.dense_flag[k] != 0;
+        const unsigned long long mask = __ballot(dense);
+        if (lane == 0) s_cnt[w] = __popcll(mask);
+        __syncthreads();
+        int at = s_base;
+        for (int v = 0; v < w; v++) at += s_cnt[v];
+        at += __popcll(mask & ((1ull << lane) - 1ull));
+        if (dense && at < bound) dlist[at] = k;
+        __syncthreads();
+        if (tid == 1023) s_base = at + (dense ? 1 : 0);
+        __syncthreads();
+    }
+    if (tid == 0) base->nd = s_base <= bound ? s_base : -2;
+}
+void launch_luc_finish(const LUArgs &a, LUCtl *base, int last_parity, bool cross, int bound, int32_t *dlist, hipStream_t s) {
+    hipLaunchKernelGGL(k_luc_finish, dim3(1), dim3(1024), 0, s, a, base, last_parity, cross ? 1 : 0, bound, dlist);
+}
+
+__global__ __launch_bounds__(256) void k_luc_pack(LUArgs a, const int32_t *__restrict__ dlist, int nd, const int32_t *__restrict__ ndp, int ld,
+                                                  double *__restrict__ Wd, double *__restrict__ diag) {
     __shared__ double tile[32][33];
+    if (ndp) nd = *ndp;
+    if (nd < 0 || nd > ld) return;
     const int t0 = blockIdx.x * 32, R0 = blockIdx.y * 32;
+    if (t0 >= nd && blockIdx.x > 0) return;
     const int tx = threadIdx.x & 31, ty = threadIdx.x >> 5;
     const size_t ldw = (size_t)a.ldw;
     for (int tt = ty; tt < 32; tt += 8) {
@@ -520,7 +556,7 @@
     __syncthreads();
     for (int rr = ty; rr < 32; rr += 8) {
         const int R = R0 + rr, t = t0 + tx;
-        if (R < a.m && t < nd) Wd[(size_t)R * nd + t] = tile[tx][rr];
+        if (R < a.m && t < nd) Wd[(size_t)R * ld + t] = tile[tx][rr];
     }
     if (blockIdx.x == 0 && threadIdx.x < 32) {
         const int R = R0 + threadIdx.x;
@@ -529,44 +565,96 @@
 }
 
 
-__global__ __launch_bounds__(256) void k_luc_pack_dense(LUArgs a, const int32_t *__restrict__ dlist, int nd,
+__global__ __launch_bounds__(256) void k_luc_pack_dense(LUArgs a, const int32_t *__restrict__ dlist, int nd, const int32_t *__restrict__ ndp, int ld,
                                                         const int32_t *__restrict__ pivrow, double *__restrict__ Wdd,
                                                         double *__restrict__ diag) {
+    if (ndp) nd = *ndp;
+    if (nd < 0 || nd > ld) return;
     const size_t ldw = (size_t)a.ldw;
     const int s = blockIdx.x;
     if (s < nd) {
         const int R = pivrow[dlist[s]];
-        for (int t = threadIdx.x; t < nd; t += 256) Wdd[(size_t)s * nd + t] = a.W[(size_t)dlist[t] * ldw + R];
+        for (int t = threadIdx.x; t < nd; t += 256) Wdd[(size_t)s * ld + t] = a.W[(size_t)dlist[t] * ldw + R];
     }
     for (int R = blockIdx.x * 256 + threadIdx.x; R < a.m; R += gridDim.x * 256) diag[R] = a.W[(size_t)a.lpos[R] * ldw + R];
 }
 
-__global__ __launch_bounds__(256) void k_luc_solve_rows(LUArgs a, const int32_t *__restrict__ dlist, int nd,
-                                                        const double *__restrict__ b, const double *__restrict__ xdL,
-                                                        const double *__restrict__ xdU, double *__restrict__ x) {
-    const int R = blockIdx.x * 256 + threadIdx.x;
-    if (R >= a.m) return;
+constexpr int kSolveTrip = 16, kSolveBufs = 3, kSolveChunk = 528;
+constexpr int kSolvePad = (2 * kSolveBufs - 1) * kSolveTrip;
+struct SolveStage { int col[kSolveChunk + kSolvePad]; double2 x[kSolveChunk + kSolvePad]; };
+__device__ __forceinline__ void luc_solve_load(const double *__restrict__ Wr, size_t ldw, const SolveStage &st, int t0, double (&va)[kSolveTrip]) {
+#pragma unroll
+    for (int u = 0; u < kSolveTrip; u++) va[u] = Wr[(size_t)st.col[t0 + u] * ldw];
+}
+__device__ __forceinline__ double luc_solve_sum(double acc, const SolveStage &st, int t0, int n, int below, const double (&va)[kSolveTrip]) {
+    double xk[kSolveTrip];
+    double2 xx[kSolveTrip];
+#pragma unroll
+    for (int u = 0; u < kSolveTrip; u++) xx[u] = st.x[t0 + u];
+#pragma unroll
+    for (int u = 0; u < kSolveTrip; u++) xk[u] = t0 + u < below ? xx[u].x : xx[u].y;
+#pragma unroll
+    for (int u = 0; u < kSolveTrip; u++) {
+        const double sum = __dadd_rn(__dmul_rn(-va[u], xk[u]), acc);
+        acc = (t0 + u < n && va[u] != 0) ? sum : acc;
+    }
+    return acc;
+}
+__global__ __launch_bounds__(64) __attribute__((amdgpu_waves_per_eu(1, 1))) void k_luc_solve_rows(LUArgs a, const int32_t *__restrict__ dlist, int nd,
+                                                       const double *__restrict__ b, const double *__restrict__ xdL,
+                                                       const double *__restrict__ xdU, double *__restrict__ x) {
+    __shared__ SolveStage st;
+    if (nd <= 0) return;
+    const int tid = threadIdx.x;
+    const int Rm = blockIdx.x * 64 + tid;
+    const int R = Rm < a.m ? Rm : a.m - 1;
     const int i = a.lpos[R];
-    if (a.dense_flag[i]) return;
+    const bool mine = Rm < a.m && !a.dense_flag[i];
     const size_t ldw = (size_t)a.ldw;
     int lo = 0, hi = nd;
     while (lo < hi) { const int mid = (lo + hi) >> 1; if (dlist[mid] < i) lo = mid + 1; else hi = mid; }
     const int cnt = lo;
     double acc = b[R];
-    for (int t0 = 0; t0 < nd; t0 += 8) {
-        double va[8], xk[8];
-#pragma unroll
-        for (int u = 0; u < 8; u++) {
-            const int t = t0 + u;
-            va[u] = t < nd ? a.W[(size_t)dlist[t < nd ? t : 0] * ldw + R] : 0.0;
-            xk[u] = t < nd ? (t < cnt ? xdL[t] : xdU[t]) : 0.0;
-        }
-#pragma unroll
-        for (int u = 0; u < 8; u++)
-            if (va[u] != 0) acc = __dadd_rn(__dmul_rn(-va[u], xk[u]), acc);
-    }
-    const double tinv = 1.0 / a.W[(size_t)i * ldw + R];
-    x[i] = __dmul_rn(acc, tinv);
+    const double uii = a.W[(size_t)i * ldw + R];
+    const double *__restrict__ Wr = a.W + R;
+    for (int c0 = 0; c0 < nd; c0 += kSolveChunk) {
+        const int n = nd - c0 < kSolveChunk ? nd - c0 : kSolveChunk;
+        __syncthreads();
+        {
+            constexpr int kIters = (kSolveChunk + kSolvePad + 63) / 64;
+            int cc[kIters];
+            double xl[kIters], xu[kIters];
+#pragma unroll
+            for (int j = 0; j < kIters; j++) {
+                const int t = tid + 64 * j, src = c0 + (t < n ? t : 0);
+                cc[j] = dlist[src]; xl[j] = xdL[src]; xu[j] = xdU[src];
+            }
+#pragma unroll
+            for (int j = 0; j < kIters; j++) {
+                const int t = tid + 64 * j;
+                if (t < kSolveChunk + kSolvePad) {
+                    st.col[t] = cc[j];
+                    st.x[t] = t < n ? make_double2(xl[j], xu[j]) : make_double2(0.0, 0.0);
+                }
+            }
+        }
+        __syncthreads();
+        const int below = cnt - c0;
+        double vaA[kSolveTrip], vaB[kSolveTrip], vaC[kSolveTrip];
+        luc_solve_load(Wr, ldw, st, 0, vaA);
+        luc_solve_load(Wr, ldw, st, kSolveTrip, vaB);
+        luc_solve_load(Wr, ldw, st, 2 * kSolveTrip, vaC);
+        for (int t0 = 0; t0 < n; t0 += 3 * kSolveTrip) {
+            acc = luc_solve_sum(acc, st, t0, n, below, vaA);
+            luc_solve_load(Wr, ldw, st, t0 + 3 * kSolveTrip, vaA);
+            acc = luc_solve_sum(acc, st, t0 + kSolveTrip, n, below, vaB);
+            luc_solve_load(Wr, ldw, st, t0 + 4 * kSolveTrip, vaB);
+            acc = luc_solve_sum(acc, st, t0 + 2 * kSolveTrip, n, below, vaC);
+            luc_solve_load(Wr, ldw, st, t0 + 5 * kSolveTrip, vaC);
+        }
+    }
+    const double tinv = 1.0 / uii;
+    if (mine) x[i] = __dmul_rn(acc, tinv);
 }
 
 constexpr int kLucSlotSteps = 32;
@@ -638,6 +726,7 @@
 
 bool lu_compressed_supported(int m, bool large) { return m <= 4096 || (large && luc_large_rpt(m) > 0); }
 int lu_compressed_nb() { return kLucSlotSteps; }
+int luc_round_slots(int m) { return m <= 512 ? 32 : (m <= 2048 ? 16 : 8); }
 
 void launch_luc_init(const LUArgs &a, hipStream_t s) {
     hipLaunchKernelGGL(k_luc_init, dim3((a.m + 255) / 256), dim3(256), 0, s, a);
@@ -647,11 +736,15 @@
 }
 void launch_luc_pack_dense(const LUArgs &a, const int32_t *dlist, int nd, const int32_t *pivrow, double *Wdd, double *diag, hipStream_t s) {
     const int grid = std::max(nd, (a.m + 255) / 256);
-    hipLaunchKernelGGL(k_luc_pack_dense, dim3(grid > 0 ? grid : 1), dim3(256), 0, s, a, dlist, nd, pivrow, Wdd, diag);
+    hipLaunchKernelGGL(k_luc_pack_dense, dim3(grid > 0 ? grid : 1), dim3(256), 0, s, a, dlist, nd, (const int32_t *)nullptr, nd, pivrow, Wdd, diag);
+}
+void launch_luc_pack_dense_dev(const LUArgs &a, const int32_t *dlist, const int32_t *ndp, int bound, const int32_t *pivrow, double *Wdd, double *diag, hipStream_t s) {
+    const int grid = std::max(bound, (a.m + 255) / 256);
+    hipLaunchKernelGGL(k_luc_pack_dense, dim3(grid > 0 ? grid : 1), dim3(256), 0, s, a, dlist, 0, ndp, bound, pivrow, Wdd, diag);
 }
 void launch_luc_solve_rows(const LUArgs &a, const int32_t *dlist, int nd, const double *b, const double *xdL, const double *xdU,
                            double *x, hipStream_t s) {
-    hipLaunchKernelGGL(k_luc_solve_rows, dim3((a.m + 255) / 256), dim3(256), 0, s, a, dlist, nd, b, xdL, xdU, x);
+    hipLaunchKernelGGL(k_luc_solve_rows, dim3((a.m + 63) / 64), dim3(64), 0, s, a, dlist, nd, b, xdL, xdU, x);
 }
 __global__ __launch_bounds__(256) void k_luc_pack_small(LUArgs a, double *__restrict__ out) {
     const int m = a.m;
@@ -678,7 +771,11 @@
 }
 void launch_luc_pack(const LUArgs &a, const int32_t *dlist, int nd, double *Wd, double *diag, hipStream_t s) {
     dim3 grid((nd + 31) / 32 > 0 ? (nd + 31) / 32 : 1, (a.m + 31) / 32);
-    hipLaunchKernelGGL(k_luc_pack, grid, dim3(256), 0, s, a, dlist, nd, Wd, diag);
+    hipLaunchKernelGGL(k_luc_pack, grid, dim3(256), 0, s, a, dlist, nd, (const int32_t *)nullptr, nd, Wd, diag);
+}
+void launch_luc_pack_dev(const LUArgs &a, const int32_t *dlist, const int32_t *ndp, int bound, double *Wd, double *diag, hipStream_t s) {
+    dim3 grid((bound + 31) / 32 > 0 ? (bound + 31) / 32 : 1, (a.m + 31) / 32);
+    hipLaunchKernelGGL(k_luc_pack, grid, dim3(256), 0, s, a, dlist, 0, ndp, bound, Wd, diag);
 }
 
 int launch_luc_rounds(const LUArgs &a, int32_t *pivrow, int nrounds, int round_base, hipStream_t s) {
diff --git a/gomilp_amd/csrc/lu_host.cpp b/gomilp_amd/csrc/lu_host.cpp
--- a/gomilp_amd/csrc/lu_host.cpp
+++ b/gomilp_amd/csrc/lu_host.cpp
@@ -45,7 +45,7 @@
 
 }
 
-void lu_host_solve(int m, int nd, const int32_t *dl, const int32_t *phys, const double *diag, const double *W, const double *rhs, double *x) {
+void lu_host_solve(int m, int nd, const int32_t *dl, const int32_t *phys, const double *diag, const double *W, int ld, const double *rhs, double *x) {
     for (int i = 0; i < m; i++) x[i] = rhs[phys[i]];
     std::vector<double> xdv(nd);
     double *xd = xdv.data();
@@ -60,12 +60,12 @@
     double acc[4];
     auto load = [&](size_t g) {
         const int k = (int)std::min<size_t>(4, nl.size() - g);
-        for (int r = 0; r < k; r++) { row[r] = W + (size_t)phys[nl[g + r].i] * nd; acc[r] = x[nl[g + r].i]; }
+        for (int r = 0; r < k; r++) { row[r] = W + (size_t)phys[nl[g + r].i] * ld; acc[r] = x[nl[g + r].i]; }
         return k;
     };
     for (int s = 0; s < nd; s++) {
         const int i = dl[s];
-        x[i] = xd[s] = chain(x[i], W + (size_t)phys[i] * nd, xd, 0, s);
+        x[i] = xd[s] = chain(x[i], W + (size_t)phys[i] * ld, xd, 0, s);
     }
     for (size_t g = 0; g < nl.size(); g += 4) {
         const int k = load(g);
@@ -76,7 +76,7 @@
     for (int s = nd - 1; s >= 0; s--) {
         const int i = dl[s];
         const double tinv = 1 / diag[phys[i]];
-        x[i] = xd[s] = chain(x[i], W + (size_t)phys[i] * nd, xd, s + 1, nd) * tinv;
+        x[i] = xd[s] = chain(x[i], W + (size_t)phys[i] * ld, xd, s + 1, nd) * tinv;
     }
     for (size_t g = 0; g < nl.size(); g += 4) {
         const int k = load(g);
@@ -91,20 +91,20 @@
     }
 }
 
-void lu_host_solve_coupled(int nd, const int32_t *dl, const int32_t *phys, const double *diag, const double *W, const double *rhs,
+void lu_host_solve_coupled(int nd, const int32_t *dl, const int32_t *phys, const double *diag, const double *W, int ld, const double *rhs,
                            double *xdl, double *xdu) {
     int s = 0;
     for (; s + 4 <= nd; s += 4) {
         const double *row[4];
         double acc[4];
-        for (int r = 0; r < 4; r++) { row[r] = W + (size_t)(s + r) * nd; acc[r] = rhs[phys[dl[s + r]]]; }
+        for (int r = 0; r < 4; r++) { row[r] = W + (size_t)(s + r) * ld; acc[r] = rhs[phys[dl[s + r]]]; }
         chain4(acc, row, xdl, 0, s);
         for (int r = 0; r < 4; r++) xdl[s + r] = chain(acc[r], row[r], xdl, s, s + r);
     }
-    for (; s < nd; s++) xdl[s] = chain(rhs[phys[dl[s]]], W + (size_t)s * nd, xdl, 0, s);
+    for (; s < nd; s++) xdl[s] = chain(rhs[phys[dl[s]]], W + (size_t)s * ld, xdl, 0, s);
     for (s = nd - 1; s >= 0; s--) {
         const double tinv = 1 / diag[phys[dl[s]]];
-        xdu[s] = chain(xdl[s], W + (size_t)s * nd, xdu, s + 1, nd) * tinv;
+        xdu[s] = chain(xdl[s], W + (size_t)s * ld, xdu, s + 1, nd) * tinv;
     }
 }
 
diff --git a/gomilp_amd/csrc/lu_host.h b/gomilp_amd/csrc/lu_host.h
--- a/gomilp_amd/csrc/lu_host.h
+++ b/gomilp_amd/csrc/lu_host.h
@@ -5,9 +5,9 @@
 
 bool lu_det_is_zero(const double *diag, const int32_t *phys, int m);
 
-void lu_host_solve(int m, int nd, const int32_t *dl, const int32_t *phys, const double *diag, const double *W, const double *rhs, double *x);
+void lu_host_solve(int m, int nd, const int32_t *dl, const int32_t *phys, const double *diag, const double *W, int ld, const double *rhs, double *x);
 
-void lu_host_solve_coupled(int nd, const int32_t *dl, const int32_t *phys, const double *diag, const double *W, const double *rhs,
+void lu_host_solve_coupled(int nd, const int32_t *dl, const int32_t *phys, const double *diag, const double *W, int ld, const double *rhs,
                            double *xdl, double *xdu);
 
 }
diff --git a/gomilp_amd/lp.py b/gomilp_amd/lp.py
--- a/gomilp_amd/lp.py
+++ b/gomilp_amd/lp.py
@@ -62,7 +62,7 @@
 
 EXPORTS = [
     "gomilp_lp_solve_warm", "gomilp_frontier_solve_warm", "gomilp_pool_release_warm",
-    "gomilp_lp_upload_child", "gomilp_pool_create", "gomilp_pool_destroy", "gomilp_pool_set", "gomilp_pool_set_root", "gomilp_frontier_solve", "gomilp_pool_add_root", "gomilp_frontier_solve_roots", "gomilp_pool_solve_root", "gomilp_debug_find_independent", "gomilp_debug_find_independent_device", "gomilp_debug_cond_estimate", "gomilp_debug_gonum_lu_cond", "gomilp_debug_lu_host_solve",
+    "gomilp_lp_upload_child", "gomilp_pool_create", "gomilp_pool_destroy", "gomilp_pool_set", "gomilp_pool_set_root", "gomilp_frontier_solve", "gomilp_pool_add_root", "gomilp_frontier_solve_roots", "gomilp_pool_solve_root", "gomilp_debug_find_independent", "gomilp_debug_find_independent_device", "gomilp_debug_cond_estimate", "gomilp_debug_gonum_lu_cond", "gomilp_debug_lu_host_solve", "gomilp_debug_lu_host_solve_ld",
     "gomilp_lp_simplex", "gomilp_ctx_create", "gomilp_ctx_destroy", "gomilp_ctx_device", "gomilp_ctx_set",
     "gomilp_lp_upload", "gomilp_lp_free", "gomilp_lp_solve_resident", "gomilp_lp_last_trace", "gomilp_version",
     "gomilp_device_count", "gomilp_compiled_arch", "gomilp_comm_unique_id", "gomilp_comm_create", "gomilp_comm_destroy",
@@ -121,6 +121,8 @@
     L.gomilp_debug_gonum_lu_cond.argtypes = [dp, C.c_int64, C.c_int, C.POINTER(C.c_double)]
     L.gomilp_debug_lu_host_solve.restype = C.c_int
     L.gomilp_debug_lu_host_solve.argtypes = [C.c_int64, C.c_int64, i32p, i32p, dp, dp, C.c_int, dp, dp]
+    L.gomilp_debug_lu_host_solve_ld.restype = C.c_int
+    L.gomilp_debug_lu_host_solve_ld.argtypes = [C.c_int64, C.c_int64, i32p, i32p, dp, dp, C.c_int64, C.c_int, dp, dp]
     L.gomilp_debug_find_independent.restype = C.c_int64
     L.gomilp_debug_find_independent_device.restype = C.c_int64
     L.gomilp_debug_find_independent_device.argtypes = [C.c_void_p, C.c_int64, ip, C.c_int64]
@@ -513,17 +515,18 @@
     return float(c.value), bool(rc)
 
 
-def debug_lu_host_solve(dl, phys, diag, W, rhs, coupled: bool = False):
+def debug_lu_host_solve(dl, phys, diag, W, rhs, coupled: bool = False, ld=None):
     dl = np.ascontiguousarray(dl, dtype=np.int32)
     phys = np.ascontiguousarray(phys, dtype=np.int32)
     diag = np.ascontiguousarray(diag, dtype=np.float64)
     W = np.ascontiguousarray(W, dtype=np.float64)
     rhs = np.ascontiguousarray(rhs, dtype=np.float64)
     m, nd = phys.size, dl.size
-    assert diag.shape == (m,) and rhs.shape == (m,) and W.shape == ((nd if coupled else m), nd)
+    ld = nd if ld is None else int(ld)
+    assert diag.shape == (m,) and rhs.shape == (m,) and W.shape == ((nd if coupled else m), ld)
     x = np.zeros(nd if coupled else m)
     i32p = C.POINTER(C.c_int32)
-    rc = lib().gomilp_debug_lu_host_solve(m, nd, dl.ctypes.data_as(i32p), phys.ctypes.data_as(i32p), _dp(diag), _dp(W), 1 if coupled else 0, _dp(rhs), _dp(x))
+    rc = lib().gomilp_debug_lu_host_solve_ld(m, nd, dl.ctypes.data_as(i32p), phys.ctypes.data_as(i32p), _dp(diag), _dp(W), ld, 1 if coupled else 0, _dp(rhs), _dp(x))
     if rc < 0:
         raise ValueError("bad shape")
     return x, bool(rc)
diff --git a/include/gomilp_lp.h b/include/gomilp_lp.h
--- a/include/gomilp_lp.h
+++ b/include/gomilp_lp.h
@@ -164,6 +164,8 @@
 int gomilp_debug_gonum_lu_cond(const double *M, int64_t n, int transposed, double *cond);
 int gomilp_debug_lu_host_solve(int64_t m, int64_t nd, const int32_t *dl, const int32_t *phys, const double *diag, const double *W, int coupled,
                                const double *rhs, double *x);
+int gomilp_debug_lu_host_solve_ld(int64_t m, int64_t nd, const int32_t *dl, const int32_t *phys, const double *diag, const double *W, int64_t ld,
+                                  int coupled, const double *rhs, double *x);
 
 const char *gomilp_version(void);
 int gomilp_device_count(void);
```

Result: no change. 213,000, median of 3 (+0.5%).
